# AlfredUg/MiCall-Lite

Hardware: AMD Instinct MI355X
Metric: paired 2×251 nt reads/sec mapped+realigned; fraction of HBM roofline (higher is better)
Workload: dtype int32; 1 GPU; C2: synthetic 2x251 nt HIV-1 pol read pairs (10% divergent sample genome, 0.5% errors), prelim_map end-to-end vs 74 seeds + 1 remap iteration(s) (--local vs consensus) + pileups, default projects.json; pairs_per_gpu=1000000, read_len=251, parallelism=dp1 (one GPU, no collective), dist_world=1

## Files before the change

### include/micall_hip.h

```cpp
#ifndef MICALL_HIP_H
#define MICALL_HIP_H

#include <stddef.h>
#include <stdint.h>

#ifdef __cplusplus
extern "C" {
#endif

#define MH_MAXOPS 128

enum { MH_E2E = 0, MH_LOCAL = 1 };
enum { MH_OP_M = 0, MH_OP_I = 1, MH_OP_D = 2, MH_OP_S = 4 };

typedef struct {
    int mode;
    int rdg_open, rdg_ext;
    int rfg_open, rfg_ext;
    int maxins;
} mh_params;

typedef struct {
    int32_t ref, pos, rev, score, secbest, flag, mapq, rnext, pnext, tlen;
    int32_t sam_ref, sam_pos, xm, xo, xg, nm, ys, yt, yf, n_cigar;
// ... 21 lines not shown
int mh_reads_count(mh_ctx *ctx, int64_t *n_reads, int *paired);

typedef struct mh_fastq mh_fastq;
int mh_fastq_open_part(const char *path, int fd, int part, int parts, mh_fastq **out, int64_t *info);
int mh_fastq_scan_part(const char *path, int fd, int part, int parts, int64_t *info);
int mh_fastq_member_open(const char *path, int fd, int part, int parts, mh_fastq **out, int64_t *info);
int mh_fastq_member_decode(mh_fastq *fq, int64_t end_bit, int64_t *info);
int mh_fastq_member_tail(mh_fastq *fq, const char *window, char *tail);
int mh_fastq_member_finish(mh_fastq *fq, const char *window, int64_t c0, int64_t c1, int64_t *info);
int mh_fastq_frame(mh_fastq *fq, int64_t line0, int starts_line, int64_t *out5);
int mh_fastq_record_offset(mh_fastq *fq, int64_t k, int64_t *off);
int mh_fastq_splice(mh_fastq *fq, int64_t lo, int64_t hi, const char *front, int64_t flen,
                    const char *back, int64_t blen);
int mh_fastq_view(mh_fastq *fq, const char **data, int64_t *len);
int mh_fastq_close(mh_fastq *fq);
int mh_fastq_parse(mh_fastq *fq1, mh_fastq *fq2, char *names, size_t names_cap, uint8_t *seq,
                   uint8_t *qual, size_t bases_cap, int32_t *lens, int64_t reads_cap, int64_t *n_reads,
                   int64_t *n_bases, size_t *names_used);
int mh_reads_load_staged(mh_ctx *ctx, mh_fastq *fq1, mh_fastq *fq2, const int64_t *range4,
                         int64_t fastq_lines1, int64_t *n_reads);
int mh_reads_fastq_lines(mh_ctx *ctx, int64_t *lines1);

int mh_map(mh_ctx *ctx, const mh_params *par);
int mh_alns_fetch(mh_ctx *ctx, int64_t first, int64_t n, mh_aln *out);
int mh_map_counts(mh_ctx *ctx, int64_t *lines, int64_t *filtered, int64_t *mapped,
                  int64_t *first_row, int64_t *first_mapped, int64_t *unmapped,
                  int64_t *star_lines, int64_t *star_first);
int mh_map_stats(mh_ctx *ctx, int64_t *out5);
int mh_test_set_capacities(mh_ctx *ctx, int64_t cigar_pool_words, int64_t pileup_events,
                           int64_t pileup_event_bytes, int64_t token_bytes);
int mh_test_pileup_info(mh_ctx *ctx, int64_t *out16, int n_refs, int32_t *win_len);
int mh_test_force_index_collision(mh_ctx *ctx, int on);
int mh_retry_counts(mh_ctx *ctx, int64_t *out4);
int mh_test_set_gotoh_wait(mh_ctx *ctx, int64_t ticks);
int mh_recs_fetch(mh_ctx *ctx, int64_t first, int64_t n, int32_t *out20);
int mh_recs_fetch_fields(mh_ctx *ctx, int64_t first, int64_t n, int field0, int nfields, int32_t *out);
int mh_reads_set_names(mh_ctx *ctx, int64_t n, const char *const *names);
int mh_format_rows(mh_ctx *ctx, int style, const int64_t *order, int64_t first, int64_t n,
                   const char *const *refnames, char *buf, size_t cap, size_t *used);
int mh_format_segments(mh_ctx *ctx, int style, const int64_t *order, int64_t n,
                       const char *const *refnames, int n_seg, const int64_t *seg_rows,
                       int64_t *seg_bytes);
int mh_write_segments(mh_ctx *ctx, int fd, const int64_t *seg_off, uint32_t *crc);
uint32_t mh_crc32_combine(uint32_t a, uint32_t b, int64_t len_b);
int mh_file_crc32(int fd, int64_t *size, uint32_t *crc);
enum { MH_PHASE_INFLATE = 0, MH_PHASE_PARSE = 1, MH_PHASE_UPLOAD = 2, MH_PHASE_FORMAT = 3,
       MH_PHASE_WRITE = 4, MH_PHASES = 5 };
int mh_phase_times(mh_ctx *ctx, double *ms, int reset);
int mh_write_rows_crc(mh_ctx *ctx, int style, const int64_t *order, int64_t first, int64_t n,
                      const char *const *refnames, int fd, int64_t offset, int64_t *written,
                      uint32_t *crc);

int mh_rows_load(mh_ctx *ctx, int64_t n_rows, const int32_t *flag, const int32_t *ref,
                 const int32_t *pos, const int32_t *cigar_off, const int32_t *n_cigar,
                 const uint32_t *cigar, const uint8_t *seq, const uint8_t *qual,
                 const int64_t *offsets, const int32_t *lens, int64_t n_units,
                 const int64_t *unit_rows);
int mh_rows_load_csv(mh_ctx *ctx, const char *text, int64_t len, int n_refs,
                     const char *const *refnames, int64_t *n_rows, int64_t *n_units,
                     int32_t *n_present);
int mh_rows_info(mh_ctx *ctx, int32_t *out4, int32_t *present, char *unknown, size_t cap);
#define MH_PILEUP_SLACK 2048
int mh_pileup(mh_ctx *ctx, int source, int q_cutoff, int n_refs, const int32_t *ref_lens);
int mh_pileup_only(mh_ctx *ctx, int source, int q_cutoff, int n_refs, const int32_t *ref_lens, int n_sel,
                   const int32_t *sel);
int mh_pileup_dims(mh_ctx *ctx, int *n_refs, int32_t *cap, int64_t *n_events,
// ... 132 lines not shown
```

### micall-lite_amd/csrc/mh_a2c.hip

```cpp
#include <algorithm>
#include <atomic>
#include <charconv>
#include <chrono>
#include <cstring>
#include <deque>
#include <map>
#include <string>
#include <unordered_map>
#include <vector>

#include "mh_gunzip.h"
#include "mh_internal.h"
#include "mh_sam2aln.h"
#include "mh_text.h"

namespace mh {

constexpr int A2C_W = 21;
constexpr int A2C_LANES = 3 * A2C_W;
constexpr int A2C_CHUNK = 1024;
constexpr int A2C_NAA = 21;
constexpr int A2C_STRIDE = A2C_NAA + 18;
constexpr int A2C_CELLS = A2C_LANES * A2C_STRIDE;
constexpr int A2C_SLOTS = 4;
// ... 698 lines not shown
    if (int st = a2c_upload(S, S.d_bin_rows, bin_rows.data(), bin_rows.size(), s)) return st;
    if (int st = a2c_upload(S, S.d_chunks, chunks.data(), chunks.size(), s)) return st;
    if (int st = a2c_upload(S, S.d_code, S.code, 512, s)) return st;
    if (int st = a2c_upload(S, S.d_cls, S.cls, 256, s)) return st;
    return a2c_count_chunks(c, S, chunks.size());
}

static int a2c_count_chunks(Ctx &c, A2CState &S, size_t n_chunks)
{
    hipStream_t s = c.stream;
    const size_t cells = (size_t)S.n_bins * A2C_CELLS;
    if (int st = a2c_reserve(S, S.d_cnt, sizeof(uint32_t) * cells)) return st;
    if (int st = a2c_reserve(S, S.d_first, sizeof(uint32_t) * cells)) return st;
    if (cells) {
        MH_HIP(hipMemsetAsync(S.d_cnt, 0, sizeof(uint32_t) * cells, s));
        MH_HIP(hipMemsetAsync(S.d_first, 0xff, sizeof(uint32_t) * cells, s));
    }
    if (n_chunks) {
        A2CCountArgs a{S.d_text, S.d_rows, S.d_bin_rows, S.d_chunks, S.d_code, S.d_cls,
                       S.d_cnt, S.d_first};
        const int p0 = prof_begin(c, "k_a2c_count");
        hipLaunchKernelGGL(k_a2c_count, dim3((unsigned)n_chunks), dim3(256), 0, s, a);
        prof_end(c, p0);
        MH_HIP(hipGetLastError());
    }
    S.h_cnt.resize(cells);
    S.h_first.resize(cells);
    if (cells) {
        MH_HIP(hipMemcpyAsync(S.h_cnt.data(), S.d_cnt, sizeof(uint32_t) * cells,
                              hipMemcpyDeviceToHost, s));
        MH_HIP(hipMemcpyAsync(S.h_first.data(), S.d_first, sizeof(uint32_t) * cells,
                              hipMemcpyDeviceToHost, s));
    }
    MH_HIP(hipStreamSynchronize(s));
    prof_flush(c);
    return 0;
}

static int a2c_parse_csv(A2CState &S, const char *text, int64_t len, bool &use_pool,
                         int64_t body_lo = -1, int64_t body_hi = -1)
{
    const char *p = text, *end = text + len;
    std::vector<std::string> head;
    S.rows.clear();
    S.dev_rows = false;
    S.g_first.assign(1, 0);
    S.g_ref.clear();
    S.g_qcut.clear();
    S.pool.clear();
    use_pool = false;
    if (!csv_record(p, end, head)) return 0;
    if (body_lo >= 0) {
        p = text + std::max<int64_t>(body_lo, p - text);
        end = text + std::max<int64_t>(body_hi, p - text);
    }
    static const char *const want[N_COLS] = {"refname", "qcut", "count", "offset", "seq"};
    int col[N_COLS];
    int need = 0;
    for (int k = 0; k < N_COLS; ++k) {
        col[k] = -1;
        for (size_t z = 0; z < head.size(); ++z)
            if (head[z] == want[k]) col[k] = (int)z;
        need = std::max(need, col[k] + 1);
    }
    const int64_t body = end - p;
    const bool quoted = memchr(p, '"', (size_t)body) != nullptr;
    for (int k = 0; k < N_COLS; ++k)
// ... 188 lines not shown
    S.g_qcut.clear();
    for (int64_t g = 0; g < ng; ++g) {
        S.g_ref.push_back(Q.names[(size_t)O.g_name[g]]);
        S.g_qcut.push_back(std::to_string(O.g_qcut[g]));
    }
    S.g_ncod.assign(3 * (size_t)ng, 0);
    S.g_bin0.assign((size_t)ng + 1, 0);
    S.n_bins = 0;
    hipStream_t s = c.stream;
    if (int st = a2c_upload(S, S.d_code, S.code, 512, s)) return st;
    if (int st = a2c_upload(S, S.d_cls, S.cls, 256, s)) return st;
    size_t n_chunks = 0;
    auto t1 = t0;
    if (n) {
        std::vector<int32_t> gfirst(O.g_first.begin(), O.g_first.end());
        if (int st = a2c_upload(S, S.d_order, O.rows.data(), (size_t)n, s)) return st;
        if (int st = a2c_upload(S, S.d_gfirst, gfirst.data(), gfirst.size(), s)) return st;
        if (int st = a2c_reserve(S, S.d_text, (size_t)text_len + 16)) return st;
        if (int st = a2c_reserve(S, S.d_rows, sizeof(A2CRow) * (size_t)n)) return st;
        if (int st = a2c_reserve(S, S.d_ncod, sizeof(int32_t) * (3 * (size_t)ng + 1))) return st;
        MH_HIP(hipMemcpyAsync(S.d_text, Q.d_gather, (size_t)text_len, hipMemcpyDeviceToDevice, s));
        MH_HIP(hipMemsetAsync(S.d_text + text_len, 0, 16, s));
        MH_HIP(hipMemsetAsync(S.d_ncod, 0, sizeof(int32_t) * (3 * (size_t)ng + 1), s));
        int64_t per_block = (n + 2047) / 2048;
        per_block = std::max<int64_t>(256 / A2C_TEAM, (per_block + 15) & ~(int64_t)15);
        A2CStageArgs a{S.d_order, S.d_gfirst, Q.d_goff, Q.d_res, Q.d_uniq, S.d_text, S.d_cls, S.d_rows,
                       S.d_ncod, (int32_t)n, (int32_t)ng, (int32_t)per_block};
        const int p0 = prof_begin(c, "k_a2c_stage");
        hipLaunchKernelGGL(k_a2c_stage, dim3((unsigned)((n + per_block - 1) / per_block)), dim3(256), 0, s, a);
        prof_end(c, p0);
        MH_HIP(hipGetLastError());
        std::vector<int32_t> ncod(3 * (size_t)ng + 1);
        MH_HIP(hipMemcpyAsync(ncod.data(), S.d_ncod, sizeof(int32_t) * ncod.size(), hipMemcpyDeviceToHost, s));
        MH_HIP(hipStreamSynchronize(s));
        prof_flush(c);
        if (ncod[3 * (size_t)ng]) return 1;
        S.t_parse = ms_since(t0);
        t1 = std::chrono::steady_clock::now();
        std::vector<int32_t> gbin0((size_t)ng + 1, 0);
        for (int64_t g = 0; g < ng; ++g) {
            const int32_t *nc = &ncod[3 * (size_t)g];
            for (int f = 0; f < 3; ++f) S.g_ncod[3 * (size_t)g + f] = nc[f];
            const int top = std::max(nc[0], std::max(nc[1], nc[2]));
            S.g_bin0[(size_t)g + 1] = S.g_bin0[(size_t)g] + (top + A2C_W - 1) / A2C_W;
            if (S.g_bin0[(size_t)g + 1] >= INT32_MAX) return 1;
            gbin0[(size_t)g + 1] = (int32_t)S.g_bin0[(size_t)g + 1];
        }
        S.n_bins = S.g_bin0[(size_t)ng];
        const size_t nb = (size_t)S.n_bins;
        if (int st = a2c_upload(S, S.d_gbin0, gbin0.data(), gbin0.size(), s)) return st;
        if (int st = a2c_reserve(S, S.d_bstart, sizeof(unsigned long long) * (nb + 1))) return st;
        if (int st = a2c_reserve(S, S.d_bcur, sizeof(unsigned long long) * (nb + 1))) return st;
        MH_HIP(hipMemsetAsync(S.d_bcur, 0, sizeof(unsigned long long) * (nb + 1), s));
        A2CBinArgs b{S.d_rows, S.d_gfirst, S.d_gbin0, (int32_t)n, (int32_t)ng, S.d_bcur, nullptr, nullptr, 0};
        const unsigned row_blocks = (unsigned)((n + 255) / 256);
        const int p1 = prof_begin(c, "k_a2c_bin_count");
        hipLaunchKernelGGL(k_a2c_bin_count, dim3(row_blocks), dim3(256), 0, s, b);
        prof_end(c, p1);
        const int p2 = prof_begin(c, "k_a2c_bin_scan");
        hipLaunchKernelGGL(k_a2c_bin_scan, dim3(1), dim3(1024), 0, s, S.d_bcur, S.d_bstart, (int)nb);
        prof_end(c, p2);
        MH_HIP(hipGetLastError());
        std::vector<unsigned long long> start(nb + 1);
        MH_HIP(hipMemcpyAsync(start.data(), S.d_bstart, sizeof(unsigned long long) * (nb + 1),
                              hipMemcpyDeviceToHost, s));
        MH_HIP(hipMemcpyAsync(S.d_bcur, S.d_bstart, sizeof(unsigned long long) * (nb + 1),
                              hipMemcpyDeviceToDevice, s));
        MH_HIP(hipStreamSynchronize(s));
        std::vector<A2CChunk> chunks;
        for (int64_t g = 0; g < ng; ++g)
            for (int64_t bin = S.g_bin0[(size_t)g]; bin < S.g_bin0[(size_t)g + 1]; ++bin)
                for (int64_t i = (int64_t)start[(size_t)bin]; i < (int64_t)start[(size_t)bin + 1]; i += A2C_CHUNK)
                    chunks.push_back({(int32_t)bin, (int32_t)((bin - S.g_bin0[(size_t)g]) * A2C_W), i,
                                      std::min<int64_t>(i + A2C_CHUNK, (int64_t)start[(size_t)bin + 1])});
        n_chunks = chunks.size();
        if (int st = a2c_reserve(S, S.d_bin_rows, sizeof(int32_t) * (size_t)start[nb])) return st;
        if (int st = a2c_upload(S, S.d_chunks, chunks.data(), chunks.size(), s)) return st;
        b.cnt = nullptr;
        b.cur = S.d_bcur;
        b.bin_rows = S.d_bin_rows;
        b.total = start[nb];
        const int p3 = prof_begin(c, "k_a2c_bin_fill");
        hipLaunchKernelGGL(k_a2c_bin_fill, dim3(row_blocks), dim3(256), 0, s, b);
        prof_end(c, p3);
        MH_HIP(hipGetLastError());
    } else {
        S.t_parse = ms_since(t0);
        t1 = std::chrono::steady_clock::now();
    }
    if (int st = a2c_count_chunks(c, S, n_chunks)) return st;
    S.t_count = ms_since(t1);
    if (n_groups) *n_groups = ng;
    return 0;
}

extern "C" int mh_a2c_load_resident(mh_ctx *ctx, int slot, const char *codon_chars, int64_t *n_groups)
{
    if (!ctx || slot < 0 || slot >= A2C_SLOTS) return -3;
    Ctx &c = *ctx_of(ctx);
    MH_HIP(hipSetDevice(c.device));
    A2CState &S = *a2c_state(c, slot);
// ... 167 lines not shown
    };
    A2CInsArgs a{};
    uint64_t tsize = 1024;
    unsigned long long ctr[3] = {0, 0, 0};
    std::vector<int32_t> lr(2 * (size_t)n_ranges);
    std::vector<A2CEntry> ent;
    std::vector<int64_t> eoff;
    hipError_t e = hipMalloc(&d_lr, sizeof(int32_t) * lr.size());
    for (int k = 0; k < n_ranges; ++k) { lr[k] = left[k]; lr[n_ranges + k] = right[k]; }
    if (e == hipSuccess) e = hipMemcpyAsync(d_lr, lr.data(), sizeof(int32_t) * lr.size(), hipMemcpyHostToDevice, s);
    if (e == hipSuccess) e = hipMalloc(&d_h, sizeof(uint64_t) * np);
    if (e == hipSuccess) e = hipMalloc(&d_ctr, sizeof(unsigned long long) * 3);
    if (e == hipSuccess) e = hipMemsetAsync(d_ctr, 0, sizeof(unsigned long long) * 3, s);
    if (e != hipSuccess) { fail(e, "mh_a2c_inserts alloc"); goto done; }
    a.text = S.d_text;
    a.rows = S.d_rows + S.g_first[g];
    a.row0 = S.dev_rows ? 0 : S.rows[(size_t)S.g_first[g]].local;
    a.code = S.d_code;
    a.cls = S.d_cls;
    a.left = d_lr;
    a.right = d_lr + n_ranges;
    a.n_rows = nr;
    a.n_pairs = np;
    a.frame = frame;
    a.h = d_h;
    a.ctr = d_ctr;
    {
        const int p0 = prof_begin(c, "k_a2c_ins");
        hipLaunchKernelGGL(k_a2c_ins_hash, dim3((unsigned)((np + 255) / 256)), dim3(256), 0, s, a);
        prof_end(c, p0);
    }
    e = hipGetLastError();
    if (e == hipSuccess) e = hipMemcpyAsync(ctr, d_ctr, sizeof(ctr), hipMemcpyDeviceToHost, s);
    if (e == hipSuccess) e = hipStreamSynchronize(s);
    if (e != hipSuccess) { fail(e, "k_a2c_ins_hash"); goto done; }
    if (ctr[0] == 0) goto done;
    while (tsize < 2 * ctr[0]) tsize <<= 1;
    e = hipMalloc(&d_tkey, sizeof(uint64_t) * tsize);
    if (e == hipSuccess) e = hipMalloc(&d_tcnt, sizeof(unsigned long long) * tsize);
    if (e == hipSuccess) e = hipMalloc(&d_tfirst, sizeof(uint32_t) * tsize);
    if (e == hipSuccess) e = hipMalloc(&d_trange, sizeof(int32_t) * tsize);
    if (e == hipSuccess) e = hipMalloc(&d_ent, sizeof(A2CEntry) * ctr[0]);
    if (e == hipSuccess) e = hipMemsetAsync(d_tkey, 0, sizeof(uint64_t) * tsize, s);
    if (e == hipSuccess) e = hipMemsetAsync(d_tcnt, 0, sizeof(unsigned long long) * tsize, s);
    if (e == hipSuccess) e = hipMemsetAsync(d_tfirst, 0xff, sizeof(uint32_t) * tsize, s);
    if (e != hipSuccess) { fail(e, "mh_a2c_inserts table"); goto done; }
    a.tkey = d_tkey;
    a.tcnt = d_tcnt;
    a.tfirst = d_tfirst;
    a.trange = d_trange;
    a.mask = tsize - 1;
    a.entries = d_ent;
    {
        const int p0 = prof_begin(c, "k_a2c_ins");
        hipLaunchKernelGGL(k_a2c_ins_count, dim3((unsigned)((np + 255) / 256)), dim3(256), 0, s, a);
        hipLaunchKernelGGL(k_a2c_ins_verify, dim3((unsigned)((np + 255) / 256)), dim3(256), 0, s, a);
        hipLaunchKernelGGL(k_a2c_ins_compact, dim3((unsigned)((tsize + 255) / 256)), dim3(256), 0, s, a);
        prof_end(c, p0);
    }
    e = hipGetLastError();
    if (e == hipSuccess) e = hipMemcpyAsync(ctr, d_ctr, sizeof(ctr), hipMemcpyDeviceToHost, s);
    if (e == hipSuccess) e = hipStreamSynchronize(s);
    if (e != hipSuccess) { fail(e, "k_a2c_ins"); goto done; }
    if (ctr[1]) {
        set_error("aln2counts: insertion-string hash collision (distinct strings share a key)");
        rc = -4;
        goto done;
    }
    ent.resize(ctr[2]);
    e = copy_sync(c, ent.data(), d_ent, sizeof(A2CEntry) * ent.size(), hipMemcpyDeviceToHost);
    if (e != hipSuccess) { fail(e, "mh_a2c_inserts fetch"); goto done; }
    std::sort(ent.begin(), ent.end(), [](const A2CEntry &x, const A2CEntry &y) {
        return x.range != y.range ? x.range < y.range : x.first < y.first;
    });
    eoff.resize(ent.size() + 1);
    eoff[0] = 0;
    for (size_t k = 0; k < ent.size(); ++k) eoff[k + 1] = eoff[k] + ent[k].n_codons + 1;
    S.aminos.assign((size_t)eoff.back(), '\0');
    e = hipMalloc(&d_sorted, sizeof(A2CEntry) * ent.size());
    if (e == hipSuccess) e = hipMalloc(&d_eoff, sizeof(int64_t) * eoff.size());
    if (e == hipSuccess) e = hipMalloc(&d_out, (size_t)eoff.back());
    if (e == hipSuccess) e = hipMemcpyAsync(d_sorted, ent.data(), sizeof(A2CEntry) * ent.size(), hipMemcpyHostToDevice, s);
    if (e == hipSuccess) e = hipMemcpyAsync(d_eoff, eoff.data(), sizeof(int64_t) * eoff.size(), hipMemcpyHostToDevice, s);
    if (e != hipSuccess) { fail(e, "mh_a2c_inserts gather"); goto done; }
    hipLaunchKernelGGL(k_a2c_ins_gather, dim3((unsigned)((ent.size() + 255) / 256)), dim3(256), 0, s,
                       a, d_sorted, d_eoff, (int64_t)ent.size(), d_out);
    e = hipGetLastError();
    if (e == hipSuccess) e = hipMemcpyAsync(&S.aminos[0], d_out, (size_t)eoff.back(), hipMemcpyDeviceToHost, s);
    if (e == hipSuccess) e = hipStreamSynchronize(s);
    if (e != hipSuccess) { fail(e, "k_a2c_ins_gather"); goto done; }
    S.entries = std::move(ent);
    if (n_entries) *n_entries = (int64_t)S.entries.size();
done:
    hipFree(d_lr); hipFree(d_h); hipFree(d_ctr); hipFree(d_tkey); hipFree(d_tcnt);
    hipFree(d_tfirst); hipFree(d_trange); hipFree(d_ent); hipFree(d_sorted); hipFree(d_eoff);
    hipFree(d_out);
    prof_flush(c);
    S.t_ins += ms_since(t0);
    if (rc) a2c_clear_inserts(S);
    return rc;
}

extern "C" int mh_a2c_insert_entries(mh_ctx *ctx, int slot, int32_t *range, int64_t *count,
                                     uint32_t *first, char *aminos, size_t cap, size_t *used)
{
    if (!ctx || slot < 0 || slot >= A2C_SLOTS) return -3;
    Ctx &c = *ctx_of(ctx);
    A2CState &S = *a2c_state(c, slot);
    for (size_t k = 0; k < S.entries.size(); ++k) {
        if (range) range[k] = S.entries[k].range;
        if (count) count[k] = (int64_t)S.entries[k].count;
        if (first) first[k] = S.entries[k].first;
    }
    if (used) *used = S.aminos.size();
    if (aminos) {
        if (cap < S.aminos.size()) { set_error("mh_a2c_insert_entries: buffer too small"); return -2; }
        memcpy(aminos, S.aminos.data(), S.aminos.size());
    }
    return 0;
}

extern "C" int mh_a2c_insert_rows(mh_ctx *ctx, int slot, const char *lead, int n_ranges,
// ... 316 lines not shown
```

### micall-lite_amd/csrc/mh_api.cpp

```cpp
#include <errno.h>
#include <fcntl.h>
#include <sys/mman.h>
#include <sys/stat.h>
#include <unistd.h>
#include <zlib.h>

#include <algorithm>
#include <atomic>
#include <chrono>
#include <cmath>
#include <cstdarg>
#include <cstdio>
#include <cstring>
#include <memory>
#include <new>
#include <string>
#include <condition_variable>
#include <deque>
#include <exception>
#include <mutex>
#include <functional>
#include <string_view>
#include <thread>
#include <unordered_map>
#include <vector>

#include "mh_fastq.h"
#include "mh_gunzip.h"
#include "mh_internal.h"
#include "mh_text.h"

#include <map>
#include <tuple>

namespace mh {

static thread_local char g_err[1024];

void set_error(const char *fmt, ...)
{
    va_list ap;
    va_start(ap, fmt);
    vsnprintf(g_err, sizeof(g_err), fmt, ap);
    va_end(ap);
}

static std::string last_error_text() { return std::string(g_err); }

int hip_fail(hipError_t e, const char *what)
{
    set_error("HIP error %d (%s) in %s", (int)e, hipGetErrorString(e), what);
    return -4;
}

hipError_t copy_sync(Ctx &c, void *dst, const void *src, size_t bytes, hipMemcpyKind kind)
{
    hipError_t e = hipMemcpyAsync(dst, src, bytes, kind, c.stream);
    return e == hipSuccess ? hipStreamSynchronize(c.stream) : e;
}

int prof_begin(Ctx &c, const char *name)
{
    if (!c.prof) return -1;
    ProfPending p{name, nullptr, nullptr};
    if (hipEventCreate(&p.a) != hipSuccess || hipEventCreate(&p.b) != hipSuccess) return -1;
    hipEventRecord(p.a, c.stream);
    c.prof_pending.push_back(p);
    return (int)c.prof_pending.size() - 1;
}

void prof_end(Ctx &c, int slot)
{
    if (slot < 0 || slot >= (int)c.prof_pending.size()) return;
    hipEventRecord(c.prof_pending[slot].b, c.stream);
}

void prof_flush(Ctx &c)
{
    for (auto &p : c.prof_pending) {
        float ms = 0.f;
        if (hipEventSynchronize(p.b) == hipSuccess && hipEventElapsedTime(&ms, p.a, p.b) == hipSuccess) {
            ProfEntry &e = c.prof_acc[p.name];
            e.ms += ms;
            e.launches += 1;
        }
        hipEventDestroy(p.a);
        hipEventDestroy(p.b);
    }
    c.prof_pending.clear();
}

static int seed_interval(int mode, int len)
{
    const double f = mode == MH_LOCAL ? 0.75 : 1.15;
    int iv = (int)(1.0 + f * std::sqrt((double)len) + 0.5);
    return iv < 1 ? 1 : iv;
}

static int min_score(int mode, int len)
{
    if (mode == MH_LOCAL) {
        double v = 20.0 + 8.0 * std::log((double)(len > 0 ? len : 1));
        long s = (long)v;
        return (int)(s < 0 ? 0 : s);
    }
    long s = (long)(-0.6 + -0.6 * (double)len);
    return (int)(s > 0 ? 0 : s);
}

static int n_ceil(int len) { return (int)(0.0 + 0.15 * (double)len); }

static int max_gaps(int perfect, int minsc, int oe, int ex)
{
// ... 136 lines not shown
static inline uint64_t mix64(uint64_t h, uint64_t w)
{
    h = (h ^ w) * 0x9E3779B97F4A7C15ull;
    return h ^ (h >> 29);
}

static uint64_t signature(int n, const char *const *seqs, int seedlen)
{
    uint64_t h = 1469598103934665603ull ^ (uint64_t)seedlen;
    for (int r = 0; r < n; ++r) {
        const size_t len = std::strlen(seqs[r]);
        h = mix64(h, (uint64_t)len);
        uint64_t q[4] = {h, h ^ 1, h ^ 2, h ^ 3};
        size_t i = 0;
        for (; i + 32 <= len; i += 32)
            for (int k = 0; k < 4; ++k) {
                uint64_t w;
                std::memcpy(&w, seqs[r] + i + 8 * k, 8);
                q[k] = mix64(q[k], w);
            }
        h = mix64(mix64(mix64(mix64(h, q[0]), q[1]), q[2]), q[3]);
        for (; i + 8 <= len; i += 8) {
            uint64_t w;
            std::memcpy(&w, seqs[r] + i, 8);
            h = mix64(h, w);
        }
        uint64_t tail = 0;
        std::memcpy(&tail, seqs[r] + i, len - i);
        h = mix64(h, tail ^ 0xffull << 56);
    }
    return mix64(h, (uint64_t)n);
}

static int build_index(DevIndex &ix, int n_refs, const char *const *seqs, int seedlen)
{
    static const bool trace = getenv("MH_INDEX_TRACE") && *getenv("MH_INDEX_TRACE") == '1';
    const auto tb = std::chrono::steady_clock::now();
    auto mark = [&](const char *what) {
        if (trace)
            fprintf(stderr, "index %s %.2f ms\n", what,
                    std::chrono::duration<double, std::milli>(std::chrono::steady_clock::now() - tb).count());
    };
    struct E { uint64_t key; int32_t ref, pos; };
    std::vector<int64_t> ref_off(n_refs);
    std::vector<int32_t> ref_len(n_refs);
    int64_t total_len = 0;
    for (int r = 0; r < n_refs; ++r) {
        ref_len[r] = (int)std::strlen(seqs[r]);
        ref_off[r] = total_len;
        total_len += ref_len[r];
    }
    std::vector<uint8_t> codes((size_t)total_len);
    const int nt = std::max(1, std::min<int>(s2a_threads(), n_refs));
    std::vector<std::vector<E>> per(n_refs);
    mark("pre");
    std::vector<double> t_start((size_t)nt, 0.0);
    {
        std::atomic<int> next(0);
        par_for(nt, [&](int t) {
            t_start[(size_t)t] = std::chrono::duration<double, std::milli>(std::chrono::steady_clock::now() - tb).count();
            for (int r; (r = next.fetch_add(1)) < n_refs;) {
                const int L = ref_len[r];
                uint8_t *cr = codes.data() + ref_off[r];
                std::vector<E> &v = per[r];
                v.reserve(L > seedlen ? (size_t)(L - seedlen + 1) : 0);
                uint64_t key = 0;
                int last_n = -1;
// ... 69 lines not shown
        const uint32_t c = codes[j] > 3 ? 0u : codes[j];
        cplane[2 * (j >> 5)] |= (c & 1u) << (j & 31);
        cplane[2 * (j >> 5) + 1] |= (c >> 1) << (j & 31);
    }
    auto al = [](size_t x) { return (x + 255) & ~(size_t)255; };
    constexpr int NP = 8;
    const size_t sz[NP] = {codes.size(), sizeof(int64_t) * (size_t)n_refs, sizeof(int32_t) * (size_t)n_refs,
                           sizeof(uint4) * cap, sizeof(int2) * hits.size(), sizeof(uint32_t) * code2.size(),
                           sizeof(uint32_t) * ncode.size(), sizeof(uint32_t) * cplane.size()};
    const void *src[NP] = {codes.data(), ref_off.data(), ref_len.data(), hent.data(), hits.data(),
                           code2.data(), ncode.data(), cplane.data()};
    size_t at[NP], total = 0;
    for (int x = 0; x < NP; ++x) { at[x] = total; total += al(sz[x]); }
    if ((int64_t)total > ix.cap_blob) {
        hipFree(ix.blob);
        ix.blob = nullptr;
        ix.cap_blob = 0;
        MH_HIP(hipMalloc(&ix.blob, total));
        ix.cap_blob = (int64_t)total;
    }
    mark("planes+alloc");
    std::vector<uint8_t> stage(total);
    for (int x = 0; x < NP; ++x) if (sz[x]) std::memcpy(stage.data() + at[x], src[x], sz[x]);
    mark("stage");
    uint8_t *d = (uint8_t *)ix.blob;
    ix.codes = d + at[0];
    ix.ref_off = (int64_t *)(d + at[1]);
    ix.ref_len = (int32_t *)(d + at[2]);
    ix.hent = (uint4 *)(d + at[3]);
    ix.hits = (int2 *)(d + at[4]);
    ix.code2 = (uint32_t *)(d + at[5]);
    ix.ncode = (uint32_t *)(d + at[6]);
    ix.cplane = (uint32_t *)(d + at[7]);
    MH_HIP(hipMemcpy(ix.blob, stage.data(), total, hipMemcpyHostToDevice));
    mark("upload");
    return 0;
}

static int load_reads(CtxEx &c, DevReads &dst, HostReads &host, int64_t n, int paired,
                      const uint8_t *seq, const uint8_t *qual, const int64_t *offsets,
                      const int32_t *lens, bool keep_host, HostReads *adopt = nullptr)
{
    if (n < 0 || (paired && (n & 1))) { set_error("reads: bad count"); return -3; }
    int max_len = 0;
    int64_t src_total = 0;
    for (int64_t r = 0; r < n; ++r) {
        if (lens[r] < 0 || lens[r] > MAXLEN) {
            set_error("reads: read %lld has length %d (max %d)", (long long)r, lens[r], MAXLEN);
            return -3;
        }
        max_len = std::max(max_len, (int)lens[r]);
        src_total = std::max(src_total, offsets[r] + lens[r]);
    }
    std::vector<int64_t> off(n > 0 ? n : 1);
    int64_t total = 0;
    for (int64_t r = 0; r < n; ++r) {
        off[r] = total;
        total += ((int64_t)lens[r] + 31) / 32 * 32;
    }
    MH_HIP(hipStreamSynchronize(c.stream));
    dst.n = n;
    dst.paired = paired;
    dst.max_len = max_len;
    dst.total_bases = total;
    MH_HIP(grow_dev(c, dst.seq2, sizeof(uint32_t) * (total / 16 + 8)));
    MH_HIP(grow_dev(c, dst.nmask, sizeof(uint32_t) * (total / 32 + 8)));
    MH_HIP(grow_dev(c, dst.qual, (size_t)total + 64));
    MH_HIP(grow_dev(c, dst.off, sizeof(int64_t) * (n > 0 ? n : 1)));
    MH_HIP(grow_dev(c, dst.len, sizeof(int32_t) * (n > 0 ? n : 1)));
    MH_HIP(hipMemsetAsync(dst.seq2, 0, sizeof(uint32_t) * (total / 16 + 8), c.stream));
    MH_HIP(hipMemsetAsync(dst.nmask, 0, sizeof(uint32_t) * (total / 32 + 8), c.stream));
    if (n > 0) {
        MH_HIP(hipMemcpyAsync(dst.off, off.data(), sizeof(int64_t) * n, hipMemcpyHostToDevice, c.stream));
        MH_HIP(hipMemcpyAsync(dst.len, lens, sizeof(int32_t) * n, hipMemcpyHostToDevice, c.stream));
        MH_HIP(grow_dev(c, c.stage_seq, (size_t)src_total + 1));
        MH_HIP(grow_dev(c, c.stage_qual, (size_t)src_total + 1));
        MH_HIP(grow_dev(c, c.stage_off, sizeof(int64_t) * (size_t)n));
        MH_HIP(hipMemcpyAsync(c.stage_seq, seq, src_total, hipMemcpyHostToDevice, c.stream));
        MH_HIP(hipMemcpyAsync(c.stage_qual, qual, src_total, hipMemcpyHostToDevice, c.stream));
        MH_HIP(hipMemcpyAsync(c.stage_off, offsets, sizeof(int64_t) * n, hipMemcpyHostToDevice, c.stream));
        MH_HIP(launch_pack_reads(dst, c.stage_seq, c.stage_qual, c.stage_off, c.stream));
        MH_HIP(hipStreamSynchronize(c.stream));
    }
    if (adopt) {
        host = std::move(*adopt);
    } else if (keep_host) {
        host.seq.assign(seq, seq + src_total);
        host.qual.assign(qual, qual + src_total);
        host.off.assign(offsets, offsets + n);
        host.len.assign(lens, lens + n);
    }
    return 0;
}

static inline void qname_span(const char *h, size_t n, bool paired, size_t *at, size_t *len)
{
    size_t a = (n && h[0] == '@') ? 1 : 0;
    while (a < n && (h[a] == ' ' || h[a] == '\t')) ++a;
    size_t b = a;
    constexpr uint64_t ONES = 0x0101010101010101ull, HIGH = 0x8080808080808080ull;
    while (b + 8 <= n) {
        uint64_t w;
        std::memcpy(&w, h + b, 8);
        if (((w - ONES * 0x21) | w) & HIGH) break;
        b += 8;
    }
    while (b < n && h[b] != ' ' && h[b] != '\t' && h[b] != '\r') ++b;
    if (paired && b - a > 2 && h[b - 2] == '/' && (h[b - 1] == '1' || h[b - 1] == '2')) b -= 2;
    *at = a;
    *len = b - a;
}

struct Fastq {
    TextBuf data;
    std::vector<int64_t> name_at, seq_at, qual_at;
// ... 160 lines not shown
}

int mh_ctx_create(int device, mh_ctx **out)
{
    if (!out) return -3;
    *out = nullptr;
    int n = 0;
    if (hipGetDeviceCount(&n) != hipSuccess || n == 0) {
        set_error("no HIP device available (the MI355X path has no CPU fallback)");
        return -5;
    }
    if (device < 0 || device >= n) { set_error("bad device %d", device); return -3; }
    MH_HIP(hipSetDevice(device));
    hipDeviceProp_t prop;
    MH_HIP(hipGetDeviceProperties(&prop, device));
    if (std::strncmp(prop.gcnArchName, "gfx950", 6) != 0) {
        set_error("device %d is %s, libmicall_hip is built for gfx950 only", device, prop.gcnArchName);
        return -5;
    }
    CtxEx *c = new (std::nothrow) CtxEx();
    if (!c) return -2;
    c->device = device;
    hipError_t e = hipStreamCreateWithFlags(&c->stream, hipStreamNonBlocking);
    if (e != hipSuccess) { delete c; return hip_fail(e, "hipStreamCreate"); }
    *out = reinterpret_cast<mh_ctx *>(c);
    return 0;
}

int mh_ctx_destroy(mh_ctx *ctx)
{
    if (!ctx) return 0;
    CtxEx *c = X(ctx);
    hipSetDevice(c->device);
    hipStreamSynchronize(c->stream);
    free_reads(c->reads);
    free_reads(c->rows.reads);
    hipFree(c->stage_seq); hipFree(c->stage_qual); hipFree(c->stage_off);
    for (auto &ix : c->cache) free_index(ix);
    free_index(c->small);
    MapState &M = c->map;
    hipFree(M.cand); hipFree(M.n_cand); hipFree(M.yf); hipFree(M.work); hipFree(M.rwork); hipFree(M.skey); hipFree(M.sinfo);
    hipFree(M.pool); hipFree(M.pool_used); hipFree(M.rec); hipFree(M.counters); hipFree(M.ref_stats);
    if (M.stats_pin) hipHostFree(M.stats_pin);
    M.stats_pin = nullptr;
    M.stats_pin_cap = 0;
    RowState &R = c->rows;
    hipFree(R.flag); hipFree(R.ref); hipFree(R.pos); hipFree(R.cig_off); hipFree(R.n_cigar);
    hipFree(R.cigar); hipFree(R.units);
    PileState &P = c->pile;
    hipFree(c->gotoh_buf);
    hipFree(P.dense); hipFree(P.nflag); hipFree(P.dflag); hipFree(P.read_counts);
    hipFree(P.first_unit); hipFree(P.max_pos); hipFree(P.ev); hipFree(P.ev_pool);
    hipFree(P.tok_slot); hipFree(P.tok_cnt); hipFree(P.tok_used); hipFree(P.tok_meta);
    hipFree(P.tok_bytes);
    hipFree(P.ev_counters);
    if (P.land) hipHostFree(P.land);
    P.land = nullptr;
    if (P.tok_pin) hipHostFree(P.tok_pin);
    P.tok_pin = nullptr;
    P.tok_pin_cap = 0;
    P.land_cap = 0;
    P.land_ok = false;
    hipFree(P.ins_scratch);
    hipFree(P.sel);
    hipFree(P.win_map);
    for (auto &kv : c->len_tabs) hipFree(kv.second);
    if (c->pin) hipHostFree(c->pin);
    s2a_free(*c);
    censor_free(*c);
    a2c_free(*c);
    hipStreamDestroy(c->stream);
    delete c;
    return 0;
}

int mh_ctx_sync(mh_ctx *ctx)
{
    if (!ctx) return -3;
    MH_HIP(hipSetDevice(X(ctx)->device));
    MH_HIP(hipStreamSynchronize(X(ctx)->stream));
    return 0;
}

int mh_ctx_stream(mh_ctx *ctx, void **stream)
{
    if (!ctx || !stream) return -3;
    *stream = (void *)X(ctx)->stream;
    return 0;
}

int mh_index_build(mh_ctx *ctx, int n_refs, const char *const *seqs, int seedlen)
{
    if (!ctx || n_refs < 0 || (n_refs > 0 && !seqs) || seedlen < 8 || seedlen > 32) {
        set_error("mh_index_build: bad arguments");
        return -3;
    }
    CtxEx *c = X(ctx);
    MH_HIP(hipSetDevice(c->device));
    MH_HIP(hipStreamSynchronize(c->stream));
    int64_t total = 0;
    for (int r = 0; r < n_refs; ++r) total += (int64_t)std::strlen(seqs[r]);
    const uint64_t sig = c->force_index_collision ? 0x5eedull : signature(n_refs, seqs, seedlen);
    const bool cacheable = total > 65536;
    c->index = DevIndex{};
    for (size_t e = 0; e < c->cache.size(); ++e) {
        const DevIndex &ix = c->cache[e];
        if (ix.sig != sig || ix.n_refs != n_refs || ix.seedlen != seedlen) continue;
        const std::string &t = c->cache_text[e];
        bool same = t.size() == (size_t)(total + n_refs);
        size_t at = 0;
        for (int r = 0; same && r < n_refs; ++r) {
            const size_t len = std::strlen(seqs[r]);
            same = std::memcmp(t.data() + at, seqs[r], len + 1) == 0;
            at += len + 1;
        }
        if (same) {
            c->index = ix;
            return 0;
        }
    }
    if (!cacheable) {
        if (int st = build_index(c->small, n_refs, seqs, seedlen)) return st;
        c->small.sig = sig;
        c->index = c->small;
        return 0;
    }
    DevIndex ix;
    if (int st = build_index(ix, n_refs, seqs, seedlen)) { free_index(ix); return st; }
    ix.sig = sig;
    if (c->cache.size() >= 2) {
        free_index(c->cache.front());
        c->cache.erase(c->cache.begin());
        c->cache_text.erase(c->cache_text.begin());
    }
    std::string text;
    text.reserve((size_t)(total + n_refs));
    for (int r = 0; r < n_refs; ++r) text.append(seqs[r], std::strlen(seqs[r]) + 1);
    c->cache.push_back(ix);
    c->cache_text.push_back(std::move(text));
    c->index = ix;
    return 0;
}

int mh_reads_load(mh_ctx *ctx, int64_t n_reads, int paired, const uint8_t *seq,
                  const uint8_t *qual, const int64_t *offsets, const int32_t *lens)
{
    if (!ctx || (n_reads > 0 && (!seq || !qual || !offsets || !lens))) return -3;
    CtxEx *c = X(ctx);
    MH_HIP(hipSetDevice(c->device));
    c->names.clear();
    c->map.valid = false;
    return load_reads(*c, c->reads, c->host, n_reads, paired, seq, qual, offsets, lens, true);
}

int mh_reads_load_fastq(mh_ctx *ctx, const char *path1, const char *path2, int64_t *n_reads)
{
    return mh_reads_load_fastq_part(ctx, path1, path2, 0, 1, n_reads, nullptr);
}

static int host_reads_from(Fastq &a, Fastq *b, int64_t a0, int64_t a1, int64_t b0, int64_t b1,
                           HostReads &h, NameTable &names, double *names_ms, double *copy_ms)
// ... 249 lines not shown
            memcpy(seq, h.seq.data(), (size_t)bases);
            memcpy(qual, h.qual.data(), (size_t)bases);
        }
        return 0;
    } catch (const std::bad_alloc &) {
        set_error("mh_fastq_parse: out of memory");
        return -2;
    }
}

int mh_reads_count(mh_ctx *ctx, int64_t *n_reads, int *paired)
{
    if (!ctx) return -3;
    if (n_reads) *n_reads = X(ctx)->reads.n;
    if (paired) *paired = X(ctx)->reads.paired;
    return 0;
}

int mh_reads_set_names(mh_ctx *ctx, int64_t n, const char *const *names)
{
    if (!ctx || n != X(ctx)->reads.n) { set_error("mh_reads_set_names: count mismatch"); return -3; }
    CtxEx *c = X(ctx);
    c->names.assign(names, n);
    return 0;
}

int mh_map(mh_ctx *ctx, const mh_params *par)
{
    if (!ctx || !par) return -3;
    CtxEx *c = X(ctx);
    MH_HIP(hipSetDevice(c->device));
    if (int st = prepare_len_tab(*c, *par)) return st;
    int st = run_map(*c, *par);
    if (st == 0) MH_HIP(hipStreamSynchronize(c->stream));
    prof_flush(*c);
    c->rec_cache.clear();
    ++c->map_gen;
    c->fmt_valid = false;
    c->fmt_chunks.clear();
    return st;
}

int mh_probe_extend(mh_ctx *ctx, const mh_params *par, int n, const int32_t *items, int32_t *out)
{
    if (!ctx || !par || n < 0 || (n > 0 && (!items || !out))) return -3;
    CtxEx *c = X(ctx);
    MH_HIP(hipSetDevice(c->device));
    if (int st = prepare_len_tab(*c, *par)) return st;
    return run_probe_ext(*c, *par, n, items, out);
}

int mh_profile(mh_ctx *ctx, int enable)
{
    if (!ctx) return -3;
    CtxEx *c = X(ctx);
    c->prof = enable != 0;
    c->prof_acc.clear();
    return 0;
}

int mh_profile_get(mh_ctx *ctx, const char *kernel, double *total_ms, int64_t *launches)
{
    if (!ctx || !kernel) return -3;
    CtxEx *c = X(ctx);
    prof_flush(*c);
    auto it = c->prof_acc.find(kernel);
    if (total_ms) *total_ms = it == c->prof_acc.end() ? 0.0 : it->second.ms;
// ... 59 lines not shown
}

int mh_map_stats(mh_ctx *ctx, int64_t *out5)
{
    if (!ctx || !out5) return -3;
    int64_t *out4 = out5;
    CtxEx *c = X(ctx);
    MapState &M = c->map;
    if (!M.valid) { set_error("no mapping results (call mh_map)"); return -3; }
    out4[0] = M.n_reads;
    out4[1] = M.last_work;
    out4[2] = M.last_cigar;
    out4[3] = M.last_fast;
    out5[4] = M.last_rescue;
    return 0;
}

int mh_test_force_index_collision(mh_ctx *ctx, int on)
{
    if (!ctx) return -3;
    X(ctx)->force_index_collision = on != 0;
    return 0;
}

int mh_test_set_capacities(mh_ctx *ctx, int64_t cigar_pool_words, int64_t pileup_events,
                           int64_t pileup_event_bytes, int64_t token_bytes)
{
    if (!ctx || cigar_pool_words < 0 || pileup_events < 0 || pileup_event_bytes < 0 || token_bytes < 0) {
        set_error("mh_test_set_capacities: bad arguments");
        return -3;
    }
    CtxEx *c = X(ctx);
    MH_HIP(hipSetDevice(c->device));
    MH_HIP(hipStreamSynchronize(c->stream));
    MapState &M = c->map;
    PileState &P = c->pile;
    hipFree(M.pool); M.pool = nullptr; M.pool_cap = 0;
    hipFree(P.ev); P.ev = nullptr; P.ev_cap = 0;
    hipFree(P.ev_pool); P.ev_pool = nullptr; P.pool_cap = 0;
    hipFree(P.tok_bytes); P.tok_bytes = nullptr; P.tok_bytes_cap = 0;
    M.valid = false;
    TestCaps &t = c->test_caps;
    t.cigar_pool_words = cigar_pool_words;
    t.pile_events = pileup_events;
    t.pile_event_bytes = pileup_event_bytes;
    t.token_bytes = token_bytes;
    return 0;
}

int mh_retry_counts(mh_ctx *ctx, int64_t *out4)
{
    if (!ctx || !out4) return -3;
    for (int k = 0; k < RETRY_KINDS; ++k) out4[k] = X(ctx)->retries[k];
    return 0;
}

int mh_test_set_gotoh_wait(mh_ctx *ctx, int64_t ticks)
{
    if (!ctx || ticks < 0) { set_error("mh_test_set_gotoh_wait: bad arguments"); return -3; }
    X(ctx)->test_caps.gotoh_wait_ticks = ticks;
    return 0;
}

int mh_recs_fetch(mh_ctx *ctx, int64_t first, int64_t n, int32_t *out20)
{
    if (!ctx || (n > 0 && !out20)) return -3;
    CtxEx *c = X(ctx);
    MapState &M = c->map;
    if (!M.valid) { set_error("no mapping results (call mh_map)"); return -3; }
    if (first < 0 || n < 0 || first + n > M.n_reads) { set_error("record range out of bounds"); return -3; }
    MH_HIP(hipSetDevice(c->device));
    if (n == 0) return 0;
    MH_HIP(hipMemcpy2DAsync(out20, sizeof(int32_t) * 20, M.rec + first, sizeof(Rec), sizeof(int32_t) * 20,
                            (size_t)n, hipMemcpyDeviceToHost, c->stream));
    MH_HIP(hipStreamSynchronize(c->stream));
    return 0;
}

int mh_recs_fetch_fields(mh_ctx *ctx, int64_t first, int64_t n, int field0, int nfields, int32_t *out)
{
    if (!ctx || (n > 0 && !out) || field0 < 0 || nfields < 1 || field0 + nfields > 20) return -3;
    CtxEx *c = X(ctx);
    MapState &M = c->map;
    if (!M.valid) { set_error("no mapping results (call mh_map)"); return -3; }
    if (first < 0 || n < 0 || first + n > M.n_reads) { set_error("record range out of bounds"); return -3; }
    MH_HIP(hipSetDevice(c->device));
    if (n == 0) return 0;
    MH_HIP(hipMemcpy2DAsync(out, sizeof(int32_t) * nfields, (const int32_t *)(M.rec + first) + field0, sizeof(Rec),
                            sizeof(int32_t) * nfields, (size_t)n, hipMemcpyDeviceToHost, c->stream));
    MH_HIP(hipStreamSynchronize(c->stream));
    return 0;
}

static inline char *put_int(char *o, int64_t v)
{
    char t[24];
    int n = 0;
    uint64_t u = v < 0 ? (uint64_t)(-(v + 1)) + 1 : (uint64_t)v;
    do { t[n++] = (char)('0' + u % 10); u /= 10; } while (u);
    if (v < 0) *o++ = '-';
    while (n) *o++ = t[--n];
    return o;
}

static inline char *put_str(char *o, const char *s, size_t n)
{
    std::memcpy(o, s, n);
    return o + n;
}

static inline uint64_t has_byte(uint64_t w, uint8_t c)
{
    const uint64_t x = w ^ (0x0101010101010101ull * c);
    return (x - 0x0101010101010101ull) & ~x & 0x8080808080808080ull;
}

static inline bool needs_quotes(const char *s, size_t n)
{
    size_t i = 0;
    uint64_t hit = 0;
    for (; i + 8 <= n; i += 8) {
        uint64_t w;
        std::memcpy(&w, s + i, 8);
// ... 923 lines not shown
        c->csv_rows_info.push_back(R.flag[i]);
        c->csv_rows_info.push_back(R.maxm[i]);
        c->csv_rows_info.push_back(dref[i]);
    }
    if (n_rows) *n_rows = nr;
    if (n_units) *n_units = nu;
    if (n_present) *n_present = (int32_t)c->csv_present.size();
    return 0;
}

extern "C" int mh_rows_info(mh_ctx *ctx, int32_t *out4, int32_t *present, char *unknown,
                            size_t cap)
{
    if (!ctx) return -3;
    CtxEx *c = X(ctx);
    if (out4) std::memcpy(out4, c->csv_rows_info.data(), sizeof(int32_t) * c->csv_rows_info.size());
    if (present) std::memcpy(present, c->csv_present.data(), sizeof(int32_t) * c->csv_present.size());
    if (unknown) {
        std::string all;
        for (auto &u : c->csv_unknown) { all += u; all.push_back('\n'); }
        if (all.size() + 1 > cap) { set_error("mh_rows_info: name buffer too small"); return -2; }
        std::memcpy(unknown, all.c_str(), all.size() + 1);
    }
    return 0;
}

extern "C" int mh_reads_fastq_lines(mh_ctx *ctx, int64_t *lines1)
{
    if (!ctx || !lines1) return -3;
    *lines1 = X(ctx)->fastq_lines1;
    return 0;
}

struct Landing {
    int64_t *read_counts, *first_unit;
    int32_t *max_pos;
    int64_t *ev_counters;
    size_t bytes;
};

static Landing landing_of(const PileState &P)
{
    const size_t nr = (size_t)P.n_refs, ev_at = (20 * nr + 7) & ~(size_t)7;
    return Landing{(int64_t *)P.land, (int64_t *)(P.land + 8 * nr), (int32_t *)(P.land + 16 * nr),
                   (int64_t *)(P.land + ev_at), 20 * nr + 64};
}

int mh_pileup(mh_ctx *ctx, int source, int q_cutoff, int n_refs, const int32_t *ref_lens)
{
    return mh_pileup_only(ctx, source, q_cutoff, n_refs, ref_lens, -1, nullptr);
}

int mh_pileup_only(mh_ctx *ctx, int source, int q_cutoff, int n_refs, const int32_t *ref_lens, int n_sel,
                   const int32_t *sel)
{
    if (!ctx || n_refs < 0 || (n_refs > 0 && !ref_lens) || (source != 0 && source != 1) ||
        (n_sel > 0 && !sel))
        return -3;
    CtxEx *c = X(ctx);
    MH_HIP(hipSetDevice(c->device));
    c->pile.only.clear();
    if (n_sel >= 0) {
        c->pile.only.assign((size_t)n_refs, 0);
        for (int k = 0; k < n_sel; ++k) {
            if (sel[k] < 0 || sel[k] >= n_refs) { set_error("mh_pileup_only: reference %d out of range", sel[k]); return -3; }
            c->pile.only[(size_t)sel[k]] = 1;
        }
    }
    int32_t cap = 1;
    for (int r = 0; r < n_refs; ++r) cap = std::max(cap, ref_lens[r] + MH_PILEUP_SLACK);
    c->pile.n_refs = n_refs;
    c->pile.cap = cap;
    c->pile.ref_lens.assign(ref_lens, ref_lens + n_refs);
    c->pile.land_ok = false;
    int st = run_pileup(*c, source, q_cutoff);
    if (st == 0) {
        PileState &P = c->pile;
        const size_t nr = (size_t)P.n_refs, need = landing_of(P).bytes;
        if (P.land_cap < need) {
            if (P.land) hipHostFree(P.land);
            P.land = nullptr;
            P.land_cap = 0;
            if (hipHostMalloc((void **)&P.land, need, hipHostMallocDefault) == hipSuccess) P.land_cap = need;
            else P.land = nullptr;
        }
        if (P.land && P.read_counts && P.first_unit && P.max_pos) {
            const Landing L = landing_of(P);
            bool ok = hipMemcpyAsync(L.read_counts, P.read_counts, 8 * nr, hipMemcpyDeviceToHost, c->stream) == hipSuccess &&
                      hipMemcpyAsync(L.first_unit, P.first_unit, 8 * nr, hipMemcpyDeviceToHost, c->stream) == hipSuccess &&
                      hipMemcpyAsync(L.max_pos, P.max_pos, 4 * nr, hipMemcpyDeviceToHost, c->stream) == hipSuccess;
            if (ok && P.ev_counters)
                ok = hipMemcpyAsync(L.ev_counters, P.ev_counters, 32, hipMemcpyDeviceToHost, c->stream) == hipSuccess;
            P.land_ok = ok;
        }
        MH_HIP(hipStreamSynchronize(c->stream));
    }
    prof_flush(*c);
    return st;
}

static int aggregate_tokens(CtxEx &c)
{
    PileState &P = c.pile;
    if (c.tok_gen == P.gen) return 0;
    c.tok_ref.clear(); c.tok_pos.clear(); c.tok_off.clear(); c.tok_len.clear();
    c.tok_count.clear(); c.tok_pool.clear();
    int64_t ctr[4] = {0, 0, 0, 0};
    if (P.ev_counters && P.land_ok)
        std::memcpy(ctr, landing_of(P).ev_counters, sizeof(ctr));
    else if (P.ev_counters)
        MH_HIP(copy_sync(c, ctr, P.ev_counters, sizeof(ctr), hipMemcpyDeviceToHost));
    const int64_t ne = ctr[0];
    if (ne > 0) {
        std::vector<int32_t> meta;
        std::string bytes;
        if (int st = run_token_aggregate(c, ne, ctr[1], meta, bytes)) return st;
        struct Key { int32_t ref, pos, off, len; int64_t count; };
        const size_t nd = meta.size() / 5;
        std::vector<Key> uniq(nd);
        for (size_t d = 0; d < nd; ++d)
            uniq[d] = Key{meta[5 * d], meta[5 * d + 1], meta[5 * d + 2], meta[5 * d + 3], meta[5 * d + 4]};
        const char *pb = bytes.data();
        std::sort(uniq.begin(), uniq.end(), [pb](const Key &a, const Key &b) {
            if (a.ref != b.ref) return a.ref < b.ref;
            if (a.pos != b.pos) return a.pos < b.pos;
            const int cmp = std::memcmp(pb + a.off, pb + b.off, (size_t)std::min(a.len, b.len));
            if (cmp != 0) return cmp < 0;
            return a.len < b.len;
        });
// ... 26 lines not shown

struct FetchPart {
    const void *src;
    size_t bytes;
    void *dst;
};

static int fetch_parts(CtxEx &c, const FetchPart *parts, int n)
{
    size_t total = 0;
    for (int i = 0; i < n; ++i) if (parts[i].dst) total += (parts[i].bytes + 255) & ~(size_t)255;
    if (total > ((size_t)64 << 20)) {
        for (int i = 0; i < n; ++i)
            if (parts[i].dst && parts[i].bytes)
                MH_HIP(copy_sync(c, parts[i].dst, parts[i].src, parts[i].bytes, hipMemcpyDeviceToHost));
        return 0;
    }
    if (c.pin_cap < total) {
        if (c.pin) hipHostFree(c.pin);
        c.pin = nullptr;
        c.pin_cap = 0;
        const size_t cap = total > ((size_t)1 << 20) ? total : ((size_t)1 << 20);
        MH_HIP(hipHostMalloc(&c.pin, cap, hipHostMallocDefault));
        c.pin_cap = cap;
    }
    size_t at = 0;
    for (int i = 0; i < n; ++i) {
        if (!parts[i].dst) continue;
        if (parts[i].bytes)
            MH_HIP(hipMemcpyAsync((char *)c.pin + at, parts[i].src, parts[i].bytes, hipMemcpyDeviceToHost,
                                  c.stream));
        at += (parts[i].bytes + 255) & ~(size_t)255;
    }
    MH_HIP(hipStreamSynchronize(c.stream));
    at = 0;
    for (int i = 0; i < n; ++i) {
        if (!parts[i].dst) continue;
        if (parts[i].bytes) std::memcpy(parts[i].dst, (const char *)c.pin + at, parts[i].bytes);
        at += (parts[i].bytes + 255) & ~(size_t)255;
    }
    return 0;
}

int mh_pileup_fetch(mh_ctx *ctx, int32_t *dense, uint8_t *nflag, uint8_t *dflag,
                    int64_t *read_counts, int64_t *first_unit, int32_t *max_pos)
{
    if (!ctx) return -3;
    CtxEx *c = X(ctx);
    PileState &P = c->pile;
    if (!P.dense) { set_error("no pileup (call mh_pileup)"); return -3; }
    MH_HIP(hipSetDevice(c->device));
    const size_t cells = (size_t)P.n_refs * P.cap, nr = (size_t)P.n_refs;
    if (!dense && !nflag && !dflag && P.land_ok) {
        const Landing L = landing_of(P);
        if (read_counts) std::memcpy(read_counts, L.read_counts, 8 * nr);
        if (first_unit) std::memcpy(first_unit, L.first_unit, 8 * nr);
        if (max_pos) std::memcpy(max_pos, L.max_pos, 4 * nr);
        return 0;
    }
    const FetchPart parts[6] = {{P.dense, sizeof(int32_t) * 4 * cells, dense},
                                {P.nflag, cells, nflag},
                                {P.dflag, cells, dflag},
                                {P.read_counts, sizeof(int64_t) * nr, read_counts},
                                {P.first_unit, sizeof(int64_t) * nr, first_unit},
                                {P.max_pos, sizeof(int32_t) * nr, max_pos}};
    return fetch_parts(*c, parts, 6);
}

int mh_pileup_fetch_refs(mh_ctx *ctx, int n_sel, const int32_t *refs, int32_t *dense, uint8_t *nflag,
                         uint8_t *dflag)
{
    if (!ctx || n_sel < 0 || (n_sel > 0 && (!refs || !dense || !nflag || !dflag))) return -3;
    CtxEx *c = X(ctx);
    PileState &P = c->pile;
    if (!P.dense) { set_error("no pileup (call mh_pileup)"); return -3; }
    MH_HIP(hipSetDevice(c->device));
    std::vector<int32_t> mx((size_t)std::max(P.n_refs, 1));
    if (P.land_ok && P.land)
        std::memcpy(mx.data(), landing_of(P).max_pos, sizeof(int32_t) * (size_t)P.n_refs);
    else
        MH_HIP(copy_sync(*c, mx.data(), P.max_pos, sizeof(int32_t) * (size_t)P.n_refs, hipMemcpyDeviceToHost));
    std::vector<FetchPart> parts;
    parts.reserve(3 * (size_t)n_sel);
    for (int k = 0; k < n_sel; ++k) {
        const int r = refs[k];
        if (r < 0 || r >= P.n_refs) { set_error("mh_pileup_fetch_refs: ref %d out of range", r); return -3; }
        const int64_t rows = std::min<int64_t>(P.cap, std::max(mx[(size_t)r], 0));
        if (rows == 0) continue;
        const int64_t base = (int64_t)r * P.cap;
        parts.push_back({P.dense + 4 * base, sizeof(int32_t) * 4 * (size_t)rows, dense + 4 * base});
        parts.push_back({P.nflag + base, (size_t)rows, nflag + base});
        parts.push_back({P.dflag + base, (size_t)rows, dflag + base});
    }
    return parts.empty() ? 0 : fetch_parts(*c, parts.data(), (int)parts.size());
}

int mh_pileup_events(mh_ctx *ctx, int32_t *ref, int32_t *pos, int32_t *tok_off, int32_t *tok_len,
                     int64_t *count, char *pool)
{
    if (!ctx) return -3;
    CtxEx *c = X(ctx);
    MH_HIP(hipSetDevice(c->device));
    if (int st = aggregate_tokens(*c)) return st;
    const size_t n = c->tok_ref.size();
    if (ref) std::memcpy(ref, c->tok_ref.data(), sizeof(int32_t) * n);
    if (pos) std::memcpy(pos, c->tok_pos.data(), sizeof(int32_t) * n);
    if (tok_off) std::memcpy(tok_off, c->tok_off.data(), sizeof(int32_t) * n);
    if (tok_len) std::memcpy(tok_len, c->tok_len.data(), sizeof(int32_t) * n);
    if (count) std::memcpy(count, c->tok_count.data(), sizeof(int64_t) * n);
    if (pool) std::memcpy(pool, c->tok_pool.data(), c->tok_pool.size());
    return 0;
}

static int gotoh_threw(const char *entry, const std::exception &e)
{
    set_error("%s: out of memory (%s)", entry, e.what());
    return -2;
}

// ... 288 lines not shown
```

### micall-lite_amd/csrc/mh_censor.hip

```cpp
#include <sys/types.h>
#include <unistd.h>
#include <zlib.h>

#include <algorithm>
#include <atomic>
#include <cerrno>
#include <chrono>
#include <cstring>
#include <exception>
#include <memory>
#include <string>
#include <string_view>
#include <thread>
#include <unordered_map>
#include <vector>

#include "mh_fastq.h"
#include "mh_gunzip.h"
#include "mh_internal.h"

namespace mh {

struct CensorState {
    TextBuf text;
// ... 229 lines not shown
        H(hipMalloc(&D.d_sign, 4 * nr), "hipMalloc");
        H(hipMalloc(&D.d_keep, 8 * nr), "hipMalloc");
    }
    if ((int64_t)bm.size() > D.cap_bad) {
        hipFree(D.d_bad);
        D.cap_bad = (int64_t)bm.size();
        H(hipMalloc(&D.d_bad, 4 * bm.size()), "hipMalloc");
    }
    if (!D.d_sums) H(hipMalloc(&D.d_sums, 16), "hipMalloc");
    if (st) { censor_free_device(D); return st; }
    H(hipMemcpyAsync(D.d_text, C.text.data(), C.text.size(), hipMemcpyHostToDevice, s), "H2D");
    H(hipMemcpyAsync(D.d_s0, C.s0.data(), 8 * nr, hipMemcpyHostToDevice, s), "H2D");
    H(hipMemcpyAsync(D.d_q0, C.q0.data(), 8 * nr, hipMemcpyHostToDevice, s), "H2D");
    H(hipMemcpyAsync(D.d_sl, C.sl.data(), 4 * nr, hipMemcpyHostToDevice, s), "H2D");
    H(hipMemcpyAsync(D.d_ql, C.ql.data(), 4 * nr, hipMemcpyHostToDevice, s), "H2D");
    H(hipMemcpyAsync(D.d_tile, C.tile.data(), 4 * nr, hipMemcpyHostToDevice, s), "H2D");
    H(hipMemcpyAsync(D.d_sign, C.sign.data(), 4 * nr, hipMemcpyHostToDevice, s), "H2D");
    H(hipMemcpyAsync(D.d_bad, bm.data(), 4 * bm.size(), hipMemcpyHostToDevice, s), "H2D");
    H(hipMemsetAsync(D.d_sums, 0, 16, s), "memset");
    CensorArgs a{D.d_text, D.d_s0, D.d_q0, D.d_sl, D.d_ql, D.d_tile, D.d_sign, nr, D.d_bad, maxc,
                 words, D.d_keep, D.d_sums};
    int64_t blocks = (nr + 3) / 4;
    if (blocks > 256 * 64) blocks = 256 * 64;
    if (!st) {
        const int pk = prof_begin(c, "k_censor");
        hipLaunchKernelGGL(k_censor, dim3((unsigned)blocks), dim3(256), 0, s, a);
        prof_end(c, pk);
        H(hipGetLastError(), "k_censor");
    }
    unsigned long long sums[2] = {0, 0};
    H(hipMemcpyAsync(C.text.data(), D.d_text, C.text.size(), hipMemcpyDeviceToHost, s), "D2H");
    H(hipMemcpyAsync(C.keep.data(), D.d_keep, 8 * nr, hipMemcpyDeviceToHost, s), "D2H");
    H(hipMemcpyAsync(sums, D.d_sums, 16, hipMemcpyDeviceToHost, s), "D2H");
    H(hipStreamSynchronize(s), "sync");
    if (st) return st;
    prof_flush(c);
    C.score_sum = (long long)sums[0];
    C.base_count = (long long)sums[1];
    return 0;
}

constexpr int64_t CENSOR_BLOCK = (int64_t)8 << 20;

static int censor_emit(CensorState &C, int dst_gzip)
{
    const int64_t nr = (int64_t)C.h0.size();
    const int64_t n = (int64_t)C.text.size();
    std::vector<int64_t> bstart{0};
    for (int64_t r = 0, base = 0; r < nr; ++r) {
        if (C.h0[r] - base >= CENSOR_BLOCK) { bstart.push_back(r); base = C.h0[r]; }
    }
    if (nr > 0) bstart.push_back(nr);
    const int64_t nb = (int64_t)bstart.size() - 1;
    if (nb <= 0) {
        C.out.clear();
        if (dst_gzip) {
            if (gzip_member("", 0, C.out, 1)) { set_error("censor: deflate failed"); return -2; }
        }
        if (C.sink_fd >= 0 && C.out.size()) {
            if (const int e = write_all_at(C.sink_fd, C.out.data(), C.out.size(), C.sink_pos)) {
                set_error("censor: write failed (%s)", strerror(e));
                return -4;
            }
            C.sink_pos += (int64_t)C.out.size();
            C.out.clear();
        }
        return 0;
// ... 230 lines not shown
```

### micall-lite_amd/csrc/mh_gotoh.hip

```cpp
#include <limits.h>

#include <atomic>
#include <functional>
#include <memory>
#include <thread>
#include <algorithm>
#include <mutex>
#include <type_traits>
#include <unordered_map>
#include <utility>
#include <vector>

#include "mh_internal.h"

namespace mh {

constexpr int G_INF = INT_MAX;
constexpr int G_HUGE = 1 << 29;
enum { GA = 1, GB = 2, GC = 4, GD = 8, GE_ = 16, GF = 32, GG = 64 };
constexpr int GOTOH_THREADS = 1024;
constexpr int GBLK = 32;
constexpr int BBLK = 16;
constexpr uint32_t GOOB = 0x80000000u;
constexpr int TBD = 128, TBR = 128;
// ... 1048 lines not shown
    prof_end(c, pf);
    const int pb = prof_begin(c, "k_gotoh_bwd");
    hipLaunchKernelGGL(k_gotoh_bwd, dim3((unsigned)strips), dim3(64), sizeof(int) * BBLK, st, S);
    prof_end(c, pb);
    const int pg = prof_begin(c, "k_gotoh");
    hipLaunchKernelGGL(k_gotoh_tb, dim3((unsigned)count), dim3(GOTOH_THREADS), TB_LDS, st,
                       (const GotohArgs *)(d + off_args));
    prof_end(c, pg);
    std::vector<int> lres(lev ? 4 * (size_t)count : 0);
    int lflag = 0;
    if (lev) {
        LevBatch LB;
        LB.args = (const LevArgs *)(d + off_lev);
        LB.tick = (const int2 *)(d + off_ltick);
        LB.strips = (int)ltick.size();
        LB.ticket = (int *)(d + off_lctr);
        LB.flags = (int *)(d + off_lctr + 4);
        LB.lut = (const uint8_t *)(d + off_lut);
        LB.ncodes = L + 1;
        LB.wait_ticks = wait_ticks;
        const int pl = prof_begin(c, "k_lev");
        hipLaunchKernelGGL(k_lev_prep, dim3((unsigned)count), dim3(64), 0, st, LB);
        if (LB.strips > 0)
            hipLaunchKernelGGL(k_lev, dim3((unsigned)LB.strips), dim3(64), (size_t)LB.ncodes * 64 * 8 + 256, st, LB);
        prof_end(c, pl);
    }
    hipError_t e = hipGetLastError();
    if (lev) {
        if (e == hipSuccess) e = hipMemcpyAsync(lres.data(), d + off_lres, sizeof(int) * lres.size(), hipMemcpyDeviceToHost, st);
        if (e == hipSuccess) e = hipMemcpyAsync(&lflag, d + off_lctr + 4, sizeof(int), hipMemcpyDeviceToHost, st);
    } else if (e == hipSuccess) {
        e = hipMemcpyAsync(oimg.get(), d + off_out, oo[count], hipMemcpyDeviceToHost, st);
    }
    if (e == hipSuccess) e = hipStreamSynchronize(st);
    if (e != hipSuccess) return hip_fail(e, "k_gotoh");
    if (S.stamps) {
        std::vector<unsigned long long> h((size_t)4 * strips * S.stamp_blocks);
        MH_HIP(hipMemcpy(h.data(), S.stamps, h.size() * sizeof(h[0]), hipMemcpyDeviceToHost));
        MH_HIP(hipFree(S.stamps));
        if (FILE *f = fopen(stamp_path, "wb")) {
            const int64_t hdr[2] = {strips, S.stamp_blocks};
            fwrite(hdr, sizeof(hdr), 1, f);
            fwrite(h.data(), sizeof(h[0]), h.size(), f);
            fclose(f);
        }
    }
    if (lev) {
        for (int t = 0; t < count; ++t) {
            const int *r = &lres[(size_t)4 * t];
            if (r[0] == -4 || lflag) {
                set_error("k_gotoh: a strip's wait for its neighbour timed out (alignment %d)", t);
                return -4;
            }
            status[t] = r[0];
            score[t] = r[1];
            lev_dist[t] = r[0] ? 0 : r[2];
        }
    }
    for (int t = 0; t < count && !lev; ++t) {
        const GotohArgs &A = args[t];
        int res[3];
        memcpy(res, &oimg[(const char *)A.result - d - off_out], sizeof(res));
        if (res[0] == -4) { set_error("k_gotoh: a strip's wait for its neighbour timed out (alignment %d)", t); return -4; }
        status[t] = res[0] ? -1 : 0;
        score[t] = res[1];
        const int len = res[0] ? 0 : res[2];
        const char *t1 = &oimg[A.out1 - d - off_out], *t2 = &oimg[A.out2 - d - off_out];
        for (int k = 0; k < len; ++k) { out1[t][k] = t1[len - 1 - k]; out2[t][k] = t2[len - 1 - k]; }
        out1[t][len] = out2[t][len] = '\0';
    }
// ... 51 lines not shown
```

### micall-lite_amd/csrc/mh_internal.h

```cpp
#pragma once
#include <hip/hip_runtime.h>
#include <stdint.h>
#include <string.h>

#include <map>
#include <mutex>
#include <string>
#include <string_view>
#include <tuple>
#include <vector>

#include "micall_hip.h"
#include "mh_gunzip.h"

namespace mh {

constexpr int BAND = 64;
constexpr int MAXCAND = 4;
constexpr int MAXHITS_SEED = 64;
constexpr int MAXHITS_MATE = 512;
constexpr int CLUSTER_GAP = 8;
constexpr int MAXSEEDS = 32;
constexpr int MAXLEN = 1024;
constexpr int GBAR = 4;
// ... 52 lines not shown

struct Cand {
    int32_t strand, ref, center, support;
};

struct Slot {
    int32_t valid, strand, ref, pos, end, score, xm, xo, xg, nm, n_cigar, cig_off;
    int32_t maxm;
};

struct alignas(16) SlotKey {
    int32_t rs;
    int32_t pos, end, score;
};
struct alignas(16) SlotInfo {
    int32_t cig_off;
    uint32_t xm_xo;
    uint32_t xg_nc;
    int32_t maxm;
};
static_assert(sizeof(SlotInfo) == 16, "a read's MAXCAND statistics fill half a 128-B line");

struct Rec {
    int32_t ref, pos, rev, score, secbest, flag, mapq, rnext, pnext, tlen;
    int32_t sam_ref, sam_pos, xm, xo, xg, nm, ys, yt, yf, n_cigar;
    int32_t cig_off, maxm;
};

__host__ __device__ inline int64_t slot_at(int32_t sid, int64_t plane)
{
    const uint32_t u = (uint32_t)sid;
    return (int64_t)(u % MAXCAND) * plane + (int64_t)(u / MAXCAND);
}

struct MapState {
    int64_t n_reads = 0;
    int n_refs = 0;
    mh_params par{};
    Cand *cand = nullptr;
    int32_t *n_cand = nullptr;
    int32_t *yf = nullptr;
    int32_t *work = nullptr;
    int32_t *rwork = nullptr;
    SlotKey *skey = nullptr;
    SlotInfo *sinfo = nullptr;
    uint32_t *pool = nullptr;
    int64_t pool_cap = 0;
    unsigned long long *pool_used = nullptr;
    Rec *rec = nullptr;
    int32_t *counters = nullptr;
    int64_t *ref_stats = nullptr;
    int64_t cap_reads = 0;
    int cap_refs = 0;
    int64_t last_work = 0;
    int64_t last_cigar = 0;
    int64_t last_fast = 0;
    int64_t last_rescue = 0;
    bool valid = false;
    std::vector<int64_t> stats_host;
    int64_t *stats_pin = nullptr;
    size_t stats_pin_cap = 0;
    bool stats_pin_ready = false;
    std::map<std::pair<const void *, int>, int> dp_occ;
    bool stats_host_valid = false;
};

struct RowState {
    int64_t n_rows = 0, n_units = 0;
    int32_t *flag = nullptr, *ref = nullptr, *pos = nullptr, *cig_off = nullptr,
            *n_cigar = nullptr;
    uint32_t *cigar = nullptr;
    int64_t *units = nullptr;
    DevReads reads;
    int hot_ref = -1;
    std::vector<int64_t> ref_rows;
    int max_span = 0;
};

struct PileState {
    int n_refs = 0;
    int32_t cap = 0;
    int32_t *dense = nullptr;
    uint8_t *nflag = nullptr;
    uint8_t *dflag = nullptr;
    int64_t *read_counts = nullptr;
    int64_t *first_unit = nullptr;
    int32_t *max_pos = nullptr;
    int32_t *ev = nullptr;
    char *ev_pool = nullptr;
    int64_t ev_cap = 0, pool_cap = 0;
    int64_t *ev_counters = nullptr;
    int64_t alloc_cells = 0;
    int alloc_refs = 0;
    int64_t gen = 0;
    char *land = nullptr;
    size_t land_cap = 0;
    bool land_ok = false;
    std::vector<int32_t> ref_lens;
    std::vector<uint8_t> only;
    int32_t *sel = nullptr;
    int sel_cap = 0;
    int32_t *win_map = nullptr;
    int win_map_cap = 0;
    char *ins_scratch = nullptr;
    int64_t ins_scratch_bytes = 0;
    std::map<std::tuple<int, int64_t, int>, std::pair<int, int>> shapes;
    int32_t *tok_slot = nullptr;
    uint32_t *tok_cnt = nullptr;
    int32_t *tok_used = nullptr;
    int64_t tok_cap = 0;
    int32_t *tok_meta = nullptr;
    char *tok_bytes = nullptr;
    int64_t tok_meta_cap = 0, tok_bytes_cap = 0;
    char *tok_pin = nullptr;
    size_t tok_pin_cap = 0;
    struct Info {
        int64_t blocks = 0, n_units = 0;
        int wpb = 0, win_words = 0;
        std::vector<int32_t> win_map;
        int64_t tok_insert_blocks = 0, tok_count_blocks = 0, tok_ne = 0, tok_nd = 0;
    } info;
};

hipError_t launch_pack_reads(DevReads &r, const uint8_t *d_seq, const uint8_t *d_qual,
                             const int64_t *d_src_off, hipStream_t s);
int run_map(struct Ctx &c, const mh_params &par);
int run_probe_ext(struct Ctx &c, const mh_params &par, int n, const int32_t *items, int32_t *out);
const int64_t *map_stats_host(struct Ctx &c);
int run_pileup(struct Ctx &c, int source, int q_cutoff);
int run_token_aggregate(struct Ctx &c, int64_t n_events, int64_t pool_used,
                        std::vector<int32_t> &meta, std::string &bytes);
int run_gotoh(struct Ctx &c, const char *s1, const char *s2, int gop, int gep, int is_global,
              const char *alphabet, const int *matrix, char *out1, char *out2, int cap,
              int *score);
int run_gotoh_batch(struct Ctx &c, int count, const char *const *s1, const char *const *s2,
                    int gop, int gep, int is_global, const char *alphabet, const int *matrix,
                    char *const *out1, char *const *out2, const int *cap, int *score,
                    int *status);
int run_gotoh_distance_batch(struct Ctx &c, int count, const char *const *s1, const char *const *s2,
                             const char *const *text, int gop, int gep, int is_global,
                             const char *alphabet, const int *matrix, int *dist, int *score,
                             int *status);

struct NameTable {
    TextBuf pool;
    std::vector<int64_t> off{0};
    size_t size() const { return off.size() - 1; }
    std::string_view operator[](size_t r) const
    {
        return std::string_view(pool.data() + off[r], (size_t)(off[r + 1] - off[r]));
    }
    void clear() { pool.clear(); off.assign(1, 0); }
    void assign(const char *const *names, int64_t n)
    {
        clear();
        off.resize((size_t)n + 1);
// ... 4 lines not shown
    void swap(NameTable &o) { pool.swap(o.pool); off.swap(o.off); }
};

struct ProfEntry {
    double ms = 0.0;
    int64_t launches = 0;
};

struct ProfPending {
    const char *name;
    hipEvent_t a, b;
};

struct S2AState;
struct CensorState;
struct A2CState;

struct TestCaps {
    int64_t cigar_pool_words = 0;
    int64_t pile_events = 0;
    int64_t pile_event_bytes = 0;
    int64_t token_bytes = 0;
    int64_t gotoh_wait_ticks = 0;
};

enum { RETRY_CIGAR_POOL = 0, RETRY_PILE_EVENTS = 1, RETRY_TOKEN_BYTES = 2, RETRY_GOTOH_WAIT = 3,
       RETRY_KINDS = 4 };

struct Ctx {
    int device = 0;
    TestCaps test_caps;
    int64_t retries[RETRY_KINDS] = {0, 0, 0, 0};
    int n_cu = 0;
    bool prof = false;
    std::map<std::string, ProfEntry> prof_acc;
    std::vector<ProfPending> prof_pending;
    hipStream_t stream = nullptr;
    DevReads reads;
    NameTable names;
    std::vector<std::string> host_seq, host_qual;
    DevIndex index;
    MapState map;
    RowState rows;
    PileState pile;
    int32_t *len_tab = nullptr;
    S2AState *s2a = nullptr;
    int64_t s2a_serial = 0;
    CensorState *censor = nullptr;
    A2CState **a2c = nullptr;
    int64_t len_tab_key = -1;
    std::map<int64_t, int32_t *> len_tabs;
    char *gotoh_buf = nullptr;
    size_t gotoh_cap = 0;
    std::mutex gotoh_mutex;
};

void set_error(const char *fmt, ...);
int host_read_text(Ctx &c, int64_t r, bool rev, char *seq, char *qual);
Ctx *ctx_of(mh_ctx *ctx);
void s2a_free(Ctx &c);
void censor_free(Ctx &c);
void a2c_free(Ctx &c);
int prof_begin(Ctx &c, const char *name);
void prof_end(Ctx &c, int slot);
void prof_flush(Ctx &c);
int hip_fail(hipError_t e, const char *what);
hipError_t copy_sync(Ctx &c, void *dst, const void *src, size_t bytes, hipMemcpyKind kind);

}

#define MH_HIP(call)                                                  \
    do {                                                              \
        hipError_t e_ = (call);                                       \
        if (e_ != hipSuccess) return ::mh::hip_fail(e_, #call);       \
    } while (0)
```

### micall-lite_amd/csrc/mh_map.hip

```cpp
#include <cstring>

#include "mh_internal.h"

namespace mh {

template <int CTRL, int ROWMASK = 0xF>
__device__ __forceinline__ int dpp(int old, int v)
{
    return __builtin_amdgcn_update_dpp(old, v, CTRL, ROWMASK, 0xF, false);
}
constexpr int DPP_ROW_SHR1 = 0x111, DPP_ROW_SHR2 = 0x112, DPP_ROW_SHR4 = 0x114,
              DPP_ROW_SHR8 = 0x118, DPP_WAVE_SHL1 = 0x130, DPP_WAVE_SHR1 = 0x138;

__device__ __forceinline__ int wave_uniform(int v) { return __builtin_amdgcn_readfirstlane(v); }

__device__ __forceinline__ void wave_sync()
{
    __builtin_amdgcn_fence(__ATOMIC_RELEASE, "wavefront");
    __builtin_amdgcn_wave_barrier();
    __builtin_amdgcn_fence(__ATOMIC_ACQUIRE, "wavefront");
}

template <class Op>
__device__ __forceinline__ int wave_scan_dpp(int v, int identity, Op op)
// ... 1589 lines not shown
        A.skey[at] = SlotKey{out.valid ? (out.ref << 1 | out.strand) : -1, out.pos, out.end, out.score};
        A.sinfo[at] = SlotInfo{out.cig_off, (uint32_t)out.xm | (uint32_t)out.xo << 16,
                                   (uint32_t)out.xg | (uint32_t)out.n_cigar << 16, out.maxm};
    }
    wave_sync();
}

template <int LOCAL>
__device__ void finish_ext(const DpArgs &A, const XItem &it, const XView &X, const uint32_t *bits,
                           int hcol, int best, int bi, int bl, int lane, int64_t &ck_base,
                           int &ck_left, int fast_low = -2)
{
    best = __builtin_amdgcn_readfirstlane(best);
    bi = __builtin_amdgcn_readfirstlane(bi);
    bl = __builtin_amdgcn_readfirstlane(bl);
    const WalkOut W = walk1<LOCAL>(A, it, X, bits, hcol, best, bi, bl, lane, fast_low);
    wave_sync();
    post_ext<LOCAL>(A, it, X, best, bi, bl, lane, ck_base, ck_left, W);
}

template <int LOCAL, int ROUND>
__global__ __launch_bounds__(256) void k_dp(DpArgs A)
{
    extern __shared__ __attribute__((aligned(16))) unsigned char smem[];
    const int lane = threadIdx.x & 63;
    const int wv = wave_uniform(threadIdx.x >> 6);
    const int wpb = blockDim.x >> 6;
    unsigned char *wbase = smem + (size_t)wv * A.wave_lds;
    uint32_t *bits = (uint32_t *)wbase;
    unsigned char *xbase = wbase + (size_t)32 * A.rows_pad;
    const XView X0 = xview(xbase, A.rows_pad, 0), X1 = xview(xbase, A.rows_pad, 1);
    unsigned char *raw = xbase + 2 * xview_bytes(A.rows_pad);
    const int n_work = A.counters[0];
    const int gmin = A.oeI < A.oeD ? A.oeI : A.oeD;

    int64_t ck_base = 0;
    int ck_left = 0;
    int n_fast = 0;
    constexpr int QCH = DP_QUEUE_CHUNK;
    const int gwaves = gridDim.x * wpb;
    constexpr bool one_round = ROUND > 0;
    int cA = (blockIdx.x * wpb + wv) * QCH, cB = 0, qv = 0, p = 0;
    auto grab = [&]() {
        if (lane == 0) qv = atomicAdd(A.queue, QCH) + gwaves * QCH;
    };
    grab();
    cB = __builtin_amdgcn_readfirstlane(qv);
    grab();
    auto at = [&](int d) {
        const int q = p + d;
        return q < QCH ? cA + q : cB + (q - QCH);
    };
    int w = cA;
    XItem cur{};
    int sid1 = 0, m1 = 0, sid2 = 0;
    Cand cd1{};
    int64_t roff1 = 0;
    auto to_item = [&](int sid, const Cand &cd, int m, int64_t roff) {
        XItem x;
        x.sid = sid;
        x.m = m;
        x.roff = roff;
        x.d0 = cd.center - XCENTER;
        x.strand = cd.strand;
        x.ref = cd.ref;
        x.reflen = ldc(&A.I.ref_len[cd.ref]);
// ... 569 lines not shown
        A.rec[r2] = o2;
        tally(A, T, o1, r1);
        tally(A, T, o2, r2);
    }
    if (T) {
        __syncthreads();
        tally_flush(A, T);
    }
}

static int64_t pool_words_for(int64_t n)
{
    return (n > 0 ? n : 1) * 8 + 4096 + 2 * (int64_t)DP_MAX_BLOCKS * DP_WAVES_PER_BLOCK * POOL_CHUNK;
}

static int ensure_map_buffers(Ctx &c)
{
    MapState &M = c.map;
    const int64_t n = c.reads.n;
    if (M.cap_reads < n || M.cand == nullptr) {
        hipFree(M.cand); hipFree(M.n_cand); hipFree(M.yf); hipFree(M.work);
        hipFree(M.rwork); hipFree(M.skey); hipFree(M.sinfo); hipFree(M.rec);
        const int64_t cap = n > 0 ? n : 1;
        MH_HIP(hipMalloc(&M.cand, sizeof(Cand) * cap * MAXCAND));
        MH_HIP(hipMalloc(&M.n_cand, sizeof(int32_t) * cap));
        MH_HIP(hipMalloc(&M.yf, sizeof(int32_t) * cap));
        MH_HIP(hipMalloc(&M.work, sizeof(int32_t) * cap * MAXCAND));
        MH_HIP(hipMalloc(&M.rwork, sizeof(int32_t) * (cap / 2 + 1)));
        MH_HIP(hipMalloc(&M.skey, sizeof(SlotKey) * cap * MAXCAND));
        MH_HIP(hipMalloc(&M.sinfo, sizeof(SlotInfo) * cap * MAXCAND));
        MH_HIP(hipMalloc(&M.rec, sizeof(Rec) * cap));
        M.cap_reads = cap;
    }
    if (M.counters == nullptr) MH_HIP(hipMalloc(&M.counters, sizeof(int32_t) * 8));
    if (M.cap_refs < c.index.n_refs || M.ref_stats == nullptr) {
        hipFree(M.ref_stats);
        const int cr = c.index.n_refs > 0 ? c.index.n_refs : 1;
        MH_HIP(hipMalloc(&M.ref_stats, sizeof(int64_t) * (5 * cr + 3)));
        M.cap_refs = cr;
    }
    if (M.pool_used == nullptr) MH_HIP(hipMalloc(&M.pool_used, sizeof(unsigned long long)));
    const int64_t test_cap = c.test_caps.cigar_pool_words;
    const int64_t need = test_cap > 0 ? test_cap : pool_words_for(n);
    if (need > (int64_t)INT32_MAX) {
        set_error("mh_map: %lld reads need a CIGAR pool past 2^31 words; map them in batches",
                  (long long)n);
        return -3;
    }
    if (M.pool == nullptr || (test_cap > 0 ? M.pool_cap != need : M.pool_cap < need)) {
        hipFree(M.pool);
        M.pool = nullptr;
        M.pool_cap = 0;
        MH_HIP(hipMalloc(&M.pool, sizeof(uint32_t) * need));
        M.pool_cap = need;
    }
    return 0;
}

__global__ void k_init_stats(int64_t *s, int n_refs)
{
    for (int i = blockIdx.x * blockDim.x + threadIdx.x; i < 5 * n_refs + 3; i += gridDim.x * blockDim.x)
        s[i] = ((i >= 3 * n_refs && i < 5 * n_refs) || i == 5 * n_refs + 2) ? INT64_MAX : 0;
}

__global__ void k_fix_first(int64_t *s, int n_refs)
{
    for (int i = blockIdx.x * blockDim.x + threadIdx.x; i < 2 * n_refs; i += gridDim.x * blockDim.x)
        if (s[3 * n_refs + i] == INT64_MAX) s[3 * n_refs + i] = -1;
    if (blockIdx.x == 0 && threadIdx.x == 0 && s[5 * n_refs + 2] == INT64_MAX) s[5 * n_refs + 2] = -1;
}

const int64_t *map_stats_host(Ctx &c)
{
    MapState &M = c.map;
    if (!M.stats_host_valid) {
        M.stats_host.resize(5 * (size_t)M.n_refs + 3);
        const size_t bytes = sizeof(int64_t) * M.stats_host.size();
        if (M.stats_pin_ready) {
            if (hipStreamSynchronize(c.stream) != hipSuccess) {
                set_error("map_stats_host: copy failed");
                return nullptr;
            }
            std::memcpy(M.stats_host.data(), M.stats_pin, bytes);
        } else if (hipMemcpyAsync(M.stats_host.data(), M.ref_stats, bytes, hipMemcpyDeviceToHost,
                                  c.stream) != hipSuccess ||
                   hipStreamSynchronize(c.stream) != hipSuccess) {
            set_error("map_stats_host: copy failed");
            return nullptr;
        }
        M.stats_host_valid = true;
    }
    return M.stats_host.data();
}

template <int LOCAL>
__global__ __launch_bounds__(64) void k_probe_ext(DpArgs A, const int32_t *items, int32_t *out, int n)
{
    extern __shared__ __attribute__((aligned(16))) unsigned char smem[];
    const int lane = threadIdx.x & 63;
    const int e = blockIdx.x;
    if (e >= n) return;
    uint32_t *bits = (uint32_t *)smem;
    unsigned char *xbase = smem + (size_t)32 * A.rows_pad;
    const XView X0 = xview(xbase, A.rows_pad, 0);
    const int gmin = A.oeI < A.oeD ? A.oeI : A.oeD;
    const int r = items[4 * e];
    XItem it;
    it.sid = 0;
    it.m = A.R.len[r];
    it.roff = A.R.off[r];
    it.strand = items[4 * e + 1];
    it.ref = items[4 * e + 2];
    it.d0 = items[4 * e + 3] - XCENTER;
    it.reflen = A.I.ref_len[it.ref];
    it.gref = A.I.ref_off[it.ref];
    it.hb = A.len_tab[3 * (MAXLEN + 1) + it.m];
    stage_ext<LOCAL>(A, it, X0, lane);
    wave_sync();
    int best = 0, bi = 0, bl = 0, low = -1;
// ... 16 lines not shown
    }
}

int run_probe_ext(Ctx &c, const mh_params &par, int n, const int32_t *items, int32_t *out)
{
    if (c.index.n_refs <= 0 || c.reads.n <= 0 || n < 0) { set_error("mh_probe_extend: no index / reads"); return -3; }
    if (par.mode != MH_E2E && par.mode != MH_LOCAL) { set_error("mh_probe_extend: bad mode"); return -3; }
    if (c.len_tab == nullptr || c.len_tab_key != len_tab_key(par)) { set_error("mh_probe_extend: length tables"); return -3; }
    for (int e = 0; e < n; ++e) {
        if (items[4 * e] < 0 || items[4 * e] >= c.reads.n || (items[4 * e + 1] & ~1) ||
            items[4 * e + 2] < 0 || items[4 * e + 2] >= c.index.n_refs) {
            set_error("mh_probe_extend: item %d out of range", e);
            return -3;
        }
    }
    if (n == 0) return 0;
    const int rows_pad = ((c.reads.max_len + 7) / 8) * 8;
    const int lds = 32 * rows_pad + 2 * xview_bytes(rows_pad);
    if (lds > 160 * 1024) { set_error("mh_probe_extend: reads too long"); return -3; }
    hipStream_t s = c.stream;
    int32_t *d_items = nullptr, *d_out = nullptr;
    MH_HIP(hipMalloc(&d_items, sizeof(int32_t) * 4 * (size_t)n));
    MH_HIP(hipMalloc(&d_out, sizeof(int32_t) * 8 * (size_t)n));
    MH_HIP(hipMemcpyAsync(d_items, items, sizeof(int32_t) * 4 * (size_t)n, hipMemcpyHostToDevice, s));
    DpArgs da{c.reads, c.index, c.len_tab, nullptr, nullptr, nullptr, nullptr, nullptr, nullptr,
              nullptr, nullptr, nullptr, 0, rows_pad, lds,
              par.rfg_open + par.rfg_ext, par.rfg_ext, par.rdg_open + par.rdg_ext, par.rdg_ext};
    const void *kf = par.mode == MH_LOCAL ? (const void *)k_probe_ext<1> : (const void *)k_probe_ext<0>;
    MH_HIP(hipFuncSetAttribute(kf, hipFuncAttributeMaxDynamicSharedMemorySize, 160 * 1024));
    if (par.mode == MH_LOCAL) hipLaunchKernelGGL((k_probe_ext<1>), dim3(n), dim3(64), lds, s, da, d_items, d_out, n);
    else hipLaunchKernelGGL((k_probe_ext<0>), dim3(n), dim3(64), lds, s, da, d_items, d_out, n);
    MH_HIP(hipGetLastError());
    MH_HIP(hipMemcpyAsync(out, d_out, sizeof(int32_t) * 8 * (size_t)n, hipMemcpyDeviceToHost, s));
    MH_HIP(hipStreamSynchronize(s));
    hipFree(d_items);
    hipFree(d_out);
    return 0;
}

int run_map(Ctx &c, const mh_params &par)
{
    c.map.stats_host_valid = false;
    c.map.stats_pin_ready = false;
    if (c.index.n_refs <= 0 || c.index.hent == nullptr) {
        set_error("mh_map: no reference index (call mh_index_build first)");
        return -3;
    }
    if (par.mode != MH_E2E && par.mode != MH_LOCAL) { set_error("mh_map: bad mode"); return -3; }
    const int SL = par.mode == MH_LOCAL ? 20 : 22;
    if (c.index.seedlen != SL) {
        set_error("mh_map: index seed length %d does not match mode (%d)", c.index.seedlen, SL);
        return -3;
    }
    if (c.len_tab == nullptr || c.len_tab_key != len_tab_key(par)) {
        set_error("mh_map: length tables not prepared");
        return -3;
    }
    if (int st = ensure_map_buffers(c)) return st;
    MapState &M = c.map;
    const int64_t n = c.reads.n;
    M.n_reads = n;
    M.n_refs = c.index.n_refs;
    M.par = par;
    hipStream_t s = c.stream;
    M.last_work = M.last_cigar = 0;
    if (n == 0) hipLaunchKernelGGL(k_init_stats, dim3(64), dim3(256), 0, s, M.ref_stats, M.n_refs);
    if (n > 0) {
        auto launch_seed = [&]() -> int {
            SeedArgs sa{c.reads, c.index, par.mode, c.len_tab, M.cand, M.n_cand, M.yf, M.work, M.counters, M.cap_reads};
            int64_t blocks = ((n + SEED_CHUNK - 1) / SEED_CHUNK + 3) / 4;
            if (blocks > 1 << 16) blocks = 1 << 16;
            const int pk = prof_begin(c, "k_seed");
            hipLaunchKernelGGL(k_seed, dim3((unsigned)blocks), dim3(256), 0, s, sa);
            prof_end(c, pk);
            MH_HIP(hipGetLastError());
            return 0;
        };

        const int rows_pad = ((c.reads.max_len + 7) / 8) * 8;
        const int wave_lds = 32 * rows_pad + 2 * xview_bytes(rows_pad) + raw_bytes(rows_pad);
        if (wave_lds > 160 * 1024) { set_error("mh_map: reads too long for LDS"); return -3; }
        int wpb = 1;
        for (int w = DP_WAVES_PER_BLOCK; w >= 1; --w)
            if ((160 * 1024 / (w * wave_lds)) * w > (160 * 1024 / (wpb * wave_lds)) * wpb ||
                ((160 * 1024 / (w * wave_lds)) * w == (160 * 1024 / (wpb * wave_lds)) * wpb && w > wpb))
                wpb = w;
        auto launch_dp = [&](const int32_t *work, const int32_t *count, int32_t *queue,
                             int64_t max_items, const char *name) -> int {
            DpArgs da{c.reads, c.index, c.len_tab, M.cand, work, count, M.skey, M.sinfo, M.pool,
                      M.pool_used, M.counters + 1, queue, M.pool_cap, rows_pad, wave_lds,
                      par.rfg_open + par.rfg_ext, par.rfg_ext, par.rdg_open + par.rdg_ext,
                      par.rdg_ext, M.cap_reads};
            const int round = rows_pad <= 256 ? 256 : rows_pad <= 320 ? 320 : 0;
            const void *kf =
                par.mode == MH_LOCAL
                    ? (round == 256 ? (const void *)k_dp<1, 256> : round ? (const void *)k_dp<1, 320> : (const void *)k_dp<1, 0>)
                    : (round == 256 ? (const void *)k_dp<0, 256> : round ? (const void *)k_dp<0, 320> : (const void *)k_dp<0, 0>);
            const auto okey = std::make_pair(kf, wpb * wave_lds);
            auto occ = M.dp_occ.find(okey);
// ... 3 lines not shown
                int nb = 0;
                MH_HIP(hipOccupancyMaxActiveBlocksPerMultiprocessor(&nb, kf, 64 * wpb, (size_t)wpb * wave_lds));
                occ = M.dp_occ.emplace(okey, nb).first;
            }
            const int per_cu = occ->second;
            int64_t dblocks = (int64_t)(c.n_cu > 0 ? c.n_cu : 256) * (per_cu > 0 ? per_cu : 1);
            const int64_t need = (max_items + (int64_t)wpb * DP_QUEUE_CHUNK - 1) / ((int64_t)wpb * DP_QUEUE_CHUNK);
            if (dblocks > need) dblocks = need;
            if (dblocks > DP_MAX_BLOCKS) dblocks = DP_MAX_BLOCKS;
            if (dblocks < 1) dblocks = 1;
            const int pd = prof_begin(c, name);
            const dim3 grid((unsigned)dblocks), block(64 * wpb);
            const size_t lds = (size_t)wpb * wave_lds;
            if (par.mode == MH_LOCAL) {
                if (round == 256) hipLaunchKernelGGL((k_dp<1, 256>), grid, block, lds, s, da);
                else if (round) hipLaunchKernelGGL((k_dp<1, 320>), grid, block, lds, s, da);
                else hipLaunchKernelGGL((k_dp<1, 0>), grid, block, lds, s, da);
            } else {
                if (round == 256) hipLaunchKernelGGL((k_dp<0, 256>), grid, block, lds, s, da);
                else if (round) hipLaunchKernelGGL((k_dp<0, 320>), grid, block, lds, s, da);
                else hipLaunchKernelGGL((k_dp<0, 0>), grid, block, lds, s, da);
            }
            prof_end(c, pd);
            MH_HIP(hipGetLastError());
            return 0;
        };
        const int64_t units = c.reads.paired ? n / 2 : n;
        PairArgs pa{c.reads, c.len_tab, M.skey, M.sinfo, M.n_cand, M.yf, M.pool, M.rec, M.ref_stats,
                    M.n_refs, par.mode == MH_LOCAL, par.maxins, c.reads.paired, M.cap_reads};
        int64_t pblocks = (units + 255) / 256;
        if (pblocks > 1 << 16) pblocks = 1 << 16;
        if (pblocks < 1) pblocks = 1;
        for (int attempt = 0; attempt < 2; ++attempt) {
            hipLaunchKernelGGL(k_init_stats, dim3(64), dim3(256), 0, s, M.ref_stats, M.n_refs);
            MH_HIP(hipMemsetAsync(M.counters, 0, sizeof(int32_t) * 8, s));
            MH_HIP(hipMemsetAsync(M.pool_used, 0, sizeof(unsigned long long), s));
            if (int st = launch_seed()) return st;
            if (int st = launch_dp(M.work, M.counters, M.counters + 5, n * 2, "k_dp")) return st;
            if (c.reads.paired && units > 0) {
                RescueArgs ra{c.reads, c.index, M.skey, M.n_cand, M.yf, M.cand, M.rwork,
                              M.counters + 4, par.maxins, M.cap_reads};
                int64_t rblocks = (units + 255) / 256;
                if (rblocks > 4096) rblocks = 4096;
                const int pr = prof_begin(c, "k_rescue");
                hipLaunchKernelGGL(k_rescue, dim3((unsigned)rblocks), dim3(256), 0, s, ra);
                prof_end(c, pr);
                MH_HIP(hipGetLastError());
                if (int st = launch_dp(M.rwork, M.counters + 4, M.counters + 6, units, "k_dp_rescue")) return st;
            }
            pa.pool = M.pool;
            const int pp = prof_begin(c, "k_pair");
            hipLaunchKernelGGL(k_pair, dim3((unsigned)pblocks), dim3(256), 0, s, pa);
            prof_end(c, pp);
            MH_HIP(hipGetLastError());
            int32_t ctr[5];
            unsigned long long used = 0;
            MH_HIP(hipMemcpyAsync(ctr, M.counters, sizeof(ctr), hipMemcpyDeviceToHost, s));
            MH_HIP(hipMemcpyAsync(&used, M.pool_used, sizeof(used), hipMemcpyDeviceToHost, s));
            MH_HIP(hipStreamSynchronize(s));
            M.last_work = ctr[0] + ctr[4];
            M.last_rescue = ctr[4];
            M.last_cigar = (int64_t)used;
            M.last_fast = ctr[3];
            if (!ctr[2]) break;
            if (attempt == 1) { set_error("mh_map: CIGAR pool overflow after a retry"); return -2; }
            ++c.retries[RETRY_CIGAR_POOL];
            hipFree(M.pool);
            M.pool = nullptr;
            M.pool_cap = 0;
            int64_t grown = (int64_t)used * 2 + pool_words_for(0);
            if (grown > (int64_t)INT32_MAX) grown = INT32_MAX;
            if ((int64_t)used > grown) {
                set_error("mh_map: CIGAR pool demand %llu words passes the int32 offsets",
                          (unsigned long long)used);
                return -2;
            }
            MH_HIP(hipMalloc(&M.pool, sizeof(uint32_t) * grown));
            M.pool_cap = grown;
        }
    }
    hipLaunchKernelGGL(k_fix_first, dim3(8), dim3(256), 0, s, M.ref_stats, M.n_refs);
    MH_HIP(hipGetLastError());
    {
        const size_t bytes = sizeof(int64_t) * (5 * (size_t)M.n_refs + 3);
        if (M.stats_pin_cap < bytes) {
            if (M.stats_pin) hipHostFree(M.stats_pin);
            M.stats_pin = nullptr;
            M.stats_pin_cap = 0;
            if (hipHostMalloc(&M.stats_pin, bytes, hipHostMallocDefault) == hipSuccess)
                M.stats_pin_cap = bytes;
            else
                M.stats_pin = nullptr;
        }
        if (M.stats_pin && hipMemcpyAsync(M.stats_pin, M.ref_stats, bytes, hipMemcpyDeviceToHost, s) == hipSuccess)
            M.stats_pin_ready = true;
    }
    M.valid = true;
    return 0;
}

}
```

### micall-lite_amd/csrc/mh_pileup.hip

```cpp
#include <cstring>

#include "mh_internal.h"

namespace mh {

constexpr int PU_INSBUF = 3 * 1024;
constexpr int PU_MAXINS = 2 * MH_MAXOPS;
constexpr int PU_LDS = 160 * 1024 - 64;
constexpr int PU_XCH = 5;
constexpr unsigned long long PILE_ERR_ROW = 1, PILE_ERR_INSBUF = 2;

struct RowV {
    int present, flag, ref, pos, n_cigar, rev, m;
    const uint32_t *cig;
    int64_t roff;
    uint32_t op0;
};

__device__ __forceinline__ void fetch_ops(RowV &v, int lane)
{
    v.op0 = 0;
    if (v.present && lane < v.n_cigar) v.op0 = v.cig[lane];
}

// ... 681 lines not shown
            const int ia = i0 + lane, ib = ia + 64;
            const char ma = merged(ia), mb = merged(ib);
            count(ia, ma);
            count(ib, mb);
        }
        mxp = wave_max_all(mxp);
        err = wave_max_all(err);
        if (lane == 0) {
            atomicAdd(&rl[ref].read_count, 1u);
            atomicMin(&rl[ref].first_unit, (long long)u);
            if (mxp > 0) atomicMax(&rl[ref].max_pos, mxp);
            if (err) atomicExch(&A.ev_ctr[3], PILE_ERR_ROW);
        }
        __builtin_amdgcn_wave_barrier();
    }
    __syncthreads();
    for (int r = 0; r < NR; ++r) {
        const int wo = wmap[2 * r], wl = wmap[2 * r + 1];
        if (wo < 0) continue;
        int32_t *dst = A.dense + (int64_t)r * A.cap * 4;
        for (int x = threadIdx.x; x < 4 * wl; x += blockDim.x) {
            const unsigned int v = (win[wo + ((x & 3) >> 1) * wl + (x >> 2)] >> (16 * (x & 1))) & 0xffffu;
            if (v) atomicAdd(&dst[x], (int)v);
        }
    }
    for (int r = threadIdx.x; r < NR; r += blockDim.x) {
        if (!rl[r].read_count) continue;
        atomicAdd(&A.read_counts[r], (unsigned long long)rl[r].read_count);
        atomicMin(&A.first_unit[r], rl[r].first_unit);
        if (rl[r].max_pos > 0) atomicMax(&A.max_pos[r], rl[r].max_pos);
    }
}

__global__ void k_pile_init(long long *first_unit, int32_t *max_pos, int n)
{
    for (int i = blockIdx.x * blockDim.x + threadIdx.x; i < n; i += gridDim.x * blockDim.x) {
        first_unit[i] = INT64_MAX;
        max_pos[i] = 0;
    }
}

__global__ void k_pile_fix(long long *first_unit, int n)
{
    for (int i = blockIdx.x * blockDim.x + threadIdx.x; i < n; i += gridDim.x * blockDim.x)
        if (first_unit[i] == INT64_MAX) first_unit[i] = -1;
}

static int ensure_pile(Ctx &c)
{
    PileState &P = c.pile;
    const int64_t cells = (int64_t)(P.n_refs > 0 ? P.n_refs : 1) * P.cap;
    if (P.alloc_cells < cells) {
        hipFree(P.dense); hipFree(P.nflag); hipFree(P.dflag);
        MH_HIP(hipMalloc(&P.dense, sizeof(int32_t) * 4 * cells));
        MH_HIP(hipMalloc(&P.nflag, cells));
        MH_HIP(hipMalloc(&P.dflag, cells));
        P.alloc_cells = cells;
    }
    if (P.alloc_refs < (P.n_refs > 0 ? P.n_refs : 1)) {
        hipFree(P.read_counts); hipFree(P.first_unit); hipFree(P.max_pos);
        const int nr = P.n_refs > 0 ? P.n_refs : 1;
        MH_HIP(hipMalloc(&P.read_counts, sizeof(int64_t) * nr));
        MH_HIP(hipMalloc(&P.first_unit, sizeof(int64_t) * nr));
        MH_HIP(hipMalloc(&P.max_pos, sizeof(int32_t) * nr));
        P.alloc_refs = nr;
    }
    if (!P.ev_counters) MH_HIP(hipMalloc(&P.ev_counters, sizeof(int64_t) * 4));
    const int64_t t_ev = c.test_caps.pile_events, t_pool = c.test_caps.pile_event_bytes;
    if (!P.ev || (t_ev > 0 && P.ev_cap != t_ev)) {
        hipFree(P.ev);
        P.ev = nullptr;
        P.ev_cap = t_ev > 0 ? t_ev : 1 << 16;
// ... 58 lines not shown
        g.win_map[2 * (size_t)r + 1] = want;
        words += 2 * (int64_t)want;
    }
    g.win_words = (int)words;
    const int64_t lds0 = (int64_t)base + 4 * words;
    const auto key = std::make_tuple(source, lds0, g.unit_bytes);
    auto hit = P.shapes.find(key);
    if (hit == P.shapes.end()) {
        if (!c.n_cu) MH_HIP(hipDeviceGetAttribute(&c.n_cu, hipDeviceAttributeMultiprocessorCount, c.device));
        const void *kern = source == 0 ? (const void *)k_pileup<0, false> : (const void *)k_pileup<1, false>;
        MH_HIP(hipFuncSetAttribute(kern, hipFuncAttributeMaxDynamicSharedMemorySize, PU_LDS));
        int best_w = 0, best_wpb = 1, best_nb = 1;
        for (int wpb = 16; wpb >= 1; --wpb) {
            const int64_t lds = lds0 + (int64_t)wpb * g.unit_bytes;
            if (lds > PU_LDS) continue;
            int nb = 0;
            MH_HIP(hipOccupancyMaxActiveBlocksPerMultiprocessor(&nb, kern, 64 * wpb, (size_t)lds));
            if (nb * wpb > best_w) { best_w = nb * wpb; best_wpb = wpb; best_nb = nb; }
        }
        hit = P.shapes.emplace(key, std::make_pair(best_wpb, best_nb > 0 ? best_nb : 1)).first;
    }
    g.wpb = hit->second.first;
    g.lds = (size_t)lds0 + (size_t)g.wpb * g.unit_bytes;
    g.blocks = (n_units + g.wpb - 1) / g.wpb;
    const int64_t n_cu = c.n_cu > 0 ? c.n_cu : 256;
    const int64_t max_blocks = words > 0 ? n_cu * hit->second.second : n_cu * 8;
    if (g.blocks > max_blocks) g.blocks = max_blocks;
    if (words > 0 && g.blocks < (n_units + PU_UNITS_PER_BLOCK - 1) / PU_UNITS_PER_BLOCK)
        g.blocks = (n_units + PU_UNITS_PER_BLOCK - 1) / PU_UNITS_PER_BLOCK;
    if (g.blocks < 1) g.blocks = 1;
    return 0;
}

int run_pileup(Ctx &c, int source, int q_cutoff)
{
    PileState &P = c.pile;
    ++P.gen;
    int64_t n_units;
    const DevReads *R;
    if (source == 0) {
        if (!c.map.valid) { set_error("mh_pileup: no mapping results"); return -3; }
        R = &c.reads;
        n_units = c.reads.paired ? c.reads.n / 2 : c.reads.n;
    } else {
        R = &c.rows.reads;
        n_units = c.rows.n_units;
    }
    if (int st = ensure_pile(c)) return st;
    hipStream_t s = c.stream;
    PileGeometry geo;
    if (int st = pile_geometry(c, source, n_units, geo)) return st;
    P.info.blocks = geo.blocks;
    P.info.wpb = geo.wpb;
    P.info.win_words = geo.win_words;
    P.info.n_units = n_units;
    P.info.win_map = geo.win_map;
    P.info.tok_insert_blocks = P.info.tok_count_blocks = P.info.tok_ne = P.info.tok_nd = 0;
    {
        const int64_t need = geo.blocks * geo.wpb * (int64_t)PU_INS_BYTES;
        if (P.ins_scratch_bytes < need) {
            hipFree(P.ins_scratch);
            P.ins_scratch = nullptr;
            MH_HIP(hipMalloc(&P.ins_scratch, need));
            P.ins_scratch_bytes = need;
        }
    }
    if (P.win_map_cap < 2 * P.n_refs || !P.win_map) {
        hipFree(P.win_map);
        P.win_map = nullptr;
        P.win_map_cap = 2 * (P.n_refs > 16 ? P.n_refs : 16);
        MH_HIP(hipMalloc(&P.win_map, sizeof(int32_t) * P.win_map_cap));
    }
    if (P.n_refs > 0)
        MH_HIP(hipMemcpyAsync(P.win_map, geo.win_map.data(), sizeof(int32_t) * 2 * P.n_refs,
                              hipMemcpyHostToDevice, s));
    const int64_t cells = (int64_t)P.n_refs * P.cap;
    for (int attempt = 0; attempt < 3; ++attempt) {
        MH_HIP(hipMemsetAsync(P.dense, 0, sizeof(int32_t) * 4 * (cells > 0 ? cells : 1), s));
        MH_HIP(hipMemsetAsync(P.nflag, 0, cells > 0 ? cells : 1, s));
        MH_HIP(hipMemsetAsync(P.dflag, 0, cells > 0 ? cells : 1, s));
        MH_HIP(hipMemsetAsync(P.read_counts, 0, sizeof(int64_t) * (P.n_refs > 0 ? P.n_refs : 1), s));
        MH_HIP(hipMemsetAsync(P.ev_counters, 0, sizeof(int64_t) * 4, s));
        hipLaunchKernelGGL(k_pile_init, dim3(8), dim3(256), 0, s, (long long *)P.first_unit,
                           P.max_pos, P.n_refs);
        PileArgs A{};
        A.rec = c.map.rec;
        A.pool = c.map.pool;
        A.R = *R;
        A.paired = source == 0 ? c.reads.paired : 0;
        A.flag = c.rows.flag; A.ref = c.rows.ref; A.pos = c.rows.pos; A.cig_off = c.rows.cig_off;
        A.n_cigar = c.rows.n_cigar; A.cigar = c.rows.cigar; A.units = c.rows.units;
        A.n_units = n_units;
        A.n_refs = P.n_refs;
        A.cap = P.cap;
        A.dense = P.dense; A.nflag = P.nflag; A.dflag = P.dflag;
        A.read_counts = (unsigned long long *)P.read_counts;
        A.first_unit = (long long *)P.first_unit;
        A.max_pos = P.max_pos;
        A.ev = P.ev; A.ev_pool = P.ev_pool; A.ev_cap = P.ev_cap; A.pool_cap = P.pool_cap;
        A.ev_ctr = (unsigned long long *)P.ev_counters;
        A.q_cutoff = q_cutoff;
        A.win_map = P.win_map;
        A.win_words = geo.win_words;
        A.span_cap = geo.span;
        A.unit_bytes = geo.unit_bytes;
        A.ins_scratch = P.ins_scratch;
        if (n_units > 0) {
            const int pk = prof_begin(c, "k_pileup");
            const bool skip = P.only.size() == (size_t)P.n_refs &&
                              std::find(P.only.begin(), P.only.end(), (uint8_t)0) != P.only.end();
            const void *kern = source == 0 ? (skip ? (const void *)k_pileup<0, true> : (const void *)k_pileup<0, false>)
                                           : (skip ? (const void *)k_pileup<1, true> : (const void *)k_pileup<1, false>);
            MH_HIP(hipFuncSetAttribute(kern, hipFuncAttributeMaxDynamicSharedMemorySize, (int)geo.lds));
            void *kargs[] = {&A};
            MH_HIP(hipLaunchKernel(kern, dim3((unsigned)geo.blocks), dim3(64 * geo.wpb), kargs, geo.lds, s));
            prof_end(c, pk);
            MH_HIP(hipGetLastError());
        }
        hipLaunchKernelGGL(k_pile_fix, dim3(8), dim3(256), 0, s, (long long *)P.first_unit, P.n_refs);
        int64_t ctr[4];
        MH_HIP(hipMemcpyAsync(ctr, P.ev_counters, sizeof(ctr), hipMemcpyDeviceToHost, s));
        MH_HIP(hipStreamSynchronize(s));
        if (ctr[3] == (int64_t)PILE_ERR_INSBUF) {
            set_error("mh_pileup: the merged insertions of one read pair exceed PU_INSBUF (%d bytes)",
                      PU_INSBUF);
            return -3;
        }
        if (ctr[3]) {
            set_error("mh_pileup: malformed alignment row (CIGAR/position)");
            return -3;
        }
        if (!ctr[2]) return 0;
        ++c.retries[RETRY_PILE_EVENTS];
        hipFree(P.ev); hipFree(P.ev_pool);
        P.ev = nullptr; P.ev_pool = nullptr;
        P.ev_cap = ctr[0] * 2 + 1024;
        P.pool_cap = ctr[1] * 2 + 4096;
        MH_HIP(hipMalloc(&P.ev, sizeof(int32_t) * 4 * P.ev_cap));
        MH_HIP(hipMalloc(&P.ev_pool, P.pool_cap));
    }
    set_error("mh_pileup: event buffer overflow");
    return -2;
}

__device__ __forceinline__ uint64_t token_hash(int32_t ref, int32_t pos, const char *b, int32_t len)
{
    uint64_t h = 1469598103934665603ull;
    for (int32_t x = 0; x < len; ++x) h = (h ^ (unsigned char)b[x]) * 1099511628211ull;
    h ^= ((uint64_t)(uint32_t)ref << 32) | (uint32_t)pos;
    h ^= h >> 33; h *= 0xff51afd7ed558ccdull; h ^= h >> 33;
    return h;
}

__device__ __forceinline__ bool same_event(const int32_t *ev, const char *pool, int64_t u, int32_t r,
                                           int32_t ps, int32_t of, int32_t ln)
{
    bool same = ev[4 * u] == r && ev[4 * u + 1] == ps && ev[4 * u + 3] == ln;
    for (int32_t x = 0; same && x < ln; ++x) same = pool[ev[4 * u + 2] + x] == pool[of + x];
    return same;
}

constexpr int TOK_LDS_SLOTS = 4096;
constexpr int TOK_LDS_PROBES = 32;
__global__ __launch_bounds__(1024) void k_tok_insert(const int32_t *ev, const char *pool, int64_t ne,
                                                     int32_t *slot, int32_t *used, int32_t *eslot,
                                                     int64_t mask)
{
    __shared__ int32_t lrep[TOK_LDS_SLOTS];
    __shared__ int32_t lglob[TOK_LDS_SLOTS];
    for (int x = threadIdx.x; x < TOK_LDS_SLOTS; x += blockDim.x) lrep[x] = 0;
    __syncthreads();
    const int64_t per = (ne + gridDim.x - 1) / gridDim.x;
    const int64_t a = (int64_t)blockIdx.x * per, b = a + per < ne ? a + per : ne;
    for (int64_t e0 = a; e0 < b; e0 += blockDim.x) {
        const int64_t e = e0 + threadIdx.x;
        const bool live = e < b;
        int32_t r = 0, ps = 0, of = 0, ln = 0;
        uint64_t h = 0;
        int li = -1;
        bool lead = false;
        if (live) {
            r = ev[4 * e]; ps = ev[4 * e + 1]; of = ev[4 * e + 2]; ln = ev[4 * e + 3];
            h = token_hash(r, ps, pool + of, ln);
            int x = (int)((h >> 40) & (TOK_LDS_SLOTS - 1));
            for (int p = 0; p < TOK_LDS_PROBES; ++p, x = (x + 1) & (TOK_LDS_SLOTS - 1)) {
                int32_t s = lrep[x];
                if (s == 0) {
                    s = atomicCAS(&lrep[x], 0, (int32_t)(e + 1));
                    if (s == 0) { li = x; lead = true; break; }
                }
                if (same_event(ev, pool, s - 1, r, ps, of, ln)) { li = x; break; }
            }
        }
        __syncthreads();
        if (live && (lead || li < 0)) {
            int64_t i = (int64_t)(h & (uint64_t)mask);
            for (;;) {
                int32_t s = slot[i];
                if (s == 0) {
                    s = atomicCAS(&slot[i], 0, (int32_t)(e + 1));
                    if (s == 0) {
                        used[1 + atomicAdd(&used[0], 1)] = (int32_t)i;
                        break;
                    }
                }
                if (same_event(ev, pool, s - 1, r, ps, of, ln)) break;
                i = (i + 1) & mask;
            }
            eslot[e] = (int32_t)i;
            if (lead) lglob[li] = (int32_t)i;
        }
        __syncthreads();
        if (live && !lead && li >= 0) eslot[e] = lglob[li];
    }
}

__global__ void k_tok_number(const int32_t *used, int32_t *slotid)
{
    const int nd = used[0];
    for (int d = blockIdx.x * blockDim.x + threadIdx.x; d < nd; d += gridDim.x * blockDim.x)
        slotid[used[1 + d]] = d;
}

constexpr int TOK_LDS_KEYS = 8192;
__global__ __launch_bounds__(1024) void k_tok_count(const int32_t *eslot, int64_t ne,
                                                    const int32_t *slotid, const int32_t *used,
                                                    uint32_t *cnt)
{
    __shared__ uint32_t hist[TOK_LDS_KEYS];
    const int nd = used[0];
    const bool lds = nd <= TOK_LDS_KEYS;
    if (lds)
        for (int d = threadIdx.x; d < nd; d += blockDim.x) hist[d] = 0;
    __syncthreads();
    const int64_t per = (ne + gridDim.x - 1) / gridDim.x;
    const int64_t a = (int64_t)blockIdx.x * per, b = a + per < ne ? a + per : ne;
    for (int64_t e = a + threadIdx.x; e < b; e += blockDim.x) {
        const int d = slotid[eslot[e]];
        if (lds) atomicAdd(&hist[d], 1u);
        else atomicAdd(&cnt[d], 1u);
    }
    __syncthreads();
    if (lds)
        for (int d = threadIdx.x; d < nd; d += blockDim.x)
            if (hist[d]) atomicAdd(&cnt[d], hist[d]);
}

__global__ void k_tok_gather(const int32_t *ev, const char *pool, const int32_t *slot,
                             const uint32_t *cnt, const int32_t *used, int32_t *meta,
                             char *bytes, int64_t bytes_cap, int32_t *overflow)
{
    const int lane = threadIdx.x;
    const int nd = used[0];
    int base = 0;
    for (int d0 = 0; d0 < nd; d0 += 64) {
        const int d = d0 + lane;
        int32_t ln = 0, u = 0, i = 0;
        if (d < nd) {
            i = used[1 + d];
            u = slot[i] - 1;
            ln = ev[4 * u + 3];
        }
        const int incl = wave_incl_scan(ln, lane);
        const int off = base + incl - ln;
        if (d < nd) {
            meta[5 * d] = ev[4 * u];
            meta[5 * d + 1] = ev[4 * u + 1];
            meta[5 * d + 2] = off;
            meta[5 * d + 3] = ln;
            meta[5 * d + 4] = (int32_t)cnt[d];
            if (off + ln <= bytes_cap) {
                for (int32_t x = 0; x < ln; ++x) bytes[off + x] = pool[ev[4 * u + 2] + x];
            } else {
                *overflow = 1;
            }
        }
        base += __builtin_amdgcn_readlane(incl, 63);
    }
}

int run_token_aggregate(Ctx &c, int64_t ne, int64_t pool_used, std::vector<int32_t> &meta,
                        std::string &bytes)
{
    PileState &P = c.pile;
    hipStream_t s = c.stream;
    meta.clear();
    bytes.clear();
    if (ne <= 0) return 0;
    int64_t cap = 1024;
    while (cap < 2 * ne) cap <<= 1;
    if (P.tok_cap < cap) {
        hipFree(P.tok_slot); hipFree(P.tok_cnt); hipFree(P.tok_used);
        P.tok_slot = nullptr; P.tok_cnt = nullptr; P.tok_used = nullptr; P.tok_cap = 0;
        MH_HIP(hipMalloc(&P.tok_slot, sizeof(int32_t) * 2 * cap + sizeof(int32_t) * (cap / 2 + 1)));
        MH_HIP(hipMalloc(&P.tok_cnt, sizeof(uint32_t) * cap));
        MH_HIP(hipMalloc(&P.tok_used, sizeof(int32_t) * (cap + 1)));
        P.tok_cap = cap;
    }
    if (P.tok_meta_cap < ne) {
        hipFree(P.tok_meta);
        P.tok_meta = nullptr;
        P.tok_meta_cap = 0;
        MH_HIP(hipMalloc(&P.tok_meta, sizeof(int32_t) * (5 * (size_t)ne + 1)));
        P.tok_meta_cap = ne;
    }
    int32_t *ovf = P.tok_meta + 5 * (size_t)P.tok_meta_cap;
    const int64_t want = c.test_caps.token_bytes > 0 ? c.test_caps.token_bytes
                                                     : std::max<int64_t>(pool_used, 64);
    if (P.tok_bytes_cap < want || (c.test_caps.token_bytes > 0 && P.tok_bytes_cap != want)) {
        hipFree(P.tok_bytes);
        P.tok_bytes = nullptr;
        P.tok_bytes_cap = 0;
        MH_HIP(hipMalloc(&P.tok_bytes, (size_t)want));
        P.tok_bytes_cap = want;
    }
    int32_t *slotid = P.tok_slot + cap, *eslot = P.tok_slot + 2 * cap;
    MH_HIP(hipMemsetAsync(P.tok_slot, 0, sizeof(int32_t) * cap, s));
    MH_HIP(hipMemsetAsync(P.tok_cnt, 0, sizeof(uint32_t) * cap, s));
    MH_HIP(hipMemsetAsync(P.tok_used, 0, sizeof(int32_t), s));
    int64_t blocks = (ne + 1023) / 1024;
    if (blocks > 256) blocks = 256;
    hipLaunchKernelGGL(k_tok_insert, dim3((unsigned)blocks), dim3(1024), 0, s, P.ev, P.ev_pool, ne,
                       P.tok_slot, P.tok_used, eslot, cap - 1);
    hipLaunchKernelGGL(k_tok_number, dim3(64), dim3(256), 0, s, P.tok_used, slotid);
    int64_t cblocks = (ne + 4095) / 4096;
    if (cblocks > 256) cblocks = 256;
    hipLaunchKernelGGL(k_tok_count, dim3((unsigned)cblocks), dim3(1024), 0, s, eslot, ne, slotid,
                       P.tok_used, P.tok_cnt);
    MH_HIP(hipGetLastError());
    const int64_t K = std::min<int64_t>(ne, 4096), B = std::min<int64_t>(P.tok_bytes_cap, 64 << 10);
    const size_t pin_need = 16 + 20 * (size_t)K + (size_t)B;
    if (P.tok_pin_cap < pin_need) {
        if (P.tok_pin) hipHostFree(P.tok_pin);
        P.tok_pin = nullptr;
        P.tok_pin_cap = 0;
        MH_HIP(hipHostMalloc((void **)&P.tok_pin, pin_need, hipHostMallocDefault));
        P.tok_pin_cap = pin_need;
    }
    for (int attempt = 0; attempt < 2; ++attempt) {
        MH_HIP(hipMemsetAsync(ovf, 0, sizeof(int32_t), s));
        hipLaunchKernelGGL(k_tok_gather, dim3(1), dim3(64), 0, s, P.ev, P.ev_pool, P.tok_slot,
                           P.tok_cnt, P.tok_used, P.tok_meta, P.tok_bytes, P.tok_bytes_cap, ovf);
        MH_HIP(hipGetLastError());
        MH_HIP(hipMemcpyAsync(P.tok_pin, P.tok_used, sizeof(int32_t), hipMemcpyDeviceToHost, s));
        MH_HIP(hipMemcpyAsync(P.tok_pin + 4, ovf, sizeof(int32_t), hipMemcpyDeviceToHost, s));
        MH_HIP(hipMemcpyAsync(P.tok_pin + 16, P.tok_meta, 20 * (size_t)K, hipMemcpyDeviceToHost, s));
        MH_HIP(hipMemcpyAsync(P.tok_pin + 16 + 20 * (size_t)K, P.tok_bytes, (size_t)B, hipMemcpyDeviceToHost, s));
        MH_HIP(hipStreamSynchronize(s));
        int32_t nd = 0, of = 0;
        std::memcpy(&nd, P.tok_pin, 4);
        std::memcpy(&of, P.tok_pin + 4, 4);
        P.info.tok_insert_blocks = blocks;
        P.info.tok_count_blocks = cblocks;
        P.info.tok_ne = ne;
        P.info.tok_nd = nd;
        if (nd <= 0) return 0;
        meta.resize(5 * (size_t)nd);
        std::memcpy(meta.data(), P.tok_pin + 16, 20 * (size_t)std::min<int64_t>(nd, K));
        if (nd > K)
            MH_HIP(copy_sync(c, meta.data() + 5 * (size_t)K, P.tok_meta + 5 * (size_t)K,
                             20 * (size_t)(nd - K), hipMemcpyDeviceToHost));
        const int64_t total = (int64_t)meta[5 * (size_t)(nd - 1) + 2] + meta[5 * (size_t)(nd - 1) + 3];
        if (!of) {
            bytes.resize((size_t)total);
            if (total > 0) std::memcpy(&bytes[0], P.tok_pin + 16 + 20 * (size_t)K, (size_t)std::min(total, B));
            if (total > B)
                MH_HIP(copy_sync(c, &bytes[(size_t)B], P.tok_bytes + B, (size_t)(total - B), hipMemcpyDeviceToHost));
            return 0;
        }
        ++c.retries[RETRY_TOKEN_BYTES];
        hipFree(P.tok_bytes);
        P.tok_bytes = nullptr;
        P.tok_bytes_cap = 0;
        MH_HIP(hipMalloc(&P.tok_bytes, (size_t)total));
        P.tok_bytes_cap = total;
    }
    set_error("mh_pileup_events: token gather overflow");
    return -2;
}

__global__ void k_pile_export(const int32_t *dense, const uint8_t *nflag, const uint8_t *dflag,
                              const int64_t *read_counts, const int64_t *first_unit,
                              const int32_t *max_pos, int32_t cap, int n_refs, const int32_t *sel,
                              int n_sel, int64_t unit_base, int32_t *sum, int32_t *mx,
                              uint8_t *flags)
{
    const int sidx = blockIdx.y;
    const int64_t stride = (int64_t)gridDim.x * blockDim.x;
    const int64_t t0 = (int64_t)blockIdx.x * blockDim.x + threadIdx.x;
    if (sidx < n_sel) {
        const int64_t src = (int64_t)sel[sidx] * cap, dst = (int64_t)sidx * cap;
        for (int64_t i = t0; i < 4 * (int64_t)cap; i += stride) sum[4 * dst + i] = dense[4 * src + i];
        for (int64_t i = t0; i < cap; i += stride) {
            flags[dst + i] = nflag[src + i];
            flags[(int64_t)n_sel * cap + dst + i] = dflag[src + i];
        }
    }
    if (sidx == 0) {
        for (int64_t i = t0; i < n_refs; i += stride) {
            sum[4 * (int64_t)n_sel * cap + i] = (int32_t)read_counts[i];
            mx[i] = max_pos[i];
            mx[n_refs + i] = first_unit[i] < 0 ? INT32_MIN : (int32_t)(-(first_unit[i] + unit_base));
        }
    }
}

__global__ void k_pile_import(int32_t *dense, uint8_t *nflag, uint8_t *dflag, int64_t *read_counts,
                              int64_t *first_unit, int32_t *max_pos, int32_t cap, int n_refs,
                              const int32_t *sel, int n_sel, const int32_t *sum, const int32_t *mx,
                              const uint8_t *flags)
{
// ... 60 lines not shown
}

static int upload_sel(Ctx &c, int n_sel, const int32_t *sel, int32_t **dsel)
{
    PileState &P = c.pile;
    for (int i = 0; i < n_sel; ++i)
        if (sel[i] < 0 || sel[i] >= P.n_refs) { set_error("pileup exchange: ref %d out of range", sel[i]); return -3; }
    if (P.sel_cap < n_sel || !P.sel) {
        hipFree(P.sel);
        P.sel = nullptr;
        P.sel_cap = n_sel > 64 ? n_sel : 64;
        MH_HIP(hipMalloc(&P.sel, sizeof(int32_t) * P.sel_cap));
    }
    if (n_sel) MH_HIP(copy_sync(c, P.sel, sel, sizeof(int32_t) * n_sel, hipMemcpyHostToDevice));
    *dsel = P.sel;
    return 0;
}

extern "C" int mh_pileup_export(mh_ctx *ctx, int n_sel, const int32_t *sel, int64_t unit_base,
                                void *dev_sum, void *dev_max, void *dev_flags)
{
    if (!ctx || !dev_sum || !dev_max || (n_sel > 0 && (!sel || !dev_flags))) return -3;
    Ctx &c = *reinterpret_cast<Ctx *>(ctx);
    PileState &P = c.pile;
    if (!P.dense) { set_error("no pileup to export"); return -3; }
    MH_HIP(hipSetDevice(c.device));
    int32_t *dsel = nullptr;
    if (int st = upload_sel(c, n_sel, sel, &dsel)) return st;
    hipLaunchKernelGGL(k_pile_export, dim3(64, n_sel > 0 ? n_sel : 1), dim3(256), 0, c.stream,
                       P.dense, P.nflag, P.dflag, P.read_counts, P.first_unit, P.max_pos, P.cap,
                       P.n_refs, n_sel > 0 ? dsel : nullptr, n_sel, unit_base, (int32_t *)dev_sum,
                       (int32_t *)dev_max, (uint8_t *)dev_flags);
    MH_HIP(hipGetLastError());
    MH_HIP(hipStreamSynchronize(c.stream));
    return 0;
}

extern "C" int mh_pileup_import(mh_ctx *ctx, int n_sel, const int32_t *sel, const void *dev_sum,
                                const void *dev_max, const void *dev_flags)
{
    if (!ctx || !dev_sum || !dev_max || (n_sel > 0 && (!sel || !dev_flags))) return -3;
    Ctx &c = *reinterpret_cast<Ctx *>(ctx);
    PileState &P = c.pile;
    if (!P.dense) { set_error("no pileup to import into"); return -3; }
    MH_HIP(hipSetDevice(c.device));
    P.land_ok = false;
    int32_t *dsel = nullptr;
    if (int st = upload_sel(c, n_sel, sel, &dsel)) return st;
    hipLaunchKernelGGL(k_pile_import, dim3(64, n_sel > 0 ? n_sel : 1), dim3(256), 0, c.stream,
                       P.dense, P.nflag, P.dflag, P.read_counts, P.first_unit, P.max_pos, P.cap,
                       P.n_refs, n_sel > 0 ? dsel : nullptr, n_sel, (const int32_t *)dev_sum,
                       (const int32_t *)dev_max, (const uint8_t *)dev_flags);
    MH_HIP(hipGetLastError());
    MH_HIP(hipStreamSynchronize(c.stream));
    return 0;
}

namespace mh {

__global__ void k_ev_rebase(int32_t *ev, int64_t first, int64_t n, int32_t pool_base)
{
    for (int64_t e = (int64_t)blockIdx.x * blockDim.x + threadIdx.x; e < n;
         e += (int64_t)gridDim.x * blockDim.x)
        ev[4 * (first + e) + 2] += pool_base;
}

}

extern "C" int mh_pileup_event_bytes(mh_ctx *ctx, int64_t *n_events, int64_t *pool_bytes)
{
    if (!ctx) return -3;
    Ctx &c = *reinterpret_cast<Ctx *>(ctx);
    PileState &P = c.pile;
    int64_t ctr[4] = {0, 0, 0, 0};
    MH_HIP(hipSetDevice(c.device));
    if (P.ev_counters) MH_HIP(copy_sync(c, ctr, P.ev_counters, sizeof(ctr), hipMemcpyDeviceToHost));
    if (n_events) *n_events = ctr[0];
    if (pool_bytes) *pool_bytes = ctr[1];
    return 0;
}

extern "C" int mh_pileup_events_export(mh_ctx *ctx, void *dev_events, void *dev_pool)
{
    if (!ctx) return -3;
    Ctx &c = *reinterpret_cast<Ctx *>(ctx);
    PileState &P = c.pile;
    int64_t n = 0, bytes = 0;
    if (int st = mh_pileup_event_bytes(ctx, &n, &bytes)) return st;
    if ((n > 0 && !dev_events) || (bytes > 0 && !dev_pool)) return -3;
    if (n > 0) MH_HIP(hipMemcpyAsync(dev_events, P.ev, sizeof(int32_t) * 4 * n,
                                     hipMemcpyDeviceToDevice, c.stream));
    if (bytes > 0) MH_HIP(hipMemcpyAsync(dev_pool, P.ev_pool, bytes, hipMemcpyDeviceToDevice, c.stream));
    MH_HIP(hipStreamSynchronize(c.stream));
    return 0;
}

extern "C" int mh_pileup_events_import(mh_ctx *ctx, int parts, const int64_t *n_events,
                                       const int64_t *pool_bytes, const void *dev_events,
                                       int64_t events_stride, const void *dev_pool,
                                       int64_t pool_stride)
{
    if (!ctx || parts < 0 || (parts > 0 && (!n_events || !pool_bytes))) return -3;
    Ctx &c = *reinterpret_cast<Ctx *>(ctx);
    PileState &P = c.pile;
    int64_t tot_n = 0, tot_b = 0;
    for (int p = 0; p < parts; ++p) {
        if (n_events[p] < 0 || pool_bytes[p] < 0 || 4 * n_events[p] > events_stride ||
            pool_bytes[p] > pool_stride) { set_error("mh_pileup_events_import: bad part %d", p); return -3; }
        tot_n += n_events[p];
        tot_b += pool_bytes[p];
    }
    if ((tot_n > 0 && !dev_events) || (tot_b > 0 && !dev_pool)) return -3;
    if (tot_b >= INT32_MAX) { set_error("mh_pileup_events_import: pool too large"); return -2; }
    MH_HIP(hipSetDevice(c.device));
    if (P.ev_cap < tot_n || !P.ev) {
        hipFree(P.ev);
        P.ev_cap = tot_n * 2 + 1024;
        MH_HIP(hipMalloc(&P.ev, sizeof(int32_t) * 4 * P.ev_cap));
    }
    if (P.pool_cap < tot_b || !P.ev_pool) {
        hipFree(P.ev_pool);
        P.pool_cap = tot_b * 2 + 4096;
        MH_HIP(hipMalloc(&P.ev_pool, P.pool_cap));
    }
    if (!P.ev_counters) MH_HIP(hipMalloc(&P.ev_counters, sizeof(int64_t) * 4));
    int64_t at_n = 0, at_b = 0;
    for (int p = 0; p < parts; ++p) {
        const int32_t *src_e = (const int32_t *)dev_events + (size_t)p * events_stride;
        const char *src_b = (const char *)dev_pool + (size_t)p * pool_stride;
        if (n_events[p] > 0) {
            MH_HIP(hipMemcpyAsync(P.ev + 4 * at_n, src_e, sizeof(int32_t) * 4 * n_events[p],
                                  hipMemcpyDeviceToDevice, c.stream));
            if (at_b > 0) {
                int64_t blocks = (n_events[p] + 255) / 256;
                if (blocks > 4096) blocks = 4096;
                hipLaunchKernelGGL(k_ev_rebase, dim3((unsigned)blocks), dim3(256), 0, c.stream,
                                   P.ev, at_n, n_events[p], (int32_t)at_b);
                MH_HIP(hipGetLastError());
            }
        }
        if (pool_bytes[p] > 0)
            MH_HIP(hipMemcpyAsync(P.ev_pool + at_b, src_b, pool_bytes[p], hipMemcpyDeviceToDevice,
                                  c.stream));
        at_n += n_events[p];
        at_b += pool_bytes[p];
    }
    const int64_t ctr[4] = {tot_n, tot_b, 0, 0};
    MH_HIP(hipMemcpyAsync(P.ev_counters, ctr, sizeof(ctr), hipMemcpyHostToDevice, c.stream));
    MH_HIP(hipStreamSynchronize(c.stream));
    ++P.gen;
    P.land_ok = false;
    return 0;
}
```

### micall-lite_amd/csrc/mh_sam2aln.hip

```cpp
#include <fcntl.h>
#include <sys/mman.h>
#include <sys/stat.h>
#include <unistd.h>

#include <algorithm>
#include <cerrno>
#include <chrono>
#include <cstring>
#include <string>
#include <thread>
#include <vector>

#include "mh_gunzip.h"
#include "mh_sam2aln.h"

namespace mh {

static void s2a_free_device(S2AState &S)
{
    hipFree(S.d_seq); hipFree(S.d_qual); hipFree(S.d_out); hipFree(S.d_gather);
    hipFree(S.d_soff); hipFree(S.d_units); hipFree(S.d_slot); hipFree(S.d_goff);
    hipFree(S.d_pos); hipFree(S.d_cigoff); hipFree(S.d_ncig);
    hipFree(S.d_uref); hipFree(S.d_res); hipFree(S.d_tcnt); hipFree(S.d_trep);
    hipFree(S.d_uniq); hipFree(S.d_ctr); hipFree(S.d_cig); hipFree(S.d_h); hipFree(S.d_tkey);
// ... 593 lines not shown
    S2AArgs a{dev ? dev->seq : S.d_seq, dev ? dev->qual : S.d_qual, dev ? dev->soff : S.d_soff,
              dev ? dev->pos : S.d_pos, dev ? dev->cig_off : S.d_cigoff,
              dev ? dev->n_cig : S.d_ncig, dev ? dev->cig : S.d_cig, S.d_units, S.d_uref,
              S.d_slot, nm, nc, {}, max_prop_n, span_cap, ops_cap,
              wave_bytes, S.d_out, S.d_res, S.d_h, S.d_ctr};
    for (int k = 0; k < nc; ++k) a.cut[k] = (unsigned char)(S.q_cutoffs[k] + 33);
    int64_t blocks = (nm + wpb - 1) / wpb;
    if (blocks > 256 * 64) blocks = 256 * 64;
    void (*merge)(S2AArgs) = nc == 1 ? k_s2a_merge<1> : nc == 2 ? k_s2a_merge<2>
                             : nc <= 4 ? k_s2a_merge<4> : k_s2a_merge<8>;
    MH_HIP(hipFuncSetAttribute((const void *)merge,
                               hipFuncAttributeMaxDynamicSharedMemorySize, wpb * wave_bytes));
    const int p0 = prof_begin(c, "k_s2a_merge");
    hipLaunchKernelGGL(merge, dim3((unsigned)blocks), dim3(64 * wpb), wpb * wave_bytes, s, a);
    prof_end(c, p0);
    MH_HIP(hipGetLastError());
    int64_t tb = (ne + 255) / 256;
    if (tb > 65536) tb = 65536;
    const int p1 = prof_begin(c, "k_s2a_group");
    hipLaunchKernelGGL(k_s2a_count, dim3((unsigned)tb), dim3(256), 0, s, S.d_res, S.d_h, ne,
                       S.d_tkey, S.d_tcnt, S.d_trep, tsize - 1);
    int64_t vb = (ne + 3) / 4;
    if (vb > 256 * 64) vb = 256 * 64;
    hipLaunchKernelGGL(k_s2a_verify, dim3((unsigned)vb), dim3(256), 0, s, S.d_res, S.d_h, S.d_uref,
                       S.d_slot, S.d_out, ne, nc, S.d_tkey, S.d_trep, tsize - 1, S.d_ctr);
    int64_t cb = (int64_t)((tsize + 255) / 256);
    if (cb > 65536) cb = 65536;
    hipLaunchKernelGGL(k_s2a_compact, dim3((unsigned)cb), dim3(256), 0, s, S.d_tkey, S.d_tcnt,
                       S.d_trep, tsize, S.d_uniq, S.d_ctr);
    prof_end(c, p1);
    MH_HIP(hipGetLastError());
    int32_t ctr[4];
    MH_HIP(hipMemcpyAsync(ctr, S.d_ctr, sizeof(ctr), hipMemcpyDeviceToHost, s));
    MH_HIP(hipStreamSynchronize(s));
    if (ctr[0]) {
        set_error("sam2aln: merged-sequence hash collision (distinct sequences share a key)");
        return -4;
    }
    S.n_unique = ctr[1];
    S.res.resize(4 * ne);
    S.uniq.resize(2 * (size_t)S.n_unique);
    MH_HIP(hipMemcpyAsync(S.res.data(), S.d_res, sizeof(int32_t) * 4 * ne, hipMemcpyDeviceToHost, s));
    if (S.n_unique)
        MH_HIP(hipMemcpyAsync(S.uniq.data(), S.d_uniq, sizeof(int32_t) * 2 * S.n_unique,
                              hipMemcpyDeviceToHost, s));
    MH_HIP(hipStreamSynchronize(s));
    for (int64_t e = 0; e < ne; ++e)
        if (S.res[4 * e] == S2A_EMPTY) {
            set_error("sam2aln: merged sequence of unit %lld is all gaps (float division by zero)",
                      (long long)(e / nc));
            return -3;
        }
    S.uniq_off.resize(S.n_unique + 1);
    int64_t g = 0;
    for (int64_t k = 0; k < S.n_unique; ++k) {
        S.uniq_off[k] = g;
        g += S.res[4 * (int64_t)S.uniq[2 * k] + 2];
    }
    S.uniq_off[S.n_unique] = g;
    S.gathered.resize((size_t)g);
    if (S.n_unique && g) {
        if (int st = s2a_upload(S, S.d_goff, S.uniq_off, s)) return st;
        if (int st = dev_reserve(S, S.d_gather, (size_t)g)) return st;
        int64_t gb = (S.n_unique + 3) / 4;
        if (gb > 256 * 64) gb = 256 * 64;
        hipLaunchKernelGGL(k_s2a_gather, dim3((unsigned)gb), dim3(256), 0, s, S.d_uniq, S.d_goff,
                           S.d_res, S.d_slot, S.d_out, S.n_unique, S.d_gather);
        MH_HIP(hipGetLastError());
        MH_HIP(hipMemcpyAsync(&S.gathered[0], S.d_gather, (size_t)g, hipMemcpyDeviceToHost, s));
        MH_HIP(hipStreamSynchronize(s));
    }
    prof_flush(c);
    return 0;
}

}

using namespace mh;

static int s2a_check_cutoffs(int n_cut, const int32_t *q_cutoffs)
{
    if (n_cut < 1 || n_cut > S2A_MAX_CUTS || !q_cutoffs) {
        set_error("sam2aln: %d q-cutoffs (1..%d are supported)", n_cut, S2A_MAX_CUTS);
        return -3;
    }
    for (int k = 0; k < n_cut; ++k) {
        if (q_cutoffs[k] < 0 || q_cutoffs[k] > 93) {
            set_error("sam2aln: q-cutoff %d outside 0..93", (int)q_cutoffs[k]);
            return -3;
        }
        for (int j = 0; j < k; ++j)
            if (q_cutoffs[j] == q_cutoffs[k]) {
                set_error("sam2aln: q-cutoff %d given twice", (int)q_cutoffs[k]);
                return -3;
            }
    }
    return 0;
}

extern "C" int mh_sam2aln_csv_q(mh_ctx *ctx, const char *text, int64_t len, int n_cut,
                                const int32_t *q_cutoffs, double max_prop_n, int64_t *n_units)
{
    if (!ctx || (!text && len) || len < 0) return -3;
// ... 46 lines not shown
    S.staged_reads = -1;
    if (int st = dev_reserve(S, S.d_seq, (size_t)R.total_bases + 64)) return st;
    if (int st = dev_reserve(S, S.d_qual, (size_t)R.total_bases + 64)) return st;
    if (int st = dev_reserve(S, S.d_pos, rows)) return st;
    if (int st = dev_reserve(S, S.d_cigoff, rows)) return st;
    if (int st = dev_reserve(S, S.d_ncig, rows)) return st;
    if (int st = dev_reserve(S, S.d_flag, rows)) return st;
    if (int st = dev_reserve(S, S.d_samref, rows)) return st;
    if (int st = dev_reserve(S, S.d_spanins, rows)) return st;
    S.n_rows = n;
    S.pos.resize(n); S.cig_off.resize(n); S.n_cig.resize(n); S.flag.resize(n);
    sam_ref.resize(n); span_ins.resize(n);
    const int64_t used = c.map.last_cigar < c.map.pool_cap ? c.map.last_cigar : c.map.pool_cap;
    S.cig.resize(used > 0 ? (size_t)used : 0);
    if (n == 0) return 0;
    StageArgs a{R, c.map.rec, c.map.pool, S.d_seq, S.d_qual, S.d_pos, S.d_cigoff, S.d_ncig,
                S.d_flag, S.d_samref, S.d_spanins};
    int64_t blocks = (n + 15) / 16;
    if (blocks > (1 << 20)) blocks = 1 << 20;
    const int p0 = prof_begin(c, "k_s2a_stage");
    hipLaunchKernelGGL(k_s2a_stage, dim3((unsigned)blocks), dim3(256), 0, s, a);
    prof_end(c, p0);
    MH_HIP(hipGetLastError());
    const size_t nb = sizeof(int32_t) * (size_t)n;
    MH_HIP(hipMemcpyAsync(S.pos.data(), S.d_pos, nb, hipMemcpyDeviceToHost, s));
    MH_HIP(hipMemcpyAsync(S.cig_off.data(), S.d_cigoff, nb, hipMemcpyDeviceToHost, s));
    MH_HIP(hipMemcpyAsync(S.n_cig.data(), S.d_ncig, nb, hipMemcpyDeviceToHost, s));
    MH_HIP(hipMemcpyAsync(S.flag.data(), S.d_flag, nb, hipMemcpyDeviceToHost, s));
    MH_HIP(hipMemcpyAsync(sam_ref.data(), S.d_samref, nb, hipMemcpyDeviceToHost, s));
    MH_HIP(hipMemcpyAsync(span_ins.data(), S.d_spanins, nb, hipMemcpyDeviceToHost, s));
    if (used > 0)
        MH_HIP(hipMemcpyAsync(S.cig.data(), c.map.pool, sizeof(uint32_t) * (size_t)used,
                              hipMemcpyDeviceToHost, s));
    MH_HIP(hipStreamSynchronize(s));
    S.staged_reads = n;
    return 0;
}

extern "C" int mh_sam2aln_resident(mh_ctx *ctx, int n_refs, const char *const *refnames, int n_cut,
                                   const int32_t *q_cutoffs, double max_prop_n, int64_t *n_units)
{
    if (!ctx || n_refs < 0 || (n_refs > 0 && !refnames)) return -3;
    if (int st = s2a_check_cutoffs(n_cut, q_cutoffs)) return st;
    Ctx &c = *ctx_of(ctx);
    MH_HIP(hipSetDevice(c.device));
    if (!c.map.valid || c.map.n_reads != c.reads.n) {
        set_error("mh_sam2aln_resident: no mapping pass is resident (call mh_map)");
        return -3;
    }
    if ((int64_t)c.names.size() != c.reads.n) {
        set_error("mh_sam2aln_resident: no read names are resident");
        return -3;
    }
    if (n_refs != c.map.n_refs) {
        set_error("mh_sam2aln_resident: %d reference names for a pass over %d references", n_refs,
                  c.map.n_refs);
        return -3;
    }
    if (!c.s2a) c.s2a = new S2AState();
    S2AState &S = *c.s2a;
    S.q_cutoffs.assign(q_cutoffs, q_cutoffs + n_cut);
    s2a_begin(c, S);
    S.u1.clear();
    std::vector<int32_t> sam_ref, span_ins;
    int st = 0;
    const auto t0 = std::chrono::steady_clock::now();
    auto t1 = t0, t2 = t0;
// ... 212 lines not shown
```

### micall-lite_amd/micall_amd/_native.py

```python
import ctypes
import os

import numpy as np

HERE = os.path.dirname(os.path.abspath(__file__))
LIB_PATH = os.environ.get('MICALL_HIP_LIB', os.path.join(HERE, 'libmicall_hip.so'))

E2E, LOCAL = 0, 1
MAXOPS = 128
INT32_MIN = -2 ** 31
OP_CHARS = 'MIDxS'
PILEUP_SLACK = 2048


class NativeUnavailable(RuntimeError):
    pass


class NativeError(RuntimeError):
    pass


class Params(ctypes.Structure):
    _fields_ = [('mode', ctypes.c_int), ('rdg_open', ctypes.c_int), ('rdg_ext', ctypes.c_int),
# ... 22 lines not shown
    sig = {
        'mh_version': ([], ctypes.c_int),
        'mh_last_error': ([ctypes.c_char_p, ctypes.c_size_t], ctypes.c_int),
        'mh_device_count': ([ctypes.POINTER(ctypes.c_int)], ctypes.c_int),
        'mh_ctx_create': ([ctypes.c_int, ctypes.POINTER(_P)], ctypes.c_int),
        'mh_ctx_destroy': ([_P], ctypes.c_int),
        'mh_ctx_sync': ([_P], ctypes.c_int),
        'mh_ctx_stream': ([_P, ctypes.POINTER(_P)], ctypes.c_int),
        'mh_index_build': ([_P, ctypes.c_int, ctypes.POINTER(ctypes.c_char_p), ctypes.c_int], ctypes.c_int),
        'mh_reads_load': ([_P, ctypes.c_int64, ctypes.c_int, _P, _P, _P, _P], ctypes.c_int),
        'mh_reads_load_fastq': ([_P, ctypes.c_char_p, ctypes.c_char_p, _I64P], ctypes.c_int),
        'mh_reads_load_fastq_part': ([_P, ctypes.c_char_p, ctypes.c_char_p, ctypes.c_int,
                                      ctypes.c_int, _I64P, _I64P], ctypes.c_int),
        'mh_reads_count': ([_P, _I64P, ctypes.POINTER(ctypes.c_int)], ctypes.c_int),
        'mh_reads_set_names': ([_P, ctypes.c_int64, ctypes.POINTER(ctypes.c_char_p)], ctypes.c_int),
        'mh_map': ([_P, ctypes.POINTER(Params)], ctypes.c_int),
        'mh_probe_extend': ([_P, ctypes.POINTER(Params), ctypes.c_int, _P, _P], ctypes.c_int),
        'mh_conseqs_build': ([ctypes.c_int, _P, _P, _P, _P, ctypes.c_int32, _P, _P, _P, ctypes.c_int64,
                              _P, _P, _P, _P, _P, ctypes.c_char_p, _P, ctypes.c_int64, _P, _P],
                             ctypes.c_int),
        'mh_top_tokens': ([ctypes.c_int32, ctypes.c_int32, _P, _P, _P, ctypes.c_char_p, ctypes.c_int32, _P,
                           _P], ctypes.c_int),
        'mh_alns_fetch': ([_P, ctypes.c_int64, ctypes.c_int64, _P], ctypes.c_int),
        'mh_map_counts': ([_P, _P, _P, _P, _P, _P, _I64P, _I64P, _I64P], ctypes.c_int),
        'mh_map_stats': ([_P, _P], ctypes.c_int),
        'mh_recs_fetch_fields': ([_P, ctypes.c_int64, ctypes.c_int64, ctypes.c_int, ctypes.c_int, _P],
                                 ctypes.c_int),
        'mh_recs_fetch': ([_P, ctypes.c_int64, ctypes.c_int64, _P], ctypes.c_int),
        'mh_test_set_capacities': ([_P, ctypes.c_int64, ctypes.c_int64, ctypes.c_int64,
                                    ctypes.c_int64], ctypes.c_int),
        'mh_test_pileup_info': ([_P, _P, ctypes.c_int, _P], ctypes.c_int),
        'mh_test_force_index_collision': ([_P, ctypes.c_int], ctypes.c_int),
        'mh_retry_counts': ([_P, _P], ctypes.c_int),
        'mh_test_set_gotoh_wait': ([_P, ctypes.c_int64], ctypes.c_int),
        'mh_format_rows': ([_P, ctypes.c_int, _P, ctypes.c_int64, ctypes.c_int64,
                            ctypes.POINTER(ctypes.c_char_p), _P, ctypes.c_size_t,
                            ctypes.POINTER(ctypes.c_size_t)], ctypes.c_int),
        'mh_write_rows_crc': ([_P, ctypes.c_int, _P, ctypes.c_int64, ctypes.c_int64,
                               ctypes.POINTER(ctypes.c_char_p), ctypes.c_int, ctypes.c_int64, _I64P,
                               ctypes.POINTER(ctypes.c_uint32)], ctypes.c_int),
        'mh_rows_load': ([_P, ctypes.c_int64, _P, _P, _P, _P, _P, _P, _P, _P, _P, _P,
                          ctypes.c_int64, _P], ctypes.c_int),
        'mh_rows_load_csv': ([_P, ctypes.c_char_p, ctypes.c_int64, ctypes.c_int,
                              ctypes.POINTER(ctypes.c_char_p), _I64P, _I64P, _I32P], ctypes.c_int),
        'mh_rows_info': ([_P, _P, _P, ctypes.c_char_p, ctypes.c_size_t], ctypes.c_int),
        'mh_reads_fastq_lines': ([_P, _I64P], ctypes.c_int),
        'mh_pileup': ([_P, ctypes.c_int, ctypes.c_int, ctypes.c_int, _P], ctypes.c_int),
        'mh_pileup_only': ([_P, ctypes.c_int, ctypes.c_int, ctypes.c_int, _P, ctypes.c_int, _P], ctypes.c_int),
        'mh_pileup_dims': ([_P, ctypes.POINTER(ctypes.c_int), _I32P, _I64P, _I64P], ctypes.c_int),
        'mh_pileup_fetch': ([_P, _P, _P, _P, _P, _P, _P], ctypes.c_int),
        'mh_pileup_fetch_refs': ([_P, ctypes.c_int, _P, _P, _P, _P], ctypes.c_int),
        'mh_pileup_events': ([_P, _P, _P, _P, _P, _P, _P], ctypes.c_int),
        'mh_pileup_exchange_bytes': ([_P, ctypes.c_int, _I64P, _I64P, _I64P], ctypes.c_int),
        'mh_pileup_export': ([_P, ctypes.c_int, _P, ctypes.c_int64, _P, _P, _P], ctypes.c_int),
        'mh_pileup_import': ([_P, ctypes.c_int, _P, _P, _P, _P], ctypes.c_int),
        'mh_gotoh_align': ([_P, ctypes.c_char_p, ctypes.c_char_p, ctypes.c_int, ctypes.c_int,
                            ctypes.c_int, ctypes.c_char_p, _P, ctypes.c_char_p, ctypes.c_char_p,
                            ctypes.c_int, ctypes.POINTER(ctypes.c_int)], ctypes.c_int),
        'mh_levenshtein': ([ctypes.c_char_p, ctypes.c_char_p], ctypes.c_int),
        'mh_gotoh_align_batch': ([_P, ctypes.c_int, _P, _P, ctypes.c_int, ctypes.c_int,
                                  ctypes.c_int, ctypes.c_char_p, _P, _P, _P, _P, _P, _P],
                                 ctypes.c_int),
        'mh_gotoh_distance_batch': ([_P, ctypes.c_int, _P, _P, _P, ctypes.c_int, ctypes.c_int,
                                     ctypes.c_int, ctypes.c_char_p, _P, _P, _P, _P], ctypes.c_int),
        'mh_levenshtein_batch': ([ctypes.c_int, _P, _P, _P], ctypes.c_int),
        'mh_pileup_event_bytes': ([_P, _P, _P], ctypes.c_int),
# ... 769 lines not shown
        out = np.zeros(5, dtype=np.int64)
        check(lib().mh_map_stats(self.h, _ptr(out)), 'mh_map_stats')
        return tuple(int(x) for x in out)

    def probe_extend(self, par, items):
        items = np.ascontiguousarray(items, dtype=np.int32).reshape(-1, 4)
        out = np.zeros((max(len(items), 1), 8), dtype=np.int32)
        check(lib().mh_probe_extend(self.h, ctypes.byref(par), len(items), _ptr(items), _ptr(out)),
              'mh_probe_extend')
        return out[:len(items)]

    def test_set_capacities(self, cigar_pool_words=0, pileup_events=0, pileup_event_bytes=0,
                            token_bytes=0):
        check(lib().mh_test_set_capacities(self.h, cigar_pool_words, pileup_events,
                                           pileup_event_bytes, token_bytes),
              'mh_test_set_capacities')
        self.map_serial += 1

    def test_pileup_info(self):
        n = ctypes.c_int()
        check(lib().mh_pileup_dims(self.h, ctypes.byref(n), None, None, None), 'mh_pileup_dims')
        return pileup_info(self.h, n.value)

    def test_force_index_collision(self, on=True):
        check(lib().mh_test_force_index_collision(self.h, int(bool(on))),
              'mh_test_force_index_collision')

    def retry_counts(self):
        out = np.zeros(4, dtype=np.int64)
        check(lib().mh_retry_counts(self.h, _ptr(out)), 'mh_retry_counts')
        return dict(cigar_pool=int(out[0]), pileup_events=int(out[1]), token_bytes=int(out[2]),
                    gotoh_wait=int(out[3]))

    def test_set_gotoh_wait(self, ticks):
        check(lib().mh_test_set_gotoh_wait(self.h, int(ticks)), 'mh_test_set_gotoh_wait')

    def recs(self, first=0, n=None):
        if n is None:
            n = self.reads_count()[0] - first
        out = np.zeros((max(n, 1), 20), dtype=np.int32)
        check(lib().mh_recs_fetch(self.h, first, n, _ptr(out)), 'mh_recs_fetch')
        return out[:n]

    def rec_fields(self, names, first=0, n=None):
        if n is None:
            n = self.reads_count()[0] - first
        idx = [ALN_FIELDS.index(k) for k in names]
        if idx != list(range(idx[0], idx[0] + len(idx))):
            raise ValueError('rec_fields: columns must be adjacent')
        out = np.empty((max(n, 1), len(idx)), dtype=np.int32)
        check(lib().mh_recs_fetch_fields(self.h, first, n, idx[0], len(idx), _ptr(out)),
              'mh_recs_fetch_fields')
        return out[:n]

    def format_rows(self, style, first=0, n=None, order=None):
        return bytes(self.format_rows_bytes(style, first, n, order)).decode()

    def write_rows(self, out, style, first=0, n=None, order=None):
        fd = _plain_fd(out)
        if fd is not None:
            out.flush()
            off = os.lseek(fd, 0, os.SEEK_CUR)
            written, _ = self.write_rows_at(fd, off, style, order, first, n)
            out.seek(off + written)
            return
        text = self.format_rows_bytes(style, first, n, order)
# ... 404 lines not shown
```

Baseline: 64.85 million reads/s.

## Cut host-device syncs by landing pileup rows and token tables behind pileup

Result: no change. 65.56 million reads/s, median of 4 (+1.1%).

```diff
diff --git a/include/micall_hip.h b/include/micall_hip.h
--- a/include/micall_hip.h
+++ b/include/micall_hip.h
@@ -77,6 +77,7 @@
 int mh_test_pileup_info(mh_ctx *ctx, int64_t *out16, int n_refs, int32_t *win_len);
 int mh_test_force_index_collision(mh_ctx *ctx, int on);
 int mh_retry_counts(mh_ctx *ctx, int64_t *out4);
+int mh_test_wait_count(mh_ctx *ctx, int64_t *n);
 int mh_test_set_gotoh_wait(mh_ctx *ctx, int64_t ticks);
 int mh_recs_fetch(mh_ctx *ctx, int64_t first, int64_t n, int32_t *out20);
 int mh_recs_fetch_fields(mh_ctx *ctx, int64_t first, int64_t n, int field0, int nfields, int32_t *out);
diff --git a/micall-lite_amd/csrc/mh_a2c.hip b/micall-lite_amd/csrc/mh_a2c.hip
--- a/micall-lite_amd/csrc/mh_a2c.hip
+++ b/micall-lite_amd/csrc/mh_a2c.hip
@@ -754,7 +754,7 @@
         MH_HIP(hipMemcpyAsync(S.h_first.data(), S.d_first, sizeof(uint32_t) * cells,
                               hipMemcpyDeviceToHost, s));
     }
-    MH_HIP(hipStreamSynchronize(s));
+    MH_HIP(stream_wait(c));
     prof_flush(c);
     return 0;
 }
@@ -1009,7 +1009,7 @@
         MH_HIP(hipGetLastError());
         std::vector<int32_t> ncod(3 * (size_t)ng + 1);
         MH_HIP(hipMemcpyAsync(ncod.data(), S.d_ncod, sizeof(int32_t) * ncod.size(), hipMemcpyDeviceToHost, s));
-        MH_HIP(hipStreamSynchronize(s));
+        MH_HIP(stream_wait(c));
         prof_flush(c);
         if (ncod[3 * (size_t)ng]) return 1;
         S.t_parse = ms_since(t0);
@@ -1043,7 +1043,7 @@
                               hipMemcpyDeviceToHost, s));
         MH_HIP(hipMemcpyAsync(S.d_bcur, S.d_bstart, sizeof(unsigned long long) * (nb + 1),
                               hipMemcpyDeviceToDevice, s));
-        MH_HIP(hipStreamSynchronize(s));
+        MH_HIP(stream_wait(c));
         std::vector<A2CChunk> chunks;
         for (int64_t g = 0; g < ng; ++g)
             for (int64_t bin = S.g_bin0[(size_t)g]; bin < S.g_bin0[(size_t)g + 1]; ++bin)
@@ -1277,7 +1277,7 @@
     }
     e = hipGetLastError();
     if (e == hipSuccess) e = hipMemcpyAsync(ctr, d_ctr, sizeof(ctr), hipMemcpyDeviceToHost, s);
-    if (e == hipSuccess) e = hipStreamSynchronize(s);
+    if (e == hipSuccess) e = stream_wait(c);
     if (e != hipSuccess) { fail(e, "k_a2c_ins_hash"); goto done; }
     if (ctr[0] == 0) goto done;
     while (tsize < 2 * ctr[0]) tsize <<= 1;
@@ -1305,7 +1305,7 @@
     }
     e = hipGetLastError();
     if (e == hipSuccess) e = hipMemcpyAsync(ctr, d_ctr, sizeof(ctr), hipMemcpyDeviceToHost, s);
-    if (e == hipSuccess) e = hipStreamSynchronize(s);
+    if (e == hipSuccess) e = stream_wait(c);
     if (e != hipSuccess) { fail(e, "k_a2c_ins"); goto done; }
     if (ctr[1]) {
         set_error("aln2counts: insertion-string hash collision (distinct strings share a key)");
@@ -1332,7 +1332,7 @@
                        a, d_sorted, d_eoff, (int64_t)ent.size(), d_out);
     e = hipGetLastError();
     if (e == hipSuccess) e = hipMemcpyAsync(&S.aminos[0], d_out, (size_t)eoff.back(), hipMemcpyDeviceToHost, s);
-    if (e == hipSuccess) e = hipStreamSynchronize(s);
+    if (e == hipSuccess) e = stream_wait(c);
     if (e != hipSuccess) { fail(e, "k_a2c_ins_gather"); goto done; }
     S.entries = std::move(ent);
     if (n_entries) *n_entries = (int64_t)S.entries.size();
diff --git a/micall-lite_amd/csrc/mh_api.cpp b/micall-lite_amd/csrc/mh_api.cpp
--- a/micall-lite_amd/csrc/mh_api.cpp
+++ b/micall-lite_amd/csrc/mh_api.cpp
@@ -56,7 +56,13 @@
 hipError_t copy_sync(Ctx &c, void *dst, const void *src, size_t bytes, hipMemcpyKind kind)
 {
     hipError_t e = hipMemcpyAsync(dst, src, bytes, kind, c.stream);
-    return e == hipSuccess ? hipStreamSynchronize(c.stream) : e;
+    return e == hipSuccess ? stream_wait(c) : e;
+}
+
+hipError_t stream_wait(Ctx &c)
+{
+    ++c.waits;
+    return hipStreamSynchronize(c.stream);
 }
 
 int prof_begin(Ctx &c, const char *name)
@@ -79,6 +85,7 @@
 {
     for (auto &p : c.prof_pending) {
         float ms = 0.f;
+        if (hipEventQuery(p.b) != hipSuccess) ++c.waits;
         if (hipEventSynchronize(p.b) == hipSuccess && hipEventElapsedTime(&ms, p.a, p.b) == hipSuccess) {
             ProfEntry &e = c.prof_acc[p.name];
             e.ms += ms;
@@ -281,7 +288,7 @@
     return mix64(h, (uint64_t)n);
 }
 
-static int build_index(DevIndex &ix, int n_refs, const char *const *seqs, int seedlen)
+static int build_index(Ctx &c, DevIndex &ix, int n_refs, const char *const *seqs, int seedlen)
 {
     static const bool trace = getenv("MH_INDEX_TRACE") && *getenv("MH_INDEX_TRACE") == '1';
     const auto tb = std::chrono::steady_clock::now();
@@ -417,6 +424,7 @@
     ix.code2 = (uint32_t *)(d + at[5]);
     ix.ncode = (uint32_t *)(d + at[6]);
     ix.cplane = (uint32_t *)(d + at[7]);
+    ++c.waits;
     MH_HIP(hipMemcpy(ix.blob, stage.data(), total, hipMemcpyHostToDevice));
     mark("upload");
     return 0;
@@ -443,7 +451,7 @@
         off[r] = total;
         total += ((int64_t)lens[r] + 31) / 32 * 32;
     }
-    MH_HIP(hipStreamSynchronize(c.stream));
+    MH_HIP(stream_wait(c));
     dst.n = n;
     dst.paired = paired;
     dst.max_len = max_len;
@@ -465,7 +473,7 @@
         MH_HIP(hipMemcpyAsync(c.stage_qual, qual, src_total, hipMemcpyHostToDevice, c.stream));
         MH_HIP(hipMemcpyAsync(c.stage_off, offsets, sizeof(int64_t) * n, hipMemcpyHostToDevice, c.stream));
         MH_HIP(launch_pack_reads(dst, c.stage_seq, c.stage_qual, c.stage_off, c.stream));
-        MH_HIP(hipStreamSynchronize(c.stream));
+        MH_HIP(stream_wait(c));
     }
     if (adopt) {
         host = std::move(*adopt);
@@ -692,7 +700,7 @@
     if (!ctx) return 0;
     CtxEx *c = X(ctx);
     hipSetDevice(c->device);
-    hipStreamSynchronize(c->stream);
+    stream_wait(*c);
     free_reads(c->reads);
     free_reads(c->rows.reads);
     hipFree(c->stage_seq); hipFree(c->stage_qual); hipFree(c->stage_off);
@@ -700,7 +708,7 @@
     free_index(c->small);
     MapState &M = c->map;
     hipFree(M.cand); hipFree(M.n_cand); hipFree(M.yf); hipFree(M.work); hipFree(M.rwork); hipFree(M.skey); hipFree(M.sinfo);
-    hipFree(M.pool); hipFree(M.pool_used); hipFree(M.rec); hipFree(M.counters); hipFree(M.ref_stats);
+    hipFree(M.pool); hipFree(M.rec); hipFree(M.ctl);
     if (M.stats_pin) hipHostFree(M.stats_pin);
     M.stats_pin = nullptr;
     M.stats_pin_cap = 0;
@@ -719,6 +727,12 @@
     if (P.tok_pin) hipHostFree(P.tok_pin);
     P.tok_pin = nullptr;
     P.tok_pin_cap = 0;
+    if (P.row_pin) hipHostFree(P.row_pin);
+    P.row_pin = nullptr;
+    P.row_pin_cap = 0;
+    if (P.win_pin) hipHostFree(P.win_pin);
+    P.win_pin = nullptr;
+    P.win_pin_cap = 0;
     P.land_cap = 0;
     P.land_ok = false;
     hipFree(P.ins_scratch);
@@ -738,7 +752,7 @@
 {
     if (!ctx) return -3;
     MH_HIP(hipSetDevice(X(ctx)->device));
-    MH_HIP(hipStreamSynchronize(X(ctx)->stream));
+    MH_HIP(stream_wait(*X(ctx)));
     return 0;
 }
 
@@ -757,7 +771,7 @@
     }
     CtxEx *c = X(ctx);
     MH_HIP(hipSetDevice(c->device));
-    MH_HIP(hipStreamSynchronize(c->stream));
+    MH_HIP(stream_wait(*c));
     int64_t total = 0;
     for (int r = 0; r < n_refs; ++r) total += (int64_t)std::strlen(seqs[r]);
     const uint64_t sig = c->force_index_collision ? 0x5eedull : signature(n_refs, seqs, seedlen);
@@ -780,13 +794,13 @@
         }
     }
     if (!cacheable) {
-        if (int st = build_index(c->small, n_refs, seqs, seedlen)) return st;
+        if (int st = build_index(*c, c->small, n_refs, seqs, seedlen)) return st;
         c->small.sig = sig;
         c->index = c->small;
         return 0;
     }
     DevIndex ix;
-    if (int st = build_index(ix, n_refs, seqs, seedlen)) { free_index(ix); return st; }
+    if (int st = build_index(*c, ix, n_refs, seqs, seedlen)) { free_index(ix); return st; }
     ix.sig = sig;
     if (c->cache.size() >= 2) {
         free_index(c->cache.front());
@@ -1102,7 +1116,6 @@
     MH_HIP(hipSetDevice(c->device));
     if (int st = prepare_len_tab(*c, *par)) return st;
     int st = run_map(*c, *par);
-    if (st == 0) MH_HIP(hipStreamSynchronize(c->stream));
     prof_flush(*c);
     c->rec_cache.clear();
     ++c->map_gen;
@@ -1228,7 +1241,7 @@
     }
     CtxEx *c = X(ctx);
     MH_HIP(hipSetDevice(c->device));
-    MH_HIP(hipStreamSynchronize(c->stream));
+    MH_HIP(stream_wait(*c));
     MapState &M = c->map;
     PileState &P = c->pile;
     hipFree(M.pool); M.pool = nullptr; M.pool_cap = 0;
@@ -1251,6 +1264,13 @@
     return 0;
 }
 
+int mh_test_wait_count(mh_ctx *ctx, int64_t *n)
+{
+    if (!ctx || !n) return -3;
+    *n = X(ctx)->waits;
+    return 0;
+}
+
 int mh_test_set_gotoh_wait(mh_ctx *ctx, int64_t ticks)
 {
     if (!ctx || ticks < 0) { set_error("mh_test_set_gotoh_wait: bad arguments"); return -3; }
@@ -1269,7 +1289,7 @@
     if (n == 0) return 0;
     MH_HIP(hipMemcpy2DAsync(out20, sizeof(int32_t) * 20, M.rec + first, sizeof(Rec), sizeof(int32_t) * 20,
                             (size_t)n, hipMemcpyDeviceToHost, c->stream));
-    MH_HIP(hipStreamSynchronize(c->stream));
+    MH_HIP(stream_wait(*c));
     return 0;
 }
 
@@ -1284,7 +1304,7 @@
     if (n == 0) return 0;
     MH_HIP(hipMemcpy2DAsync(out, sizeof(int32_t) * nfields, (const int32_t *)(M.rec + first) + field0, sizeof(Rec),
                             sizeof(int32_t) * nfields, (size_t)n, hipMemcpyDeviceToHost, c->stream));
-    MH_HIP(hipStreamSynchronize(c->stream));
+    MH_HIP(stream_wait(*c));
     return 0;
 }
 
@@ -2274,20 +2294,6 @@
     return 0;
 }
 
-struct Landing {
-    int64_t *read_counts, *first_unit;
-    int32_t *max_pos;
-    int64_t *ev_counters;
-    size_t bytes;
-};
-
-static Landing landing_of(const PileState &P)
-{
-    const size_t nr = (size_t)P.n_refs, ev_at = (20 * nr + 7) & ~(size_t)7;
-    return Landing{(int64_t *)P.land, (int64_t *)(P.land + 8 * nr), (int32_t *)(P.land + 16 * nr),
-                   (int64_t *)(P.land + ev_at), 20 * nr + 64};
-}
-
 int mh_pileup(mh_ctx *ctx, int source, int q_cutoff, int n_refs, const int32_t *ref_lens)
 {
     return mh_pileup_only(ctx, source, q_cutoff, n_refs, ref_lens, -1, nullptr);
@@ -2316,27 +2322,6 @@
     c->pile.ref_lens.assign(ref_lens, ref_lens + n_refs);
     c->pile.land_ok = false;
     int st = run_pileup(*c, source, q_cutoff);
-    if (st == 0) {
-        PileState &P = c->pile;
-        const size_t nr = (size_t)P.n_refs, need = landing_of(P).bytes;
-        if (P.land_cap < need) {
-            if (P.land) hipHostFree(P.land);
-            P.land = nullptr;
-            P.land_cap = 0;
-            if (hipHostMalloc((void **)&P.land, need, hipHostMallocDefault) == hipSuccess) P.land_cap = need;
-            else P.land = nullptr;
-        }
-        if (P.land && P.read_counts && P.first_unit && P.max_pos) {
-            const Landing L = landing_of(P);
-            bool ok = hipMemcpyAsync(L.read_counts, P.read_counts, 8 * nr, hipMemcpyDeviceToHost, c->stream) == hipSuccess &&
-                      hipMemcpyAsync(L.first_unit, P.first_unit, 8 * nr, hipMemcpyDeviceToHost, c->stream) == hipSuccess &&
-                      hipMemcpyAsync(L.max_pos, P.max_pos, 4 * nr, hipMemcpyDeviceToHost, c->stream) == hipSuccess;
-            if (ok && P.ev_counters)
-                ok = hipMemcpyAsync(L.ev_counters, P.ev_counters, 32, hipMemcpyDeviceToHost, c->stream) == hipSuccess;
-            P.land_ok = ok;
-        }
-        MH_HIP(hipStreamSynchronize(c->stream));
-    }
     prof_flush(*c);
     return st;
 }
@@ -2429,7 +2414,7 @@
                                   c.stream));
         at += (parts[i].bytes + 255) & ~(size_t)255;
     }
-    MH_HIP(hipStreamSynchronize(c.stream));
+    MH_HIP(stream_wait(c));
     at = 0;
     for (int i = 0; i < n; ++i) {
         if (!parts[i].dst) continue;
@@ -2477,11 +2462,33 @@
         std::memcpy(mx.data(), landing_of(P).max_pos, sizeof(int32_t) * (size_t)P.n_refs);
     else
         MH_HIP(copy_sync(*c, mx.data(), P.max_pos, sizeof(int32_t) * (size_t)P.n_refs, hipMemcpyDeviceToHost));
+    for (int k = 0; k < n_sel; ++k)
+        if (refs[k] < 0 || refs[k] >= P.n_refs) { set_error("mh_pileup_fetch_refs: ref %d out of range", refs[k]); return -3; }
+    bool landed = P.row_land_gen == P.gen && P.land_ok && P.row_pin &&
+                  P.row_land_at.size() == (size_t)P.n_refs;
+    for (int k = 0; k < n_sel && landed; ++k) {
+        const size_t r = (size_t)refs[k];
+        const int64_t rows = std::min<int64_t>(P.cap, std::max(mx[r], 0));
+        landed = rows == 0 || (P.row_land_at[r] >= 0 && rows <= P.row_land_rows[r]);
+    }
+    if (landed) {
+        for (int k = 0; k < n_sel; ++k) {
+            const size_t r = (size_t)refs[k];
+            const size_t rows = (size_t)std::min<int64_t>(P.cap, std::max(mx[r], 0));
+            if (rows == 0) continue;
+            const size_t lr = (size_t)P.row_land_rows[r];
+            const char *src = P.row_pin + P.row_land_at[r];
+            const int64_t base = (int64_t)r * P.cap;
+            std::memcpy(dense + 4 * base, src, 16 * rows);
+            std::memcpy(nflag + base, src + 16 * lr, rows);
+            std::memcpy(dflag + base, src + 17 * lr, rows);
+        }
+        return 0;
+    }
     std::vector<FetchPart> parts;
     parts.reserve(3 * (size_t)n_sel);
     for (int k = 0; k < n_sel; ++k) {
         const int r = refs[k];
-        if (r < 0 || r >= P.n_refs) { set_error("mh_pileup_fetch_refs: ref %d out of range", r); return -3; }
         const int64_t rows = std::min<int64_t>(P.cap, std::max(mx[(size_t)r], 0));
         if (rows == 0) continue;
         const int64_t base = (int64_t)r * P.cap;
diff --git a/micall-lite_amd/csrc/mh_censor.hip b/micall-lite_amd/csrc/mh_censor.hip
--- a/micall-lite_amd/csrc/mh_censor.hip
+++ b/micall-lite_amd/csrc/mh_censor.hip
@@ -285,7 +285,7 @@
     H(hipMemcpyAsync(C.text.data(), D.d_text, C.text.size(), hipMemcpyDeviceToHost, s), "D2H");
     H(hipMemcpyAsync(C.keep.data(), D.d_keep, 8 * nr, hipMemcpyDeviceToHost, s), "D2H");
     H(hipMemcpyAsync(sums, D.d_sums, 16, hipMemcpyDeviceToHost, s), "D2H");
-    H(hipStreamSynchronize(s), "sync");
+    H(stream_wait(c), "sync");
     if (st) return st;
     prof_flush(c);
     C.score_sum = (long long)sums[0];
diff --git a/micall-lite_amd/csrc/mh_gotoh.hip b/micall-lite_amd/csrc/mh_gotoh.hip
--- a/micall-lite_amd/csrc/mh_gotoh.hip
+++ b/micall-lite_amd/csrc/mh_gotoh.hip
@@ -1104,10 +1104,11 @@
     } else if (e == hipSuccess) {
         e = hipMemcpyAsync(oimg.get(), d + off_out, oo[count], hipMemcpyDeviceToHost, st);
     }
-    if (e == hipSuccess) e = hipStreamSynchronize(st);
+    if (e == hipSuccess) e = stream_wait(c);
     if (e != hipSuccess) return hip_fail(e, "k_gotoh");
     if (S.stamps) {
         std::vector<unsigned long long> h((size_t)4 * strips * S.stamp_blocks);
+        ++c.waits;
         MH_HIP(hipMemcpy(h.data(), S.stamps, h.size() * sizeof(h[0]), hipMemcpyDeviceToHost));
         MH_HIP(hipFree(S.stamps));
         if (FILE *f = fopen(stamp_path, "wb")) {
diff --git a/micall-lite_amd/csrc/mh_internal.h b/micall-lite_amd/csrc/mh_internal.h
--- a/micall-lite_amd/csrc/mh_internal.h
+++ b/micall-lite_amd/csrc/mh_internal.h
@@ -108,6 +108,8 @@
     const uint32_t u = (uint32_t)sid;
     return (int64_t)(u % MAXCAND) * plane + (int64_t)(u / MAXCAND);
 }
+
+constexpr int MAP_CTL_WORDS = 5;
 
 struct MapState {
     int64_t n_reads = 0;
@@ -126,6 +128,7 @@
     Rec *rec = nullptr;
     int32_t *counters = nullptr;
     int64_t *ref_stats = nullptr;
+    int64_t *ctl = nullptr;
     int64_t cap_reads = 0;
     int cap_refs = 0;
     int64_t last_work = 0;
@@ -172,6 +175,17 @@
     char *land = nullptr;
     size_t land_cap = 0;
     bool land_ok = false;
+    int64_t tok_land_gen = -1;
+    int64_t tok_land_keys = 0, tok_land_bytes = 0;
+    int64_t tok_want_keys = 4096, tok_want_bytes = 64 << 10;
+    bool attr_set[4] = {false, false, false, false};
+    char *row_pin = nullptr;
+    size_t row_pin_cap = 0;
+    int64_t row_land_gen = -1;
+    std::vector<int64_t> row_land_at;
+    std::vector<int32_t> row_land_rows;
+    int32_t *win_pin = nullptr;
+    int win_pin_cap = 0;
     std::vector<int32_t> ref_lens;
     std::vector<uint8_t> only;
     int32_t *sel = nullptr;
@@ -198,6 +212,22 @@
     } info;
 };
 
+constexpr size_t PILE_ROWS_LAND_MAX = (size_t)1 << 20;
+
+struct Landing {
+    int64_t *read_counts, *first_unit;
+    int32_t *max_pos;
+    int64_t *ev_counters;
+    size_t bytes;
+};
+
+inline Landing landing_of(const PileState &P)
+{
+    const size_t nr = (size_t)P.n_refs, ev_at = (20 * nr + 7) & ~(size_t)7;
+    return Landing{(int64_t *)P.land, (int64_t *)(P.land + 8 * nr), (int32_t *)(P.land + 16 * nr),
+                   (int64_t *)(P.land + ev_at), 20 * nr + 64};
+}
+
 hipError_t launch_pack_reads(DevReads &r, const uint8_t *d_seq, const uint8_t *d_qual,
                              const int64_t *d_src_off, hipStream_t s);
 int run_map(struct Ctx &c, const mh_params &par);
@@ -268,6 +298,7 @@
     TestCaps test_caps;
     int64_t retries[RETRY_KINDS] = {0, 0, 0, 0};
     int n_cu = 0;
+    int64_t waits = 0;
     bool prof = false;
     std::map<std::string, ProfEntry> prof_acc;
     std::vector<ProfPending> prof_pending;
@@ -302,6 +333,7 @@
 void prof_flush(Ctx &c);
 int hip_fail(hipError_t e, const char *what);
 hipError_t copy_sync(Ctx &c, void *dst, const void *src, size_t bytes, hipMemcpyKind kind);
+hipError_t stream_wait(Ctx &c);
 
 }
 
diff --git a/micall-lite_amd/csrc/mh_map.hip b/micall-lite_amd/csrc/mh_map.hip
--- a/micall-lite_amd/csrc/mh_map.hip
+++ b/micall-lite_amd/csrc/mh_map.hip
@@ -1645,6 +1645,7 @@
     const XView X0 = xview(xbase, A.rows_pad, 0), X1 = xview(xbase, A.rows_pad, 1);
     unsigned char *raw = xbase + 2 * xview_bytes(A.rows_pad);
     const int n_work = A.counters[0];
+    if (n_work == 0) return;
     const int gmin = A.oeI < A.oeD ? A.oeI : A.oeD;
 
     int64_t ck_base = 0;
@@ -2280,14 +2281,28 @@
         MH_HIP(hipMalloc(&M.rec, sizeof(Rec) * cap));
         M.cap_reads = cap;
     }
-    if (M.counters == nullptr) MH_HIP(hipMalloc(&M.counters, sizeof(int32_t) * 8));
-    if (M.cap_refs < c.index.n_refs || M.ref_stats == nullptr) {
-        hipFree(M.ref_stats);
+    if (M.cap_refs < c.index.n_refs || M.ctl == nullptr) {
+        hipFree(M.ctl);
+        M.ctl = nullptr;
+        M.counters = nullptr; M.pool_used = nullptr; M.ref_stats = nullptr;
+        M.cap_refs = 0;
         const int cr = c.index.n_refs > 0 ? c.index.n_refs : 1;
-        MH_HIP(hipMalloc(&M.ref_stats, sizeof(int64_t) * (5 * cr + 3)));
+        MH_HIP(hipMalloc(&M.ctl, sizeof(int64_t) * (MAP_CTL_WORDS + 5 * (size_t)cr + 3)));
+        M.counters = (int32_t *)M.ctl;
+        M.pool_used = (unsigned long long *)(M.ctl + 4);
+        M.ref_stats = M.ctl + MAP_CTL_WORDS;
         M.cap_refs = cr;
     }
-    if (M.pool_used == nullptr) MH_HIP(hipMalloc(&M.pool_used, sizeof(unsigned long long)));
+    {
+        const size_t bytes = sizeof(int64_t) * (MAP_CTL_WORDS + 5 * (size_t)M.cap_refs + 3);
+        if (M.stats_pin_cap < bytes) {
+            if (M.stats_pin) hipHostFree(M.stats_pin);
+            M.stats_pin = nullptr;
+            M.stats_pin_cap = 0;
+            MH_HIP(hipHostMalloc((void **)&M.stats_pin, bytes, hipHostMallocDefault));
+            M.stats_pin_cap = bytes;
+        }
+    }
     const int64_t test_cap = c.test_caps.cigar_pool_words;
     const int64_t need = test_cap > 0 ? test_cap : pool_words_for(n);
     if (need > (int64_t)INT32_MAX) {
@@ -2305,8 +2320,10 @@
     return 0;
 }
 
-__global__ void k_init_stats(int64_t *s, int n_refs)
-{
+__global__ void k_init_stats(int64_t *ctl, int n_refs)
+{
+    int64_t *s = ctl + MAP_CTL_WORDS;
+    if (blockIdx.x == 0 && threadIdx.x < MAP_CTL_WORDS) ctl[threadIdx.x] = 0;
     for (int i = blockIdx.x * blockDim.x + threadIdx.x; i < 5 * n_refs + 3; i += gridDim.x * blockDim.x)
         s[i] = ((i >= 3 * n_refs && i < 5 * n_refs) || i == 5 * n_refs + 2) ? INT64_MAX : 0;
 }
@@ -2325,14 +2342,10 @@
         M.stats_host.resize(5 * (size_t)M.n_refs + 3);
         const size_t bytes = sizeof(int64_t) * M.stats_host.size();
         if (M.stats_pin_ready) {
-            if (hipStreamSynchronize(c.stream) != hipSuccess) {
-                set_error("map_stats_host: copy failed");
-                return nullptr;
-            }
-            std::memcpy(M.stats_host.data(), M.stats_pin, bytes);
+            std::memcpy(M.stats_host.data(), M.stats_pin + MAP_CTL_WORDS, bytes);
         } else if (hipMemcpyAsync(M.stats_host.data(), M.ref_stats, bytes, hipMemcpyDeviceToHost,
                                   c.stream) != hipSuccess ||
-                   hipStreamSynchronize(c.stream) != hipSuccess) {
+                   stream_wait(c) != hipSuccess) {
             set_error("map_stats_host: copy failed");
             return nullptr;
         }
@@ -2415,7 +2428,7 @@
     else hipLaunchKernelGGL((k_probe_ext<0>), dim3(n), dim3(64), lds, s, da, d_items, d_out, n);
     MH_HIP(hipGetLastError());
     MH_HIP(hipMemcpyAsync(out, d_out, sizeof(int32_t) * 8 * (size_t)n, hipMemcpyDeviceToHost, s));
-    MH_HIP(hipStreamSynchronize(s));
+    MH_HIP(stream_wait(c));
     hipFree(d_items);
     hipFree(d_out);
     return 0;
@@ -2446,8 +2459,21 @@
     M.n_refs = c.index.n_refs;
     M.par = par;
     hipStream_t s = c.stream;
-    M.last_work = M.last_cigar = 0;
-    if (n == 0) hipLaunchKernelGGL(k_init_stats, dim3(64), dim3(256), 0, s, M.ref_stats, M.n_refs);
+    M.last_work = M.last_cigar = M.last_fast = M.last_rescue = 0;
+    auto land_and_wait = [&]() -> int {
+        M.stats_pin_ready = false;
+        hipLaunchKernelGGL(k_fix_first, dim3(8), dim3(256), 0, s, M.ref_stats, M.n_refs);
+        MH_HIP(hipGetLastError());
+        MH_HIP(hipMemcpyAsync(M.stats_pin, M.ctl, sizeof(int64_t) * (MAP_CTL_WORDS + 5 * (size_t)M.n_refs + 3),
+                              hipMemcpyDeviceToHost, s));
+        MH_HIP(stream_wait(c));
+        M.stats_pin_ready = true;
+        return 0;
+    };
+    if (n == 0) {
+        hipLaunchKernelGGL(k_init_stats, dim3(64), dim3(256), 0, s, M.ctl, M.n_refs);
+        if (int st = land_and_wait()) return st;
+    }
     if (n > 0) {
         auto launch_seed = [&]() -> int {
             SeedArgs sa{c.reads, c.index, par.mode, c.len_tab, M.cand, M.n_cand, M.yf, M.work, M.counters, M.cap_reads};
@@ -2517,9 +2543,7 @@
         if (pblocks > 1 << 16) pblocks = 1 << 16;
         if (pblocks < 1) pblocks = 1;
         for (int attempt = 0; attempt < 2; ++attempt) {
-            hipLaunchKernelGGL(k_init_stats, dim3(64), dim3(256), 0, s, M.ref_stats, M.n_refs);
-            MH_HIP(hipMemsetAsync(M.counters, 0, sizeof(int32_t) * 8, s));
-            MH_HIP(hipMemsetAsync(M.pool_used, 0, sizeof(unsigned long long), s));
+            hipLaunchKernelGGL(k_init_stats, dim3(64), dim3(256), 0, s, M.ctl, M.n_refs);
             if (int st = launch_seed()) return st;
             if (int st = launch_dp(M.work, M.counters, M.counters + 5, n * 2, "k_dp")) return st;
             if (c.reads.paired && units > 0) {
@@ -2538,16 +2562,17 @@
             hipLaunchKernelGGL(k_pair, dim3((unsigned)pblocks), dim3(256), 0, s, pa);
             prof_end(c, pp);
             MH_HIP(hipGetLastError());
+            if (int st = land_and_wait()) return st;
             int32_t ctr[5];
             unsigned long long used = 0;
-            MH_HIP(hipMemcpyAsync(ctr, M.counters, sizeof(ctr), hipMemcpyDeviceToHost, s));
-            MH_HIP(hipMemcpyAsync(&used, M.pool_used, sizeof(used), hipMemcpyDeviceToHost, s));
-            MH_HIP(hipStreamSynchronize(s));
+            std::memcpy(ctr, M.stats_pin, sizeof(ctr));
+            std::memcpy(&used, M.stats_pin + 4, sizeof(used));
             M.last_work = ctr[0] + ctr[4];
             M.last_rescue = ctr[4];
             M.last_cigar = (int64_t)used;
             M.last_fast = ctr[3];
             if (!ctr[2]) break;
+            M.stats_pin_ready = false;
             if (attempt == 1) { set_error("mh_map: CIGAR pool overflow after a retry"); return -2; }
             ++c.retries[RETRY_CIGAR_POOL];
             hipFree(M.pool);
@@ -2564,22 +2589,6 @@
             M.pool_cap = grown;
         }
     }
-    hipLaunchKernelGGL(k_fix_first, dim3(8), dim3(256), 0, s, M.ref_stats, M.n_refs);
-    MH_HIP(hipGetLastError());
-    {
-        const size_t bytes = sizeof(int64_t) * (5 * (size_t)M.n_refs + 3);
-        if (M.stats_pin_cap < bytes) {
-            if (M.stats_pin) hipHostFree(M.stats_pin);
-            M.stats_pin = nullptr;
-            M.stats_pin_cap = 0;
-            if (hipHostMalloc(&M.stats_pin, bytes, hipHostMallocDefault) == hipSuccess)
-                M.stats_pin_cap = bytes;
-            else
-                M.stats_pin = nullptr;
-        }
-        if (M.stats_pin && hipMemcpyAsync(M.stats_pin, M.ref_stats, bytes, hipMemcpyDeviceToHost, s) == hipSuccess)
-            M.stats_pin_ready = true;
-    }
     M.valid = true;
     return 0;
 }
diff --git a/micall-lite_amd/csrc/mh_pileup.hip b/micall-lite_amd/csrc/mh_pileup.hip
--- a/micall-lite_amd/csrc/mh_pileup.hip
+++ b/micall-lite_amd/csrc/mh_pileup.hip
@@ -737,12 +737,29 @@
     }
 }
 
-__global__ void k_pile_init(long long *first_unit, int32_t *max_pos, int n)
-{
-    for (int i = blockIdx.x * blockDim.x + threadIdx.x; i < n; i += gridDim.x * blockDim.x) {
+__global__ void k_pile_clear(uint4 *dense, uint8_t *nflag, uint8_t *dflag, int64_t cells,
+                             unsigned long long *read_counts, long long *first_unit,
+                             int32_t *max_pos, int n, unsigned long long *ev_ctr)
+{
+    const int64_t t0 = (int64_t)blockIdx.x * blockDim.x + threadIdx.x;
+    const int64_t stride = (int64_t)gridDim.x * blockDim.x;
+    const uint4 z = make_uint4(0, 0, 0, 0);
+    for (int64_t i = t0; i < cells; i += stride) dense[i] = z;
+    const int64_t quads = cells >> 4;
+    for (int64_t i = t0; i < quads; i += stride) {
+        ((uint4 *)nflag)[i] = z;
+        ((uint4 *)dflag)[i] = z;
+    }
+    for (int64_t i = (quads << 4) + t0; i < cells; i += stride) {
+        nflag[i] = 0;
+        dflag[i] = 0;
+    }
+    for (int64_t i = t0; i < n; i += stride) {
+        read_counts[i] = 0;
         first_unit[i] = INT64_MAX;
         max_pos[i] = 0;
     }
+    if (t0 < 4) ev_ctr[t0] = 0;
 }
 
 __global__ void k_pile_fix(long long *first_unit, int n)
@@ -867,6 +884,8 @@
     return 0;
 }
 
+static int tok_enqueue_behind_pileup(Ctx &c);
+
 int run_pileup(Ctx &c, int source, int q_cutoff)
 {
     PileState &P = c.pile;
@@ -906,18 +925,64 @@
         P.win_map_cap = 2 * (P.n_refs > 16 ? P.n_refs : 16);
         MH_HIP(hipMalloc(&P.win_map, sizeof(int32_t) * P.win_map_cap));
     }
-    if (P.n_refs > 0)
-        MH_HIP(hipMemcpyAsync(P.win_map, geo.win_map.data(), sizeof(int32_t) * 2 * P.n_refs,
-                              hipMemcpyHostToDevice, s));
+    if (P.n_refs > 0) {
+        if (P.win_pin_cap < 2 * P.n_refs || !P.win_pin) {
+            if (P.win_pin) hipHostFree(P.win_pin);
+            P.win_pin = nullptr;
+            P.win_pin_cap = 0;
+            MH_HIP(hipHostMalloc((void **)&P.win_pin, sizeof(int32_t) * P.win_map_cap, hipHostMallocDefault));
+            P.win_pin_cap = P.win_map_cap;
+        }
+        std::memcpy(P.win_pin, geo.win_map.data(), sizeof(int32_t) * 2 * P.n_refs);
+        MH_HIP(hipMemcpyAsync(P.win_map, P.win_pin, sizeof(int32_t) * 2 * P.n_refs, hipMemcpyHostToDevice, s));
+    }
     const int64_t cells = (int64_t)P.n_refs * P.cap;
+    const size_t nr = (size_t)P.n_refs;
+    {
+        const size_t need = landing_of(P).bytes;
+        if (P.land_cap < need) {
+            if (P.land) hipHostFree(P.land);
+            P.land = nullptr;
+            P.land_cap = 0;
+            MH_HIP(hipHostMalloc((void **)&P.land, need, hipHostMallocDefault));
+            P.land_cap = need;
+        }
+    }
+    P.row_land_gen = -1;
+    P.row_land_at.assign(nr, -1);
+    P.row_land_rows.assign(nr, 0);
+    size_t row_bytes = 0;
+    {
+        const bool some = P.only.size() == nr;
+        for (size_t r = 0; r < nr; ++r) {
+            if (some && !P.only[r]) continue;
+            const int32_t rows = std::min<int32_t>(P.cap, P.ref_lens[r] + MH_PILEUP_SLACK);
+            if (rows <= 0) continue;
+            P.row_land_at[r] = (int64_t)row_bytes;
+            P.row_land_rows[r] = rows;
+            row_bytes += ((size_t)rows * 18 + 15) & ~(size_t)15;
+        }
+    }
+    const bool land_rows = row_bytes > 0 && row_bytes < PILE_ROWS_LAND_MAX;
+    if (land_rows && P.row_pin_cap < row_bytes) {
+        if (P.row_pin) hipHostFree(P.row_pin);
+        P.row_pin = nullptr;
+        P.row_pin_cap = 0;
+        MH_HIP(hipHostMalloc((void **)&P.row_pin, row_bytes, hipHostMallocDefault));
+        P.row_pin_cap = row_bytes;
+    }
     for (int attempt = 0; attempt < 3; ++attempt) {
-        MH_HIP(hipMemsetAsync(P.dense, 0, sizeof(int32_t) * 4 * (cells > 0 ? cells : 1), s));
-        MH_HIP(hipMemsetAsync(P.nflag, 0, cells > 0 ? cells : 1, s));
-        MH_HIP(hipMemsetAsync(P.dflag, 0, cells > 0 ? cells : 1, s));
-        MH_HIP(hipMemsetAsync(P.read_counts, 0, sizeof(int64_t) * (P.n_refs > 0 ? P.n_refs : 1), s));
-        MH_HIP(hipMemsetAsync(P.ev_counters, 0, sizeof(int64_t) * 4, s));
-        hipLaunchKernelGGL(k_pile_init, dim3(8), dim3(256), 0, s, (long long *)P.first_unit,
-                           P.max_pos, P.n_refs);
+        P.land_ok = false;
+        P.tok_land_gen = -1;
+        {
+            int64_t cb = (cells + 255) / 256;
+            if (cb > 2048) cb = 2048;
+            if (cb < 1) cb = 1;
+            hipLaunchKernelGGL(k_pile_clear, dim3((unsigned)cb), dim3(256), 0, s, (uint4 *)P.dense, P.nflag,
+                               P.dflag, cells > 0 ? cells : 1, (unsigned long long *)P.read_counts,
+                               (long long *)P.first_unit, P.max_pos, P.n_refs > 0 ? P.n_refs : 1,
+                               (unsigned long long *)P.ev_counters);
+        }
         PileArgs A{};
         A.rec = c.map.rec;
         A.pool = c.map.pool;
@@ -946,16 +1011,39 @@
                               std::find(P.only.begin(), P.only.end(), (uint8_t)0) != P.only.end();
             const void *kern = source == 0 ? (skip ? (const void *)k_pileup<0, true> : (const void *)k_pileup<0, false>)
                                            : (skip ? (const void *)k_pileup<1, true> : (const void *)k_pileup<1, false>);
-            MH_HIP(hipFuncSetAttribute(kern, hipFuncAttributeMaxDynamicSharedMemorySize, (int)geo.lds));
+            const int ki = (source == 0 ? 0 : 2) + (skip ? 1 : 0);
+            if (!P.attr_set[ki]) {
+                MH_HIP(hipFuncSetAttribute(kern, hipFuncAttributeMaxDynamicSharedMemorySize, PU_LDS));
+                P.attr_set[ki] = true;
+            }
             void *kargs[] = {&A};
             MH_HIP(hipLaunchKernel(kern, dim3((unsigned)geo.blocks), dim3(64 * geo.wpb), kargs, geo.lds, s));
             prof_end(c, pk);
             MH_HIP(hipGetLastError());
         }
         hipLaunchKernelGGL(k_pile_fix, dim3(8), dim3(256), 0, s, (long long *)P.first_unit, P.n_refs);
+        MH_HIP(hipGetLastError());
+        const int tok_st = tok_enqueue_behind_pileup(c);
+        if (tok_st < 0) return tok_st;
+        const Landing L = landing_of(P);
+        MH_HIP(hipMemcpyAsync(L.read_counts, P.read_counts, 8 * nr, hipMemcpyDeviceToHost, s));
+        MH_HIP(hipMemcpyAsync(L.first_unit, P.first_unit, 8 * nr, hipMemcpyDeviceToHost, s));
+        MH_HIP(hipMemcpyAsync(L.max_pos, P.max_pos, 4 * nr, hipMemcpyDeviceToHost, s));
+        MH_HIP(hipMemcpyAsync(L.ev_counters, P.ev_counters, 32, hipMemcpyDeviceToHost, s));
+        if (land_rows) {
+            for (size_t r = 0; r < nr; ++r) {
+                if (P.row_land_at[r] < 0) continue;
+                const size_t rows = (size_t)P.row_land_rows[r];
+                const int64_t base = (int64_t)r * P.cap;
+                char *dst = P.row_pin + P.row_land_at[r];
+                MH_HIP(hipMemcpyAsync(dst, P.dense + 4 * base, 16 * rows, hipMemcpyDeviceToHost, s));
+                MH_HIP(hipMemcpyAsync(dst + 16 * rows, P.nflag + base, rows, hipMemcpyDeviceToHost, s));
+                MH_HIP(hipMemcpyAsync(dst + 17 * rows, P.dflag + base, rows, hipMemcpyDeviceToHost, s));
+            }
+        }
+        MH_HIP(stream_wait(c));
         int64_t ctr[4];
-        MH_HIP(hipMemcpyAsync(ctr, P.ev_counters, sizeof(ctr), hipMemcpyDeviceToHost, s));
-        MH_HIP(hipStreamSynchronize(s));
+        std::memcpy(ctr, L.ev_counters, sizeof(ctr));
         if (ctr[3] == (int64_t)PILE_ERR_INSBUF) {
             set_error("mh_pileup: the merged insertions of one read pair exceed PU_INSBUF (%d bytes)",
                       PU_INSBUF);
@@ -965,7 +1053,12 @@
             set_error("mh_pileup: malformed alignment row (CIGAR/position)");
             return -3;
         }
-        if (!ctr[2]) return 0;
+        if (!ctr[2]) {
+            P.land_ok = true;
+            if (tok_st == 0) P.tok_land_gen = P.gen;
+            if (land_rows) P.row_land_gen = P.gen;
+            return 0;
+        }
         ++c.retries[RETRY_PILE_EVENTS];
         hipFree(P.ev); hipFree(P.ev_pool);
         P.ev = nullptr; P.ev_pool = nullptr;
@@ -997,15 +1090,55 @@
 
 constexpr int TOK_LDS_SLOTS = 4096;
 constexpr int TOK_LDS_PROBES = 32;
+constexpr int TOK_MAX_BLOCKS = 256;
+
+__host__ __device__ inline int64_t tok_table_cap(int64_t ne)
+{
+    int64_t cap = 1024;
+    while (cap < 2 * ne) cap <<= 1;
+    return cap;
+}
+
+__host__ __device__ inline int64_t tok_blocks(int64_t ne, int per_block)
+{
+    const int64_t b = (ne + per_block - 1) / per_block;
+    return b > TOK_MAX_BLOCKS ? TOK_MAX_BLOCKS : (b < 1 ? 1 : b);
+}
+
+__device__ __forceinline__ int64_t tok_events(const int64_t *ctr)
+{
+    return (ctr[2] | ctr[3]) ? 0 : ctr[0];
+}
+
+__global__ void k_tok_clear(int32_t *slot, uint32_t *cnt, int32_t *used, int32_t *ovf, const int64_t *ctr)
+{
+    const int64_t cap = tok_table_cap(tok_events(ctr));
+    for (int64_t i = (int64_t)blockIdx.x * blockDim.x + threadIdx.x; i < cap; i += (int64_t)gridDim.x * blockDim.x) {
+        slot[i] = 0;
+        cnt[i] = 0;
+    }
+    if (blockIdx.x == 0 && threadIdx.x == 0) {
+        used[0] = 0;
+        *ovf = 0;
+    }
+}
+
 __global__ __launch_bounds__(1024) void k_tok_insert(const int32_t *ev, const char *pool, int64_t ne,
                                                      int32_t *slot, int32_t *used, int32_t *eslot,
-                                                     int64_t mask)
+                                                     int64_t mask, const int64_t *ctr)
 {
     __shared__ int32_t lrep[TOK_LDS_SLOTS];
     __shared__ int32_t lglob[TOK_LDS_SLOTS];
+    int64_t nblk = gridDim.x;
+    if (ctr) {
+        ne = tok_events(ctr);
+        mask = tok_table_cap(ne) - 1;
+        nblk = tok_blocks(ne, 1024);
+        if (ne <= 0 || blockIdx.x >= nblk) return;
+    }
     for (int x = threadIdx.x; x < TOK_LDS_SLOTS; x += blockDim.x) lrep[x] = 0;
     __syncthreads();
-    const int64_t per = (ne + gridDim.x - 1) / gridDim.x;
+    const int64_t per = (ne + nblk - 1) / nblk;
     const int64_t a = (int64_t)blockIdx.x * per, b = a + per < ne ? a + per : ne;
     for (int64_t e0 = a; e0 < b; e0 += blockDim.x) {
         const int64_t e = e0 + threadIdx.x;
@@ -1060,15 +1193,21 @@
 constexpr int TOK_LDS_KEYS = 8192;
 __global__ __launch_bounds__(1024) void k_tok_count(const int32_t *eslot, int64_t ne,
                                                     const int32_t *slotid, const int32_t *used,
-                                                    uint32_t *cnt)
+                                                    uint32_t *cnt, const int64_t *ctr)
 {
     __shared__ uint32_t hist[TOK_LDS_KEYS];
+    int64_t nblk = gridDim.x;
+    if (ctr) {
+        ne = tok_events(ctr);
+        nblk = tok_blocks(ne, 4096);
+        if (ne <= 0 || blockIdx.x >= nblk) return;
+    }
     const int nd = used[0];
     const bool lds = nd <= TOK_LDS_KEYS;
     if (lds)
         for (int d = threadIdx.x; d < nd; d += blockDim.x) hist[d] = 0;
     __syncthreads();
-    const int64_t per = (ne + gridDim.x - 1) / gridDim.x;
+    const int64_t per = (ne + nblk - 1) / nblk;
     const int64_t a = (int64_t)blockIdx.x * per, b = a + per < ne ? a + per : ne;
     for (int64_t e = a + threadIdx.x; e < b; e += blockDim.x) {
         const int d = slotid[eslot[e]];
@@ -1114,16 +1253,10 @@
     }
 }
 
-int run_token_aggregate(Ctx &c, int64_t ne, int64_t pool_used, std::vector<int32_t> &meta,
-                        std::string &bytes)
+static int tok_size(Ctx &c, int64_t ne, int64_t pool_used, int64_t K, int64_t &B)
 {
     PileState &P = c.pile;
-    hipStream_t s = c.stream;
-    meta.clear();
-    bytes.clear();
-    if (ne <= 0) return 0;
-    int64_t cap = 1024;
-    while (cap < 2 * ne) cap <<= 1;
+    const int64_t cap = tok_table_cap(ne);
     if (P.tok_cap < cap) {
         hipFree(P.tok_slot); hipFree(P.tok_cnt); hipFree(P.tok_used);
         P.tok_slot = nullptr; P.tok_cnt = nullptr; P.tok_used = nullptr; P.tok_cap = 0;
@@ -1139,7 +1272,6 @@
         MH_HIP(hipMalloc(&P.tok_meta, sizeof(int32_t) * (5 * (size_t)ne + 1)));
         P.tok_meta_cap = ne;
     }
-    int32_t *ovf = P.tok_meta + 5 * (size_t)P.tok_meta_cap;
     const int64_t want = c.test_caps.token_bytes > 0 ? c.test_caps.token_bytes
                                                      : std::max<int64_t>(pool_used, 64);
     if (P.tok_bytes_cap < want || (c.test_caps.token_bytes > 0 && P.tok_bytes_cap != want)) {
@@ -1149,21 +1281,7 @@
         MH_HIP(hipMalloc(&P.tok_bytes, (size_t)want));
         P.tok_bytes_cap = want;
     }
-    int32_t *slotid = P.tok_slot + cap, *eslot = P.tok_slot + 2 * cap;
-    MH_HIP(hipMemsetAsync(P.tok_slot, 0, sizeof(int32_t) * cap, s));
-    MH_HIP(hipMemsetAsync(P.tok_cnt, 0, sizeof(uint32_t) * cap, s));
-    MH_HIP(hipMemsetAsync(P.tok_used, 0, sizeof(int32_t), s));
-    int64_t blocks = (ne + 1023) / 1024;
-    if (blocks > 256) blocks = 256;
-    hipLaunchKernelGGL(k_tok_insert, dim3((unsigned)blocks), dim3(1024), 0, s, P.ev, P.ev_pool, ne,
-                       P.tok_slot, P.tok_used, eslot, cap - 1);
-    hipLaunchKernelGGL(k_tok_number, dim3(64), dim3(256), 0, s, P.tok_used, slotid);
-    int64_t cblocks = (ne + 4095) / 4096;
-    if (cblocks > 256) cblocks = 256;
-    hipLaunchKernelGGL(k_tok_count, dim3((unsigned)cblocks), dim3(1024), 0, s, eslot, ne, slotid,
-                       P.tok_used, P.tok_cnt);
-    MH_HIP(hipGetLastError());
-    const int64_t K = std::min<int64_t>(ne, 4096), B = std::min<int64_t>(P.tok_bytes_cap, 64 << 10);
+    B = std::min<int64_t>(P.tok_bytes_cap, B);
     const size_t pin_need = 16 + 20 * (size_t)K + (size_t)B;
     if (P.tok_pin_cap < pin_need) {
         if (P.tok_pin) hipHostFree(P.tok_pin);
@@ -1172,21 +1290,65 @@
         MH_HIP(hipHostMalloc((void **)&P.tok_pin, pin_need, hipHostMallocDefault));
         P.tok_pin_cap = pin_need;
     }
+    return 0;
+}
+
+static int tok_enqueue_tables(Ctx &c, int64_t ne, const int64_t *ctr)
+{
+    PileState &P = c.pile;
+    hipStream_t s = c.stream;
+    const int64_t cap = ctr ? P.tok_cap : tok_table_cap(ne);
+    int32_t *slotid = P.tok_slot + P.tok_cap, *eslot = P.tok_slot + 2 * P.tok_cap;
+    int32_t *ovf = P.tok_meta + 5 * (size_t)P.tok_meta_cap;
+    if (ctr) {
+        hipLaunchKernelGGL(k_tok_clear, dim3(64), dim3(256), 0, s, P.tok_slot, P.tok_cnt, P.tok_used, ovf, ctr);
+    } else {
+        MH_HIP(hipMemsetAsync(P.tok_slot, 0, sizeof(int32_t) * cap, s));
+        MH_HIP(hipMemsetAsync(P.tok_cnt, 0, sizeof(uint32_t) * cap, s));
+        MH_HIP(hipMemsetAsync(P.tok_used, 0, sizeof(int32_t), s));
+    }
+    const int64_t blocks = ctr ? TOK_MAX_BLOCKS : tok_blocks(ne, 1024);
+    hipLaunchKernelGGL(k_tok_insert, dim3((unsigned)blocks), dim3(1024), 0, s, P.ev, P.ev_pool, ne,
+                       P.tok_slot, P.tok_used, eslot, cap - 1, ctr);
+    hipLaunchKernelGGL(k_tok_number, dim3(64), dim3(256), 0, s, P.tok_used, slotid);
+    const int64_t cblocks = ctr ? TOK_MAX_BLOCKS : tok_blocks(ne, 4096);
+    hipLaunchKernelGGL(k_tok_count, dim3((unsigned)cblocks), dim3(1024), 0, s, eslot, ne, slotid,
+                       P.tok_used, P.tok_cnt, ctr);
+    MH_HIP(hipGetLastError());
+    return 0;
+}
+
+static int tok_enqueue_gather(Ctx &c, int64_t K, int64_t B, bool clear_ovf)
+{
+    PileState &P = c.pile;
+    hipStream_t s = c.stream;
+    int32_t *ovf = P.tok_meta + 5 * (size_t)P.tok_meta_cap;
+    if (clear_ovf) MH_HIP(hipMemsetAsync(ovf, 0, sizeof(int32_t), s));
+    hipLaunchKernelGGL(k_tok_gather, dim3(1), dim3(64), 0, s, P.ev, P.ev_pool, P.tok_slot,
+                       P.tok_cnt, P.tok_used, P.tok_meta, P.tok_bytes, P.tok_bytes_cap, ovf);
+    MH_HIP(hipGetLastError());
+    MH_HIP(hipMemcpyAsync(P.tok_pin, P.tok_used, sizeof(int32_t), hipMemcpyDeviceToHost, s));
+    MH_HIP(hipMemcpyAsync(P.tok_pin + 4, ovf, sizeof(int32_t), hipMemcpyDeviceToHost, s));
+    if (K > 0) MH_HIP(hipMemcpyAsync(P.tok_pin + 16, P.tok_meta, 20 * (size_t)K, hipMemcpyDeviceToHost, s));
+    if (B > 0) MH_HIP(hipMemcpyAsync(P.tok_pin + 16 + 20 * (size_t)K, P.tok_bytes, (size_t)B, hipMemcpyDeviceToHost, s));
+    return 0;
+}
+
+static int tok_collect(Ctx &c, int64_t ne, int64_t K, int64_t B, std::vector<int32_t> &meta,
+                       std::string &bytes)
+{
+    PileState &P = c.pile;
     for (int attempt = 0; attempt < 2; ++attempt) {
-        MH_HIP(hipMemsetAsync(ovf, 0, sizeof(int32_t), s));
-        hipLaunchKernelGGL(k_tok_gather, dim3(1), dim3(64), 0, s, P.ev, P.ev_pool, P.tok_slot,
-                           P.tok_cnt, P.tok_used, P.tok_meta, P.tok_bytes, P.tok_bytes_cap, ovf);
-        MH_HIP(hipGetLastError());
-        MH_HIP(hipMemcpyAsync(P.tok_pin, P.tok_used, sizeof(int32_t), hipMemcpyDeviceToHost, s));
-        MH_HIP(hipMemcpyAsync(P.tok_pin + 4, ovf, sizeof(int32_t), hipMemcpyDeviceToHost, s));
-        MH_HIP(hipMemcpyAsync(P.tok_pin + 16, P.tok_meta, 20 * (size_t)K, hipMemcpyDeviceToHost, s));
-        MH_HIP(hipMemcpyAsync(P.tok_pin + 16 + 20 * (size_t)K, P.tok_bytes, (size_t)B, hipMemcpyDeviceToHost, s));
-        MH_HIP(hipStreamSynchronize(s));
+        if (attempt > 0) {
+            B = std::min<int64_t>(P.tok_bytes_cap, B);
+            if (int st = tok_enqueue_gather(c, K, B, true)) return st;
+            MH_HIP(stream_wait(c));
+        }
         int32_t nd = 0, of = 0;
         std::memcpy(&nd, P.tok_pin, 4);
         std::memcpy(&of, P.tok_pin + 4, 4);
-        P.info.tok_insert_blocks = blocks;
-        P.info.tok_count_blocks = cblocks;
+        P.info.tok_insert_blocks = tok_blocks(ne, 1024);
+        P.info.tok_count_blocks = tok_blocks(ne, 4096);
         P.info.tok_ne = ne;
         P.info.tok_nd = nd;
         if (nd <= 0) return 0;
@@ -1212,6 +1374,44 @@
     }
     set_error("mh_pileup_events: token gather overflow");
     return -2;
+}
+
+int run_token_aggregate(Ctx &c, int64_t ne, int64_t pool_used, std::vector<int32_t> &meta,
+                        std::string &bytes)
+{
+    PileState &P = c.pile;
+    meta.clear();
+    bytes.clear();
+    if (ne <= 0) return 0;
+    if (P.tok_land_gen == P.gen) {
+        P.tok_land_gen = -1;
+        const int st = tok_collect(c, ne, P.tok_land_keys, P.tok_land_bytes, meta, bytes);
+        const int64_t nd = (int64_t)meta.size() / 5;
+        if (nd > P.tok_want_keys) P.tok_want_keys = 2 * nd;
+        if ((int64_t)bytes.size() > P.tok_want_bytes) P.tok_want_bytes = 2 * (int64_t)bytes.size();
+        return st;
+    }
+    const int64_t K = std::min<int64_t>(ne, 4096);
+    int64_t B = 64 << 10;
+    if (int st = tok_size(c, ne, pool_used, K, B)) return st;
+    if (int st = tok_enqueue_tables(c, ne, nullptr)) return st;
+    if (int st = tok_enqueue_gather(c, K, B, true)) return st;
+    MH_HIP(stream_wait(c));
+    return tok_collect(c, ne, K, B, meta, bytes);
+}
+
+static int tok_enqueue_behind_pileup(Ctx &c)
+{
+    PileState &P = c.pile;
+    if (P.ev_cap > (int64_t)1 << 28) return 1;
+    const int64_t K = std::min<int64_t>(P.tok_want_keys, P.ev_cap);
+    int64_t B = P.tok_want_bytes;
+    if (int st = tok_size(c, P.ev_cap, P.pool_cap, K, B)) return st;
+    if (int st = tok_enqueue_tables(c, 0, P.ev_counters)) return st;
+    if (int st = tok_enqueue_gather(c, K, B, false)) return st;
+    P.tok_land_keys = K;
+    P.tok_land_bytes = B;
+    return 0;
 }
 
 __global__ void k_pile_export(const int32_t *dense, const uint8_t *nflag, const uint8_t *dflag,
@@ -1338,7 +1538,7 @@
                        P.n_refs, n_sel > 0 ? dsel : nullptr, n_sel, unit_base, (int32_t *)dev_sum,
                        (int32_t *)dev_max, (uint8_t *)dev_flags);
     MH_HIP(hipGetLastError());
-    MH_HIP(hipStreamSynchronize(c.stream));
+    MH_HIP(stream_wait(c));
     return 0;
 }
 
@@ -1351,6 +1551,7 @@
     if (!P.dense) { set_error("no pileup to import into"); return -3; }
     MH_HIP(hipSetDevice(c.device));
     P.land_ok = false;
+    P.row_land_gen = -1;
     int32_t *dsel = nullptr;
     if (int st = upload_sel(c, n_sel, sel, &dsel)) return st;
     hipLaunchKernelGGL(k_pile_import, dim3(64, n_sel > 0 ? n_sel : 1), dim3(256), 0, c.stream,
@@ -1358,7 +1559,7 @@
                        P.n_refs, n_sel > 0 ? dsel : nullptr, n_sel, (const int32_t *)dev_sum,
                        (const int32_t *)dev_max, (const uint8_t *)dev_flags);
     MH_HIP(hipGetLastError());
-    MH_HIP(hipStreamSynchronize(c.stream));
+    MH_HIP(stream_wait(c));
     return 0;
 }
 
@@ -1397,7 +1598,7 @@
     if (n > 0) MH_HIP(hipMemcpyAsync(dev_events, P.ev, sizeof(int32_t) * 4 * n,
                                      hipMemcpyDeviceToDevice, c.stream));
     if (bytes > 0) MH_HIP(hipMemcpyAsync(dev_pool, P.ev_pool, bytes, hipMemcpyDeviceToDevice, c.stream));
-    MH_HIP(hipStreamSynchronize(c.stream));
+    MH_HIP(stream_wait(c));
     return 0;
 }
 
@@ -1453,7 +1654,7 @@
     }
     const int64_t ctr[4] = {tot_n, tot_b, 0, 0};
     MH_HIP(hipMemcpyAsync(P.ev_counters, ctr, sizeof(ctr), hipMemcpyHostToDevice, c.stream));
-    MH_HIP(hipStreamSynchronize(c.stream));
+    MH_HIP(stream_wait(c));
     ++P.gen;
     P.land_ok = false;
     return 0;
diff --git a/micall-lite_amd/csrc/mh_sam2aln.hip b/micall-lite_amd/csrc/mh_sam2aln.hip
--- a/micall-lite_amd/csrc/mh_sam2aln.hip
+++ b/micall-lite_amd/csrc/mh_sam2aln.hip
@@ -649,7 +649,7 @@
     MH_HIP(hipGetLastError());
     int32_t ctr[4];
     MH_HIP(hipMemcpyAsync(ctr, S.d_ctr, sizeof(ctr), hipMemcpyDeviceToHost, s));
-    MH_HIP(hipStreamSynchronize(s));
+    MH_HIP(stream_wait(c));
     if (ctr[0]) {
         set_error("sam2aln: merged-sequence hash collision (distinct sequences share a key)");
         return -4;
@@ -661,7 +661,7 @@
     if (S.n_unique)
         MH_HIP(hipMemcpyAsync(S.uniq.data(), S.d_uniq, sizeof(int32_t) * 2 * S.n_unique,
                               hipMemcpyDeviceToHost, s));
-    MH_HIP(hipStreamSynchronize(s));
+    MH_HIP(stream_wait(c));
     for (int64_t e = 0; e < ne; ++e)
         if (S.res[4 * e] == S2A_EMPTY) {
             set_error("sam2aln: merged sequence of unit %lld is all gaps (float division by zero)",
@@ -685,7 +685,7 @@
                            S.d_res, S.d_slot, S.d_out, S.n_unique, S.d_gather);
         MH_HIP(hipGetLastError());
         MH_HIP(hipMemcpyAsync(&S.gathered[0], S.d_gather, (size_t)g, hipMemcpyDeviceToHost, s));
-        MH_HIP(hipStreamSynchronize(s));
+        MH_HIP(stream_wait(c));
     }
     prof_flush(c);
     return 0;
@@ -798,7 +798,7 @@
     if (used > 0)
         MH_HIP(hipMemcpyAsync(S.cig.data(), c.map.pool, sizeof(uint32_t) * (size_t)used,
                               hipMemcpyDeviceToHost, s));
-    MH_HIP(hipStreamSynchronize(s));
+    MH_HIP(stream_wait(c));
     S.staged_reads = n;
     return 0;
 }
diff --git a/micall-lite_amd/micall_amd/_native.py b/micall-lite_amd/micall_amd/_native.py
--- a/micall-lite_amd/micall_amd/_native.py
+++ b/micall-lite_amd/micall_amd/_native.py
@@ -78,6 +78,7 @@
         'mh_test_pileup_info': ([_P, _P, ctypes.c_int, _P], ctypes.c_int),
         'mh_test_force_index_collision': ([_P, ctypes.c_int], ctypes.c_int),
         'mh_retry_counts': ([_P, _P], ctypes.c_int),
+        'mh_test_wait_count': ([_P, _I64P], ctypes.c_int),
         'mh_test_set_gotoh_wait': ([_P, ctypes.c_int64], ctypes.c_int),
         'mh_format_rows': ([_P, ctypes.c_int, _P, ctypes.c_int64, ctypes.c_int64,
                             ctypes.POINTER(ctypes.c_char_p), _P, ctypes.c_size_t,
@@ -913,6 +914,11 @@
         return dict(cigar_pool=int(out[0]), pileup_events=int(out[1]), token_bytes=int(out[2]),
                     gotoh_wait=int(out[3]))
 
+    def test_wait_count(self):
+        n = ctypes.c_int64()
+        check(lib().mh_test_wait_count(self.h, ctypes.byref(n)), 'mh_test_wait_count')
+        return int(n.value)
+
     def test_set_gotoh_wait(self, ticks):
         check(lib().mh_test_set_gotoh_wait(self.h, int(ticks)), 'mh_test_set_gotoh_wait')
 
```
